# a16z/Lasso

Hardware: AMD Instinct MI355X
Metric: prover lookups/sec for SparsePolynomialEvaluationProof, 2^24 AND lookups (higher is better)
Workload: dtype u256 (Montgomery Fr / ed25519 Fq integers)

## Files before the change

### lasso_amd/build.py

```python
import os
import subprocess
import sys

HERE = os.path.dirname(os.path.abspath(__file__))
ROOT = os.path.dirname(HERE)
HIPCC = os.environ.get("HIPCC", "/opt/rocm/bin/hipcc")
ARCH = "gfx950"


def _stale(target, sources):
    if not os.path.exists(target):
        return True
    t = os.path.getmtime(target)
    return any(os.path.getmtime(s) > t for s in sources)


def _glob(d, exts):
    return [os.path.join(d, f) for f in sorted(os.listdir(d)) if f.endswith(exts)]


CURVES = {"curve25519": ("", []), "bn254": ("_bn254", ["-DLASSO_BN254", "-Wl,-Bsymbolic"])}


def build_device(force=False, verbose=False, curve="curve25519"):
    suffix, flags = CURVES[curve]
    csrc = os.path.join(HERE, "csrc")
    target = os.path.join(HERE, f"liblasso_hip{suffix}.so")
    sources = _glob(csrc, (".hip", ".cuh")) + [os.path.join(ROOT, "include", f) for f in ("lasso_hip.h", "lasso_hip_wire.h", "lasso_hip_msm.h", "lasso_custom_check.h")]
    if force or _stale(target, sources):
        extra = os.environ.get("LASSO_EXTRA_HIPCC_FLAGS", "").split()
        cmd = [HIPCC, f"--offload-arch={ARCH}", "-O3", "-std=c++17", "-fPIC", "-shared", "-Wno-unused-result", *flags, *extra,
               "-o", target, os.path.join(csrc, "lasso_hip.hip")]
        if verbose:
            print(" ".join(cmd))
        subprocess.check_call(cmd)
    return target


def host_march_flags():
    ov = os.environ.get("LASSO_HOST_MARCH")
    if ov:
        return [] if ov == "none" else [f"-march={ov}"] + (["-DLASSO_HOST_V3"] if ov == "x86-64-v3" else [])
    try:
        flags = set(next(l for l in open("/proc/cpuinfo") if l.startswith("flags")).split())
    except Exception:
        flags = set()
    if {"avx2", "bmi1", "bmi2", "fma", "movbe"} <= flags:
        return ["-march=x86-64-v3", "-DLASSO_HOST_V3"]
    return []


def build_host(force=False, verbose=False, curve="curve25519"):
    suffix, flags = CURVES[curve]
    hdir = os.path.join(HERE, "host")
    target = os.path.join(HERE, f"liblasso_prover{suffix}.so")
    sources = _glob(hdir, (".cpp", ".hpp")) + _glob(os.path.join(HERE, "csrc"), (".cuh",)) + [os.path.join(ROOT, "include", f) for f in ("lasso_hip.h", "lasso_hip_wire.h", "lasso_hip_msm.h", "lasso_prover.h", "lasso_custom_check.h")]
    if not os.path.exists(os.path.join(hdir, "prover_capi.cpp")):
        return None
    dev = build_device(force=False, verbose=verbose, curve=curve)
    if force or _stale(target, sources + [dev]):
        cmd = ["g++", "-O2", *host_march_flags(), "-std=c++17", "-fPIC", "-shared", "-Wall", "-Wno-unused-function", "-Wno-unknown-pragmas", "-fno-gnu-unique", "-Wl,-Bsymbolic", *flags, "-o", target,
               os.path.join(hdir, "prover_capi.cpp"), "-L" + HERE, f"-llasso_hip{suffix}", "-Wl,-rpath,$ORIGIN"]
        if verbose:
            print(" ".join(cmd))
        subprocess.check_call(cmd)
    return target


def build_all(force=False, verbose=False):
    out = []
    for curve in CURVES:
        out += [build_device(force, verbose, curve), build_host(force, verbose, curve)]
    return tuple(out)


if __name__ == "__main__":
    print(build_all(force="--force" in sys.argv, verbose=True))
```

### lasso_amd/csrc/device_switches.cuh

```cuda
#pragma once
#include <cstddef>
#include <cstdint>
#include <cstdlib>

namespace lasso { namespace dsw {
inline bool unless0(const char* e) { return !(e && e[0] == '0'); }
inline bool if1(const char* e) { return e && e[0] == '1'; }
#define LASSO_DSWITCH(type, name, value) inline type name() { static const type v = (value); return v; }
LASSO_DSWITCH(bool, tagged_results, unless0(getenv("LASSO_TAGGED_RESULTS")))
LASSO_DSWITCH(long long, seq_start, [] { const char* e = getenv("LASSO_SEQ_START"); return e ? (long long)(uint32_t)strtoul(e, nullptr, 0) : -1LL; }())
LASSO_DSWITCH(bool, msm_tagged, unless0(getenv("LASSO_MSM_TAGGED")))
LASSO_DSWITCH(long, cubic_nx, [] { const char* e = getenv("LASSO_CUBIC_NX"); return e ? atol(e) : 0L; }())
LASSO_DSWITCH(bool, cubic_wide, unless0(getenv("LASSO_CUBIC_WIDE")))
LASSO_DSWITCH(unsigned, direct_nx, [] { const char* e = getenv("LASSO_DIRECT_NX"); const long x = e ? atol(e) : 16; return (unsigned)(x < 0 ? 0 : x > 64 ? 64 : x); }())
LASSO_DSWITCH(bool, eq_inline_big, if1(getenv("LASSO_EQ_INLINE_BIG")))
LASSO_DSWITCH(bool, lb_pipeline, unless0(getenv("LASSO_LB_PIPELINE")))
LASSO_DSWITCH(bool, lb_nt, if1(getenv("LASSO_LB_NT")))
LASSO_DSWITCH(unsigned, ahead_inkernel_wgs, [] { const char* e = getenv("LASSO_AHEAD_INKERNEL_WGS"); const long x = e ? atol(e) : 32; return (unsigned)(x < 0 ? 0 : x > 4096 ? 4096 : x); }())
LASSO_DSWITCH(bool, rounds_ahead, unless0(getenv("LASSO_ROUNDS_AHEAD")))
LASSO_DSWITCH(bool, layer_ahead, unless0(getenv("LASSO_LAYER_AHEAD")))
LASSO_DSWITCH(bool, tail_q_256, [] { const char* e = getenv("LASSO_TAIL_Q"); return (e ? atol(e) : 0) == 256; }())
LASSO_DSWITCH(bool, exp_no_leaf_store, if1(getenv("LASSO_EXP_NO_LEAF_STORE")))
LASSO_DSWITCH(size_t, msm_direct_max_n, [] { const char* e = getenv("LASSO_MSM_DIRECT_MAX_N"); return e ? (size_t)atoll(e) : (((size_t)1 << 17) + 64); }())
LASSO_DSWITCH(size_t, msm_direct8_max_n, [] { if (!unless0(getenv("LASSO_MSM_DIRECT8"))) return (size_t)0; const char* e = getenv("LASSO_MSM_DIRECT8_MAX_N"); return e ? (size_t)atoll(e) : (((size_t)1 << 14) + 64); }())
LASSO_DSWITCH(bool, msm_direct, unless0(getenv("LASSO_MSM_DIRECT")))
LASSO_DSWITCH(long, msm_direct_wgs, [] { const char* e = getenv("LASSO_MSM_DIRECT_WGS"); return e ? atol(e) : 0L; }())
LASSO_DSWITCH(bool, msm_fused, unless0(getenv("LASSO_MSM_FUSED")))
LASSO_DSWITCH(bool, msm_rows8, unless0(getenv("LASSO_MSM_ROWS8")))
LASSO_DSWITCH(bool, msm_rows8w, unless0(getenv("LASSO_MSM_ROWS8W")))
LASSO_DSWITCH(size_t, msm_rows8w_waves, [] { const char* e = getenv("LASSO_MSM_ROWS8W_WAVES"); const long x = e ? atol(e) : 0; return (size_t)(x < 0 ? 0 : x); }())
LASSO_DSWITCH(bool, msm_full8, if1(getenv("LASSO_MSM_FULL8")))
LASSO_DSWITCH(bool, bullet_ahead, unless0(getenv("LASSO_BULLET_AHEAD")))
LASSO_DSWITCH(bool, bullet_tail_ahead, unless0(getenv("LASSO_BULLET_TAIL_AHEAD")))
inline bool msm_pip() { return unless0(getenv("LASSO_MSM_PIP")); }
inline size_t msm_pip_min_cols() { const char* e = getenv("LASSO_MSM_PIP_MIN_COLS"); const long x = e ? atol(e) : 512; return (size_t)(x < 1 ? 1 : x); }
inline size_t msm_pip_scratch_mb() { const char* e = getenv("LASSO_MSM_PIP_SCRATCH_MB"); const long x = e ? atol(e) : 1200; return (size_t)(x < 16 ? 16 : x); }
#undef LASSO_DSWITCH
} }
```

### lasso_amd/csrc/lasso_hip.hip

```cpp
#include <hip/hip_runtime.h>
#include <mutex>
#include <string>
#include <unordered_map>
#include <vector>
#include <cstring>
#include <cstdio>
#include <cstdlib>
#include <ctime>
#include "../../include/lasso_hip.h"
#include "device_switches.cuh"
#include "launch_plan.cuh"
#include "poly_kernels.cuh"
#include "msm_kernels.cuh"
#include "densify_kernels.cuh"
#include "../../include/lasso_hip_wire.h"
#include "wire_kernels.cuh"
#include "../../include/lasso_hip_msm.h"
#include "msm_points_kernels.cuh"

__global__ void __launch_bounds__(256) k_inner_lr(const fr_t* __restrict__ a, const fr_t* __restrict__ b, size_t half, fr_t* __restrict__ partials) {
  __shared__ RedScratch S;
  fr29 acc[3] = {fr29_zero(), fr29_zero(), fr29_zero()}; uint32_t cnt = 0;
  for (size_t i = blockIdx.x * (size_t)blockDim.x + threadIdx.x; i < half; i += (size_t)gridDim.x * blockDim.x) {
    acc[0] = fr29_weak(fr29_add(acc[0], fr29_mul(fr29_unpack_u(a[i]), fr29_unpack_s(b[half + i]))));
    acc[1] = fr29_weak(fr29_add(acc[1], fr29_mul(fr29_unpack_u(a[half + i]), fr29_unpack_s(b[i]))));
    if ((++cnt & 127u) == 0) { acc[0] = fr29_mul(acc[0], fr29_one_s()); acc[1] = fr29_mul(acc[1], fr29_one_s()); }
  }
  store_block_partials<3>(acc, 2, partials + 2 * (size_t)blockIdx.x, 0, S);
}

static_assert(sizeof(lasso_fr) == 32 && sizeof(fr_t) == 32, "Fr layout");
static_assert(sizeof(lasso_affine) == 64 && sizeof(lasso_point) == 128 && sizeof(ed_point) == 128 && sizeof(niels29) == (MSM_NIELS_ALIGN > 16 ? 128 : 112) && sizeof(pt29) == MSM_PT29_BYTES, "curve layouts");

namespace dsw = lasso::dsw;
struct EventPair { hipEvent_t a, b; int kid; double bytes, units, units2; bool large; bool counted; };
#define LASSO_PROF_COUNT_SLOTS 4096
struct lasso_ctx {
  int device = 0;
  hipStream_t stream = nullptr;
  std::string err;
  void* d_scratch = nullptr; size_t scratch_cap = 0;
  void* d_pip = nullptr; size_t pip_cap = 0;
  fr_t* d_small = nullptr;
  fr_t* h_small = nullptr;
  size_t small_cap = 0;
  uint32_t* h_flag = nullptr; uint32_t* d_flag = nullptr;
  uint32_t* h_tag = nullptr; uint32_t* d_tag = nullptr;
  bool tagged = true;
  HandoffState proto;
  std::vector<lasso_fr> group_tmp;
  uint32_t* mail_h = nullptr; uint32_t* mail_d = nullptr;
  uint32_t seq = 0;
  uint64_t stat_waits = 0; double stat_wait_us = 0;
  fr_t* d_big = nullptr; fr_t* h_big = nullptr; size_t big_cap = 0;
  uint32_t* d_flags = nullptr;
  uint32_t* d_counters = nullptr;
  uint32_t* d_gmail = nullptr;
  uint32_t* pmail_h = nullptr; uint32_t* pmail_d = nullptr; uint32_t* d_gpoint = nullptr;
  uint32_t prof_mask = 0;
  std::vector<EventPair> events; size_t events_used = 0;
  uint64_t prof_launches[LASSO_K_COUNT] = {0}; double prof_ms[LASSO_K_COUNT] = {0}; double prof_bytes[LASSO_K_COUNT] = {0};
  uint64_t big_launches[LASSO_K_COUNT] = {0}; double big_ms[LASSO_K_COUNT] = {0}; double big_bytes[LASSO_K_COUNT] = {0};
  double prof_units[LASSO_K_COUNT] = {0}; double big_units[LASSO_K_COUNT] = {0};
  double prof_units2[LASSO_K_COUNT] = {0}; double big_units2[LASSO_K_COUNT] = {0};
  double prof_units3[LASSO_K_COUNT] = {0}; double big_units3[LASSO_K_COUNT] = {0};
  uint32_t* d_prof_counts = nullptr;
  void* d_terms = nullptr; std::vector<uint8_t> terms_host;
  void* rccl_comm = nullptr; int rccl_world = 0; int rccl_rank = -1;
  std::unordered_map<void*, size_t> mem_sizes; uint64_t mem_live = 0, mem_peak = 0; std::mutex mem_mu;
};
struct lasso_bases {
  size_t n = 0; niels29* d_table = nullptr;
  lasso_ctx* owner = nullptr;
  niels29* d_mult = nullptr;
  niels29* d_mult8 = nullptr;
  niels29* d_tab8[2] = {nullptr, nullptr};
  bool tab8_failed = false;
  std::mutex tab8_mu;
};

static thread_local std::string g_create_err;
static std::mutex g_ctx_mu; static std::vector<lasso_ctx*> g_ctx_live;
static lasso_ctx* live_or_null(lasso_ctx* c) { std::lock_guard<std::mutex> g(g_ctx_mu); for (lasso_ctx* x : g_ctx_live) if (x == c) return c; return nullptr; }

static int32_t fail(lasso_ctx* c, int32_t code, const std::string& msg) { if (c) c->err = msg; else g_create_err = msg; return code; }
#define HIPCHK(c, call) do { hipError_t e_ = (call); if (e_ != hipSuccess) return fail((c), e_ == hipErrorOutOfMemory ? LASSO_ERR_OOM : LASSO_ERR_HIP, std::string(#call) + ": " + hipGetErrorString(e_)); } while (0)
static inline bool bind_device(lasso_ctx* c) { if (!c) return true; int d = -1; if (hipGetDevice(&d) == hipSuccess && d == c->device) return true; return hipSetDevice(c->device) == hipSuccess; }
#define REQUIRE(c, cond) do { if (!bind_device(c)) return fail((c), LASSO_ERR_HIP, "hipSetDevice failed for the context's device"); \
                              if (!(cond)) return fail((c), LASSO_ERR_INVALID, std::string("invalid argument: ") + #cond); } while (0)

static hipError_t dmalloc(lasso_ctx* c, void** p, size_t bytes) {
  hipError_t e = hipMalloc(p, bytes);
  if (e == hipSuccess && c) { std::lock_guard<std::mutex> g(c->mem_mu); c->mem_sizes[*p] = bytes; c->mem_live += bytes; if (c->mem_live > c->mem_peak) c->mem_peak = c->mem_live; }
  return e;
}
static hipError_t dfree(lasso_ctx* c, void* p) {
  if (c && p) { std::lock_guard<std::mutex> g(c->mem_mu); auto it = c->mem_sizes.find(p); if (it != c->mem_sizes.end()) { c->mem_live -= it->second; c->mem_sizes.erase(it); } }
  return hipFree(p);
}

static int32_t grow_guard(lasso_ctx* c) {
  if (c->proto.no_grow) return LASSO_ERR_UNSUPPORTED;
  if (c->proto.waiting_on_device()) return fail(c, LASSO_ERR_INVALID, "a launch is waiting on the device for its challenge: only lasso_result_wait and the post of that challenge are legal until then");
  return 0;
}
static int32_t ensure_scratch(lasso_ctx* c, size_t bytes) {
  if (bytes <= c->scratch_cap) return 0;
  if (int32_t g = grow_guard(c)) return g;
  if (c->d_scratch) { HIPCHK(c, hipStreamSynchronize(c->stream)); HIPCHK(c, dfree(c, c->d_scratch)); c->d_scratch = nullptr; c->scratch_cap = 0; }
  size_t cap = bytes < ((size_t)1 << 22) ? ((size_t)1 << 22) : bytes;
  HIPCHK(c, dmalloc(c, &c->d_scratch, cap)); c->scratch_cap = cap; return 0;
}
static int32_t ensure_pip(lasso_ctx* c, size_t bytes) {
  if (bytes <= c->pip_cap) return 0;
  if (!c->proto.may_grow()) return LASSO_ERR_UNSUPPORTED;
  if (c->d_pip) { HIPCHK(c, hipStreamSynchronize(c->stream)); HIPCHK(c, dfree(c, c->d_pip)); c->d_pip = nullptr; c->pip_cap = 0; }
  if (dmalloc(c, &c->d_pip, bytes) != hipSuccess) { (void)hipGetLastError(); c->d_pip = nullptr; return LASSO_ERR_UNSUPPORTED; }
  c->pip_cap = bytes; return 0;
}
static int32_t ensure_small(lasso_ctx* c, size_t count) {
  if (count <= c->small_cap) return 0;
  if (int32_t g = grow_guard(c)) return g;
  HIPCHK(c, hipStreamSynchronize(c->stream));
  if (c->h_small) (void)hipHostFree(c->h_small);
  c->h_small = nullptr; c->d_small = nullptr; c->small_cap = 0;
  size_t cap = count < 4096 ? 4096 : count;
  HIPCHK(c, hipHostMalloc((void**)&c->h_small, cap * sizeof(fr_t), hipHostMallocMapped | hipHostMallocCoherent));
  HIPCHK(c, hipHostGetDevicePointer((void**)&c->d_small, c->h_small, 0));
  if (c->h_tag) (void)hipHostFree(c->h_tag);
  c->h_tag = nullptr; c->d_tag = nullptr;
  HIPCHK(c, hipHostMalloc((void**)&c->h_tag, cap * 48, hipHostMallocMapped | hipHostMallocCoherent));
  memset(c->h_tag, 0, cap * 48);
  HIPCHK(c, hipHostGetDevicePointer((void**)&c->d_tag, c->h_tag, 0));
  c->small_cap = cap; return 0;
}
static int32_t ensure_big(lasso_ctx* c, size_t count) {
  if (count <= c->big_cap) return 0;
  if (int32_t g = grow_guard(c)) return g;
  HIPCHK(c, hipStreamSynchronize(c->stream));
  if (c->d_big) (void)dfree(c, c->d_big);
  if (c->h_big) (void)hipHostFree(c->h_big);
// ... 199 lines not shown
      rc = LASSO_ERR_HIP; msg = "lasso_rccl_selftest: the 1 KB all-gather did not complete within 20 s (a peer never entered it, or the fabric is down)";
      if (a->CommAbort) (void)a->CommAbort((ncclComm_t)c->rccl_comm); c->rccl_comm = nullptr; c->rccl_world = 0;
    }
  }
  if (!rc) {
    if (hipMemcpy(all.data(), d + bytes, bytes * (size_t)world, hipMemcpyDeviceToHost) != hipSuccess) { rc = LASSO_ERR_HIP; msg = "lasso_rccl_selftest: download"; }
    else for (int g = 0; g < world && !rc; g++) for (size_t i = 0; i < bytes; i++) if (all[(size_t)g * bytes + i] != (uint8_t)(((size_t)g * 131 + i * 7 + 1) % 251)) { rc = LASSO_ERR_HIP; msg = "lasso_rccl_selftest: slot " + std::to_string(g) + " does not hold rank " + std::to_string(g) + "'s bytes"; break; }
  }
  if (ev) (void)hipEventDestroy(ev);
  if (c->rccl_comm || rc == 0) (void)hipFree(d);
  (void)hipGetLastError();
  return rc ? fail(c, rc, msg) : 0;
}
int32_t lasso_rccl_allgather(lasso_ctx* c, const void* d_send, void* d_recv, size_t bytes) {
  REQUIRE(c, d_send && d_recv && c->rccl_comm);
  RcclApi* a = rccl_api(nullptr);
  ncclResult_t r = a->AllGather(d_send, d_recv, bytes, ncclUint8, (ncclComm_t)c->rccl_comm, c->stream);
  if (r != ncclSuccess) return fail(c, LASSO_ERR_HIP, std::string("ncclAllGather: ") + a->GetErrorString(r));
  return 0;
}
int32_t lasso_points_reduce_compress(lasso_ctx* c, const void* d_parts, uint32_t groups, size_t rows, uint8_t* out32) {
  REQUIRE(c, d_parts && out32 && groups >= 1 && rows >= 1);
  int32_t rc = ensure_scratch(c, rows * 32 + 256); if (rc) return rc;
  {
    ProfScope ps(c, LASSO_K_MSM, (double)groups * rows * sizeof(pt29), (double)(groups - 1) * rows);
    hipLaunchKernelGGL(k_points_reduce_compress, dim3(grid_for(rows)), dim3(256), 0, c->stream, (const pt29*)d_parts, groups, rows, (uint32_t*)c->d_scratch);
  }
  HIPCHK(c, hipGetLastError());
  HIPCHK(c, hipMemcpyAsync(out32, c->d_scratch, rows * 32, hipMemcpyDeviceToHost, c->stream));
  HIPCHK(c, hipStreamSynchronize(c->stream));
  return 0;
}

static inline void post_mail(lasso_ctx* c, uint32_t tag, const uint32_t w[8]) {
  mail_chunks(c->mail_h, tag, w);
  mail_fence();
}
int32_t lasso_ctx_create(int32_t device, lasso_ctx** out) { return lasso_ctx_create_background(device, 0, out); }
int32_t lasso_ctx_device_uuid(lasso_ctx* c, uint8_t out[16]) {
  REQUIRE(c, c && out);
  hipUUID u; memset(&u, 0, sizeof(u));
  HIPCHK(c, hipDeviceGetUuid(&u, c->device));
  static_assert(sizeof(u.bytes) == 16, "hipUUID");
  memcpy(out, u.bytes, 16); return 0;
}
int32_t lasso_ctx_create_background(int32_t device, int32_t background, lasso_ctx** out) {
  if (!out) return fail(nullptr, LASSO_ERR_INVALID, "out is NULL");
  int n = 0;
  hipError_t e = hipGetDeviceCount(&n);
  if (e != hipSuccess || n == 0) return fail(nullptr, LASSO_ERR_HIP, std::string("no HIP device: ") + hipGetErrorString(e));
  if (device < 0 || device >= n) return fail(nullptr, LASSO_ERR_INVALID, "device index out of range");
  lasso_ctx* c = new lasso_ctx(); c->device = device;
  int prio_lo = 0, prio_hi = 0;
  if ((e = hipSetDevice(device)) == hipSuccess) (void)hipDeviceGetStreamPriorityRange(&prio_lo, &prio_hi);
  if (e != hipSuccess || (e = hipStreamCreateWithPriority(&c->stream, hipStreamNonBlocking, background ? prio_lo : prio_hi)) != hipSuccess) {
    std::string m = hipGetErrorString(e); delete c; return fail(nullptr, LASSO_ERR_HIP, m);
  }
  if (hipMalloc((void**)&c->d_flags, 64) != hipSuccess) { delete c; return fail(nullptr, LASSO_ERR_OOM, "flags alloc"); }
  if (hipMalloc((void**)&c->d_counters, (LASSO_MAX_PTRS + 40) * 4) != hipSuccess || hipMemset(c->d_counters, 0, (LASSO_MAX_PTRS + 40) * 4) != hipSuccess) { delete c; return fail(nullptr, LASSO_ERR_OOM, "counters alloc"); }
  if (hipHostMalloc((void**)&c->h_flag, 256, hipHostMallocMapped | hipHostMallocCoherent) != hipSuccess || hipHostGetDevicePointer((void**)&c->d_flag, c->h_flag, 0) != hipSuccess) { delete c; return fail(nullptr, LASSO_ERR_OOM, "mapped flag alloc"); }
  *c->h_flag = 0;
  c->tagged = dsw::tagged_results();
  if (dsw::seq_start() >= 0) c->seq = (uint32_t)dsw::seq_start();
  c->mail_h = c->h_flag + 32; c->mail_d = c->d_flag + 32;
  memset(c->h_flag, 0, 256);
  int32_t rc = ensure_small(c, (size_t)1 << 16); if (rc) { g_create_err = c->err; delete c; return rc; }
  rc = ensure_scratch(c, (size_t)1 << 22); if (rc) { g_create_err = c->err; delete c; return rc; }
  if (dmalloc(c, (void**)&c->d_gmail, 128) != hipSuccess || hipMemset(c->d_gmail, 0, 128) != hipSuccess) { g_create_err = "gmail alloc"; delete c; return LASSO_ERR_OOM; }
  if (hipHostMalloc((void**)&c->pmail_h, LASSO_PMAIL_BYTES, hipHostMallocMapped | hipHostMallocCoherent) != hipSuccess || hipHostGetDevicePointer((void**)&c->pmail_d, c->pmail_h, 0) != hipSuccess) { g_create_err = "point mailbox alloc"; delete c; return LASSO_ERR_OOM; }
  memset(c->pmail_h, 0, LASSO_PMAIL_BYTES);
  if (dmalloc(c, (void**)&c->d_gpoint, LASSO_GPOINT_BYTES) != hipSuccess || hipMemset(c->d_gpoint, 0, LASSO_GPOINT_BYTES) != hipSuccess) { g_create_err = "gpoint alloc"; delete c; return LASSO_ERR_OOM; }
  { std::lock_guard<std::mutex> g(g_ctx_mu); g_ctx_live.push_back(c); }
  *out = c; return 0;
}
int32_t lasso_abort(lasso_ctx* c) {
  REQUIRE(c, c);
  const uint32_t zero8[8] = {0, 0, 0, 0, 0, 0, 0, 0};
  if (c->proto.lay_active && c->pmail_h) for (uint32_t j = 0; j < LASSO_POINT_MAX + 2; j++) mail_chunks(c->pmail_h + 12 * j, LASSO_MAIL_POISON, zero8);
  if (c->proto.tail_active || c->proto.waiting_on_device()) { mail_chunks(c->mail_h + 12, LASSO_MAIL_POISON, zero8); post_mail(c, LASSO_MAIL_POISON, zero8); }
  (void)hipStreamSynchronize(c->stream);
  (void)hipGetLastError();
  if (c->pmail_h) memset(c->pmail_h, 0, LASSO_PMAIL_BYTES);
  mail_chunks(c->mail_h + 12, 0, zero8); post_mail(c, 0, zero8);
  c->proto.reset(); c->events_used = 0;
  HIPCHK(c, hipMemsetAsync(c->d_counters, 0, (LASSO_MAX_PTRS + 40) * 4, c->stream));
  HIPCHK(c, hipStreamSynchronize(c->stream));
  return 0;
}
void lasso_ctx_destroy(lasso_ctx* c) {
  if (!c) return;
  { std::lock_guard<std::mutex> g(g_ctx_mu); for (size_t i = 0; i < g_ctx_live.size(); i++) if (g_ctx_live[i] == c) { g_ctx_live.erase(g_ctx_live.begin() + i); break; } }
  (void)hipSetDevice(c->device);
  if (!c->proto.idle()) (void)lasso_abort(c);
  (void)hipStreamSynchronize(c->stream);
  rccl_release(c);
  for (auto& p : c->events) { (void)hipEventDestroy(p.a); (void)hipEventDestroy(p.b); }
  if (c->d_scratch) (void)hipFree(c->d_scratch);
  if (c->d_pip) (void)hipFree(c->d_pip);
  if (c->d_gmail) (void)hipFree(c->d_gmail);
  if (c->d_gpoint) (void)hipFree(c->d_gpoint);
  if (c->pmail_h) (void)hipHostFree(c->pmail_h);
  if (c->h_small) (void)hipHostFree(c->h_small);
  if (c->h_tag) (void)hipHostFree(c->h_tag);
  if (c->h_flag) (void)hipHostFree(c->h_flag);
  if (c->d_big) (void)hipFree(c->d_big);
  if (c->h_big) (void)hipHostFree(c->h_big);
  if (c->d_flags) (void)hipFree(c->d_flags);
  if (c->d_counters) (void)hipFree(c->d_counters);
  if (c->d_prof_counts) (void)hipFree(c->d_prof_counts);
  if (c->d_terms) (void)hipFree(c->d_terms);
  (void)hipStreamDestroy(c->stream);
  delete c;
}
const char* lasso_last_error(lasso_ctx* c) { return c ? c->err.c_str() : g_create_err.c_str(); }
void* lasso_stream(lasso_ctx* c) { return c ? (void*)c->stream : nullptr; }
int32_t lasso_alloc(lasso_ctx* c, size_t bytes, void** d_out) { REQUIRE(c, d_out); HIPCHK(c, dmalloc(c, d_out, bytes ? bytes : 1)); return 0; }
int32_t lasso_free(lasso_ctx* c, void* p) { if (!p) return 0; REQUIRE(c, c && !c->proto.waiting_on_device()); HIPCHK(c, hipStreamSynchronize(c->stream)); HIPCHK(c, dfree(c, p)); return 0; }
int32_t lasso_mem_stats(lasso_ctx* c, uint64_t* live_bytes, uint64_t* peak_bytes, int32_t reset_peak) {
  REQUIRE(c, c); std::lock_guard<std::mutex> g(c->mem_mu);
  if (live_bytes) *live_bytes = c->mem_live; if (peak_bytes) *peak_bytes = c->mem_peak; if (reset_peak) c->mem_peak = c->mem_live; return 0;
}
int32_t lasso_trim(lasso_ctx* c) {
  REQUIRE(c, c && c->proto.idle());
  HIPCHK(c, hipStreamSynchronize(c->stream));
  if (c->d_pip) { HIPCHK(c, dfree(c, c->d_pip)); c->d_pip = nullptr; c->pip_cap = 0; }
  if (c->scratch_cap <= ((size_t)1 << 22)) return 0;
  HIPCHK(c, dfree(c, c->d_scratch)); c->d_scratch = nullptr; c->scratch_cap = 0;
  return ensure_scratch(c, (size_t)1 << 22);
}
int32_t lasso_upload(lasso_ctx* c, void* d, const void* s, size_t n) { REQUIRE(c, d && s && !c->proto.waiting_on_device()); HIPCHK(c, hipMemcpyAsync(d, s, n, hipMemcpyHostToDevice, c->stream)); HIPCHK(c, hipStreamSynchronize(c->stream)); return 0; }
int32_t lasso_download(lasso_ctx* c, void* d, const void* s, size_t n) { REQUIRE(c, d && s && !c->proto.waiting_on_device()); HIPCHK(c, hipMemcpyAsync(d, s, n, hipMemcpyDeviceToHost, c->stream)); HIPCHK(c, hipStreamSynchronize(c->stream)); return 0; }
int32_t lasso_copy(lasso_ctx* c, void* d, const void* s, size_t n) { REQUIRE(c, d && s); ProfScope ps(c, LASSO_K_MISC, 2.0 * n); HIPCHK(c, hipMemcpyAsync(d, s, n, hipMemcpyDeviceToDevice, c->stream)); return 0; }
int32_t lasso_zero(lasso_ctx* c, void* d, size_t n) { REQUIRE(c, d); HIPCHK(c, hipMemsetAsync(d, 0, n, c->stream)); return 0; }
int32_t lasso_sync(lasso_ctx* c) { REQUIRE(c, c && !c->proto.waiting_on_device()); HIPCHK(c, hipStreamSynchronize(c->stream)); return 0; }

int32_t lasso_prof_get_large(lasso_ctx* c, int32_t k, uint64_t* launches, double* ms, double* bytes) {
  REQUIRE(c, k >= 0 && k < LASSO_K_COUNT); prof_flush(c);
  if (launches) *launches = c->big_launches[k]; if (ms) *ms = c->big_ms[k]; if (bytes) *bytes = c->big_bytes[k]; return 0;
}
int32_t lasso_wait_stats(lasso_ctx* c, uint64_t* waits, double* wait_us, int32_t reset) { REQUIRE(c, waits && wait_us); *waits = c->stat_waits; *wait_us = c->stat_wait_us; if (reset) { c->stat_waits = 0; c->stat_wait_us = 0; } return 0; }
int32_t lasso_prof_enable(lasso_ctx* c, int32_t mask) { prof_flush(c); c->prof_mask = (uint32_t)mask; return 0; }
int32_t lasso_prof_reset(lasso_ctx* c) { prof_flush(c); for (int i = 0; i < LASSO_K_COUNT; i++) { c->prof_launches[i] = 0; c->prof_ms[i] = 0; c->prof_bytes[i] = 0; c->big_launches[i] = 0; c->big_ms[i] = 0; c->big_bytes[i] = 0; c->prof_units[i] = 0; c->big_units[i] = 0; c->prof_units2[i] = 0; c->big_units2[i] = 0; c->prof_units3[i] = 0; c->big_units3[i] = 0; } return 0; }
int32_t lasso_prof_get_units(lasso_ctx* c, int32_t k, int32_t large_only, double* units) {
  REQUIRE(c, k >= 0 && k < LASSO_K_COUNT && units); prof_flush(c);
  const bool large = large_only & 1, second = large_only & 2, third = large_only & 4;
  *units = third ? (large ? c->big_units3[k] : c->prof_units3[k]) : second ? (large ? c->big_units2[k] : c->prof_units2[k]) : (large ? c->big_units[k] : c->prof_units[k]); return 0;
}
int32_t lasso_prof_get(lasso_ctx* c, int32_t k, uint64_t* launches, double* ms, double* bytes) {
  REQUIRE(c, k >= 0 && k < LASSO_K_COUNT); prof_flush(c);
  if (launches) *launches = c->prof_launches[k]; if (ms) *ms = c->prof_ms[k]; if (bytes) *bytes = c->prof_bytes[k]; return 0;
}

int32_t lasso_fr_from_u32(lasso_ctx* c, const uint32_t* d_src, size_t n, lasso_fr* d_dst) {
  REQUIRE(c, d_src && d_dst); if (!n) return 0;
  ProfScope ps(c, LASSO_K_MISC, 36.0 * n);
  hipLaunchKernelGGL(k_from_u32, dim3(grid_for(n)), dim3(LASSO_BLOCK), 0, c->stream, d_src, n, (fr_t*)d_dst);
  HIPCHK(c, hipGetLastError()); return 0;
}
__global__ void __launch_bounds__(256) k_subtable_u32(int32_t kind, uint32_t sub, uint32_t log_m, uint32_t log_r, uint32_t* __restrict__ out) {
  const size_t m = (size_t)1 << log_m; const uint32_t bits = log_m / 2, mask = (1u << bits) - 1u;
  for (size_t i = blockIdx.x * (size_t)blockDim.x + threadIdx.x; i < m; i += (size_t)gridDim.x * blockDim.x) {
    const uint32_t r = (uint32_t)i & mask, l = (uint32_t)(i >> bits) & mask;
    uint32_t v;
    if (kind == LASSO_AND) v = l & r;
    else if (kind == LASSO_OR) v = l | r;
    else if (kind == LASSO_XOR) v = l ^ r;
    else if (kind == LASSO_LT) v = sub == 0 ? (l < r ? 1u : 0u) : (l == r ? 1u : 0u);
    else { const size_t cutoff = (size_t)1 << (log_r % log_m); v = sub == 0 ? (uint32_t)i : (sub == 1 ? (i < cutoff ? (uint32_t)i : 0u) : 0u); }
    out[i] = v;
  }
}
int32_t lasso_materialize_subtable_u32(lasso_ctx* c, const lasso_strategy* s, uint32_t sub, uint32_t* d_out) {
  REQUIRE(c, s && d_out && s->kind >= LASSO_AND && s->kind <= LASSO_RANGE && s->log_m >= 1 && s->log_m <= 31);
  const uint32_t nsub = s->kind == LASSO_LT ? 2u : (s->kind == LASSO_RANGE ? 3u : 1u);
  REQUIRE(c, sub < nsub);
  hipLaunchKernelGGL(k_subtable_u32, dim3(grid_for((size_t)1 << s->log_m)), dim3(256), 0, c->stream, s->kind, sub, s->log_m, s->log_r, d_out);
  HIPCHK(c, hipGetLastError()); return 0;
}
int32_t lasso_gather(lasso_ctx* c, const lasso_fr* d_table, const uint32_t* d_idx, size_t n, lasso_fr* d_out) {
  REQUIRE(c, d_table && d_idx && d_out); if (!n) return 0;
  ProfScope ps(c, LASSO_K_MISC, 68.0 * n);
  hipLaunchKernelGGL(k_gather, dim3(grid_for(n)), dim3(LASSO_BLOCK), 0, c->stream, (const fr_t*)d_table, d_idx, n, (fr_t*)d_out);
  HIPCHK(c, hipGetLastError()); return 0;
}
int32_t lasso_eq_evals(lasso_ctx* c, const lasso_fr* r, uint32_t ell, lasso_fr* d_out) { return lasso_eq_evals_scaled(c, r, ell, nullptr, d_out); }
int32_t lasso_eq_evals_scaled(lasso_ctx* c, const lasso_fr* r, uint32_t ell, const lasso_fr* scale, lasso_fr* d_out) {
  REQUIRE(c, d_out && ell <= 40 && (r || ell == 0));
  const fr_t sc = scale ? to_fr(scale) : fr_one();
  const size_t n = (size_t)1 << ell;
  ProfScope ps(c, LASSO_K_EQ, 32.0 * n);
  if (ell <= 12) {
    RTable R; for (uint32_t j = 0; j < ell; j++) R.r[j] = to_fr(r + j);
    hipLaunchKernelGGL(k_eq_small, dim3(grid_for(n)), dim3(LASSO_BLOCK), 0, c->stream, R, ell, sc, (fr_t*)d_out);
  } else {
    const uint32_t lo_bits = ell / 2, hi_bits = ell - lo_bits;
    int32_t rc = ensure_scratch(c, (((size_t)1 << hi_bits) + ((size_t)1 << lo_bits)) * sizeof(fr_t)); if (rc) return rc;
    fr_t* hi = (fr_t*)c->d_scratch; fr_t* lo = hi + ((size_t)1 << hi_bits);
    if (hi_bits <= 16) {
      RTable16 Rh, Rl; for (uint32_t j = 0; j < 16; j++) { Rh.r[j] = j < hi_bits ? to_fr(r + j) : fr_zero(); Rl.r[j] = j < lo_bits ? to_fr(r + hi_bits + j) : fr_zero(); }
      const unsigned hb = grid_for((size_t)1 << hi_bits), lb = grid_for((size_t)1 << lo_bits);
      hipLaunchKernelGGL(k_eq_small2, dim3(hb + lb), dim3(LASSO_BLOCK), 0, c->stream, Rh, hi_bits, sc, hi, hb, Rl, lo_bits, lo);
    } else {
      RTable Rh, Rl; for (uint32_t j = 0; j < hi_bits; j++) Rh.r[j] = to_fr(r + j); for (uint32_t j = 0; j < lo_bits; j++) Rl.r[j] = to_fr(r + hi_bits + j);
      hipLaunchKernelGGL(k_eq_small, dim3(grid_for((size_t)1 << hi_bits)), dim3(LASSO_BLOCK), 0, c->stream, Rh, hi_bits, sc, hi);
      hipLaunchKernelGGL(k_eq_small, dim3(grid_for((size_t)1 << lo_bits)), dim3(LASSO_BLOCK), 0, c->stream, Rl, lo_bits, fr_one(), lo);
    }
    hipLaunchKernelGGL(k_eq_outer, dim3(grid_for(n, 4096)), dim3(LASSO_BLOCK), 0, c->stream, (const fr_t*)hi, (const fr_t*)lo, lo_bits, n, (fr_t*)d_out);
  }
  HIPCHK(c, hipGetLastError()); return 0;
}
int32_t lasso_bind_top(lasso_ctx* c, lasso_fr* const* d_polys, uint32_t npolys, size_t n, const lasso_fr* r) {
  REQUIRE(c, d_polys && r && npolys >= 1 && npolys <= LASSO_MAX_PTRS && n >= 2 && (n & (n - 1)) == 0);
  MutPtrTable T; for (uint32_t i = 0; i < npolys; i++) { REQUIRE(c, d_polys[i]); T.p[i] = (fr_t*)d_polys[i]; }
  const size_t half = n / 2;
  ProfScope ps(c, LASSO_K_BIND, 48.0 * n * npolys);
  hipLaunchKernelGGL(k_bind_top, dim3(grid_for(half, 4096), npolys), dim3(LASSO_BLOCK), 0, c->stream, T, half, to_fr(r));
  HIPCHK(c, hipGetLastError()); return 0;
}
static unsigned round_nx(size_t items, unsigned ny) { return round_nx(items, ny, dsw::cubic_nx()); }
int32_t lasso_sumcheck_cubic_round(lasso_ctx* c, const lasso_fr* const* d_A, const lasso_fr* const* d_B, uint32_t ncirc, const lasso_fr* d_C, size_t n, lasso_fr* out) {
  REQUIRE(c, d_A && d_B && d_C && out && ncirc >= 1 && ncirc <= LASSO_MAX_PTRS && n >= 2 && (n & (n - 1)) == 0);
  const size_t half = n / 2;
  int32_t rc = ensure_small(c, (size_t)ncirc * 3); if (rc) return rc;
  const uint32_t seq = next_seq(c);
  PtrTable A, B; for (uint32_t i = 0; i < ncirc; i++) { REQUIRE(c, d_A[i] && d_B[i]); A.p[i] = (const fr_t*)d_A[i]; B.p[i] = (const fr_t*)d_B[i]; }
  const unsigned ny = ncirc, nx = round_nx(half, ny);
  rc = ensure_scratch(c, (size_t)nx * ny * 3 * sizeof(fr_t)); if (rc) return rc;
  {
    ProfScope ps(c, LASSO_K_CUBIC, 32.0 * n * (2.0 * ncirc + 1.0));
    hipLaunchKernelGGL(k_cubic_round_lb, dim3(nx * ny), dim3(LASSO_BLOCK), 0, c->stream, A, B, nx, ny, (const fr_t*)d_C, half, (fr_t*)c->d_scratch, c->d_counters, RES(c), seq);
  }
  HIPCHK(c, hipGetLastError());
  return wait_flag(c, seq, (size_t)ncirc * 3, out, c->tagged);
}
extern "C++" {
struct EqPointArg { const lasso_fr* point; uint32_t ell; fr_t scale; };
static CubicPlan cubic_plan_for(lasso_ctx* c, uint32_t ncirc, size_t n, bool has_r, int NT, bool has_eqi, bool want_groups, bool ahead, const EqPointArg* eqg, int gate_ell) {
  const CubicShape s = {n, ncirc, NT, ahead, has_r, has_eqi, eqg != nullptr, eqg ? eqg->ell : 0u, gate_ell, c->prof_mask, want_groups && c->tagged};
  const CubicSwitches sw = {dsw::cubic_nx(), dsw::cubic_wide(), dsw::direct_nx(), dsw::eq_inline_big(), dsw::lb_pipeline(), dsw::lb_nt(), dsw::ahead_inkernel_wgs()};
  return cubic_plan(s, sw);
}
template <class TM, class TP>
static int32_t cubic_eqw_launch_t(lasso_ctx* c, lasso_fr* const* d_A, lasso_fr* const* d_B, uint32_t ncirc, const lasso_fr* d_E, size_t n, const lasso_fr* r, int NT, uint32_t* seq_out, const EqInline* eqi, uint32_t* groups_out, bool ahead = false, const EqPointArg* eqg = nullptr, int gate_ell = -1) {
  if (groups_out) *groups_out = 1;
  const CubicPlan P = cubic_plan_for(c, ncirc, n, r != nullptr, NT, eqi != nullptr, groups_out != nullptr, ahead, eqg, gate_ell);
  if (P.form == CUBIC_REFUSED) return fail(c, LASSO_ERR_UNSUPPORTED, P.refusal);
  TM A, B; for (uint32_t i = 0; i < ncirc; i++) { REQUIRE(c, d_A[i] && d_B[i]); A.p[i] = (fr_t*)d_A[i]; B.p[i] = (fr_t*)d_B[i]; }
  int32_t rc = ensure_small(c, (size_t)ncirc * 3); if (rc) return rc;
  const uint32_t seq = next_seq(c); *seq_out = seq;
  const unsigned nx = P.nx, ny = P.ny;
  const fr_t rr = r ? to_fr(r) : fr_zero();
  const double bytes = (P.bind ? 48.0 : 32.0) * n * (2.0 * ncirc + 1.0);
  fr_t* r_out = nullptr; uint32_t* r_flag = nullptr;
  auto reserve = [&]() -> int32_t {
    int32_t e = ensure_scratch(c, P.scratch_elems * sizeof(fr_t)); if (e) return e;
    if (P.direct) { *groups_out = nx; e = ensure_small(c, (size_t)ncirc * 3 * nx); if (e) return e; }
    r_out = c->tagged ? (fr_t*)c->d_tag : c->d_small; r_flag = P.direct ? LASSO_TAGGED_DIRECT : c->tagged ? LASSO_TAGGED : c->d_flag;
    return 0;
  };
  if (P.form == CUBIC_SMALL) {
    ProfScope ps(c, LASSO_K_CUBIC, bytes);
#define LAUNCH_CSMALL(BIND_, NT_) hipLaunchKernelGGL((k_cubic_eqw_small<BIND_, NT_, TM>), dim3(ncirc), dim3(LASSO_BLOCK), 0, c->stream, A, B, (const fr_t*)d_E, (uint32_t)P.items, rr, c->d_counters, RES(c), seq)
    if (P.bind) { if (NT == 3) LAUNCH_CSMALL(true, 3); else LAUNCH_CSMALL(true, 2); }
    else { if (NT == 3) LAUNCH_CSMALL(false, 3); else LAUNCH_CSMALL(false, 2); }
  } else if (P.form == CUBIC_FUSED) {
    if (ahead) { if ((rc = reserve())) return rc; if (P.gate) hipLaunchKernelGGL(k_gate, dim3(1), dim3(64), 0, c->stream, (const uint32_t*)c->mail_d, c->d_gmail, seq, 0u); }
    ProfScope ps(c, LASSO_K_CUBIC, bytes);
    if (!ahead && (rc = reserve())) return rc;
    const uint32_t* const gmail = ahead ? (const uint32_t*)c->d_gmail : (const uint32_t*)nullptr; const uint32_t* const wait_mail = P.inkernel ? (const uint32_t*)c->mail_d : (const uint32_t*)nullptr;
#define LAUNCH_CFUSED(NT_, WIDE_, AHEAD_) hipLaunchKernelGGL((k_cubic_eqw_fused<NT_, WIDE_, TM, AHEAD_>), dim3(nx * ny), dim3(LASSO_BLOCK), 0, c->stream, A, B, nx, ny, (const fr_t*)d_E, P.items, rr, (fr_t*)c->d_scratch, c->d_counters, r_out, r_flag, seq, gmail, wait_mail)
    if (ahead) { if (P.wide) LAUNCH_CFUSED(2, true, true); else LAUNCH_CFUSED(2, false, true); }
    else if (NT == 3) LAUNCH_CFUSED(3, false, false);
    else if (P.wide) LAUNCH_CFUSED(2, true, false);
    else LAUNCH_CFUSED(2, false, false);
  } else {
    const CubicLbPlan& L = P.lb;
    TP Ac, Bc; for (uint32_t i = 0; i < ncirc; i++) { Ac.p[i] = A.p[i]; Bc.p[i] = B.p[i]; }
    if ((rc = reserve())) return rc;
    fr_t* const f_hi = (fr_t*)c->d_scratch + P.part_elems; fr_t* const f_lo = f_hi + ((size_t)1 << L.g_hi);
    if (L.gate) { hipLaunchKernelGGL(k_gate_point, dim3(1), dim3(64), 0, c->stream, (const uint32_t*)c->pmail_d, c->d_gpoint, seq, (uint32_t)gate_ell + 2u, c->pmail_d + LASSO_PMAIL_ACK_WORD); c->proto.gate_sent = seq; }
    const uint32_t* const gate_gp = L.gate ? (const uint32_t*)c->d_gpoint : (const uint32_t*)nullptr;
    if (L.factors) {
      ProfScope pe(c, LASSO_K_EQ, L.eq_outer ? 32.0 * P.items : 32.0 * (((size_t)1 << L.g_hi) + ((size_t)1 << L.g_lo)));
      const unsigned hb = grid_for((size_t)1 << L.g_hi), lb2 = grid_for((size_t)1 << L.g_lo);
      if (L.factors_gated) hipLaunchKernelGGL(k_eq_small2_mem, dim3(hb + lb2), dim3(LASSO_BLOCK), 0, c->stream, (const uint32_t*)c->d_gpoint, seq, L.g_hi, f_hi, hb, L.g_lo, f_lo);
      else {
        RTable16 Rh, Rl; for (uint32_t j = 0; j < 16; j++) { Rh.r[j] = j < L.g_hi ? to_fr(eqg->point + j) : fr_zero(); Rl.r[j] = j < L.g_lo ? to_fr(eqg->point + L.g_hi + j) : fr_zero(); }
        hipLaunchKernelGGL(k_eq_small2, dim3(hb + lb2), dim3(LASSO_BLOCK), 0, c->stream, Rh, L.g_hi, eqg->scale, f_hi, hb, Rl, L.g_lo, f_lo);
      }
      if (L.eq_outer) hipLaunchKernelGGL(k_eq_outer, dim3(grid_for(P.items, 4096)), dim3(LASSO_BLOCK), 0, c->stream, (const fr_t*)f_hi, (const fr_t*)f_lo, L.g_lo, P.items, (fr_t*)d_E, gate_gp, seq);
    }
    ProfScope ps(c, LASSO_K_CUBIC, bytes);
#define LAUNCH_CLB(NT_, EQI_, TE_, NTL_, E_, EQ_, OUT_) hipLaunchKernelGGL((k_cubic_eqw_lb<NT_, EQI_, TP, TE_, NTL_>), dim3(nx * ny), dim3(LASSO_BLOCK), 0, c->stream, Ac, Bc, nx, ny, (const fr_t*)(E_), P.items, (fr_t*)c->d_scratch, c->d_counters, r_out, r_flag, seq, L.pipe, EQ_, (fr_t*)(OUT_))
    switch (L.eq) {
      case CUBIC_EQ_TABLE: {
        EqNone EN; if (L.eq_outer) { EN.gp = gate_gp; EN.seq = seq; }
        if (NT == 3) LAUNCH_CLB(3, false, EqNone, false, d_E, EN, nullptr);
        else if (L.nt) LAUNCH_CLB(2, false, EqNone, true, d_E, EN, nullptr);
        else LAUNCH_CLB(2, false, EqNone, false, d_E, EN, nullptr);
      } break;
      case CUBIC_EQ_LDS: LAUNCH_CLB(2, true, EqInline, false, nullptr, *eqi, d_E); break;
      case CUBIC_EQ_GATED: { EqInlineMem M; M.gp = c->d_gpoint; M.seq = seq; M.ell = (uint32_t)gate_ell; LAUNCH_CLB(2, true, EqInlineMem, false, nullptr, M, d_E); } break;
      case CUBIC_EQ_FACTORS: {
        EqGlobal G; G.hi = f_hi; G.lo = f_lo; G.lo_bits = L.g_lo; G.ell = L.g_ell; G.gp = L.gate ? c->d_gpoint : nullptr; G.seq = L.gate ? seq : 0;
        LAUNCH_CLB(2, true, EqGlobal, false, nullptr, G, d_E);
      } break;
    }
  }
  HIPCHK(c, hipGetLastError());
  return 0;
}
}
static int32_t cubic_eqw_launch(lasso_ctx* c, lasso_fr* const* d_A, lasso_fr* const* d_B, uint32_t ncirc, const lasso_fr* d_E, size_t n, const lasso_fr* r, int NT, uint32_t* seq_out, const EqInline* eqi = nullptr, uint32_t* groups_out = nullptr, bool ahead = false, const EqPointArg* eqg = nullptr, int gate_ell = -1) {
  return ncirc <= 8 ? cubic_eqw_launch_t<MutPtrTable8, PtrTable8>(c, d_A, d_B, ncirc, d_E, n, r, NT, seq_out, eqi, groups_out, ahead, eqg, gate_ell) : cubic_eqw_launch_t<MutPtrTable, PtrTable>(c, d_A, d_B, ncirc, d_E, n, r, NT, seq_out, eqi, groups_out, ahead, eqg, gate_ell);
}
int32_t lasso_sumcheck_cubic_eqw_round(lasso_ctx* c, const lasso_fr* const* d_A, const lasso_fr* const* d_B, uint32_t ncirc, const lasso_fr* d_E, size_t n, lasso_fr* out) {
  REQUIRE(c, d_A && d_B && d_E && out && ncirc >= 1 && ncirc <= LASSO_MAX_PTRS && n >= 2 && (n & (n - 1)) == 0);
  uint32_t seq, groups; int32_t rc = cubic_eqw_launch(c, (lasso_fr* const*)d_A, (lasso_fr* const*)d_B, ncirc, d_E, n, nullptr, 3, &seq, nullptr, &groups); if (rc) return rc;
  return wait_flag(c, seq, (size_t)ncirc * 3, out, c->tagged, groups, 3);
}
int32_t lasso_sumcheck_cubic_eqw_round_fused(lasso_ctx* c, lasso_fr* const* d_A, lasso_fr* const* d_B, uint32_t ncirc, const lasso_fr* d_E, size_t n, const lasso_fr* r, lasso_fr* out) {
  REQUIRE(c, d_A && d_B && d_E && r && out && ncirc >= 1 && ncirc <= LASSO_MAX_PTRS && n >= 4 && (n & (n - 1)) == 0);
  uint32_t seq, groups; int32_t rc = cubic_eqw_launch(c, d_A, d_B, ncirc, d_E, n, r, 3, &seq, nullptr, &groups); if (rc) return rc;
  return wait_flag(c, seq, (size_t)ncirc * 3, out, c->tagged, groups, 3);
}
int32_t lasso_sumcheck_cubic_eqw2_begin(lasso_ctx* c, lasso_fr* const* d_A, lasso_fr* const* d_B, uint32_t ncirc, const lasso_fr* d_E, size_t n, const lasso_fr* r) {
  REQUIRE(c, d_A && d_B && d_E && ncirc >= 1 && ncirc <= LASSO_MAX_PTRS && n >= (r ? 4u : 2u) && (n & (n - 1)) == 0 && !c->proto.pending);
  uint32_t seq, groups; int32_t rc = cubic_eqw_launch(c, d_A, d_B, ncirc, d_E, n, r, 2, &seq, nullptr, &groups); if (rc) return rc;
  c->proto.park(Handoff{seq, (size_t)ncirc * 2, c->tagged, groups, 2});
  return 0;
}
int32_t lasso_sumcheck_cubic_eqw2_begin_ahead(lasso_ctx* c, lasso_fr* const* d_A, lasso_fr* const* d_B, uint32_t ncirc, const lasso_fr* d_E, size_t n) {
  REQUIRE(c, d_A && d_B && d_E && ncirc >= 1 && ncirc <= LASSO_MAX_PTRS && n >= 4 && (n & (n - 1)) == 0 && !c->proto.ahead_active && !c->proto.tail_active && !c->proto.defer_next);
  const CubicPlan P = cubic_plan_for(c, ncirc, n, false, 2, false, true, true, nullptr, -1);
  if (P.form == CUBIC_REFUSED) return fail(c, LASSO_ERR_UNSUPPORTED, "lasso_sumcheck_cubic_eqw2_begin_ahead: streaming rounds only");
  { int32_t rc0 = ensure_small(c, (size_t)ncirc * 3 * (P.direct ? P.nx : 1)); if (rc0) return rc0; rc0 = ensure_scratch(c, P.scratch_elems * sizeof(fr_t)); if (rc0) return rc0; }
  uint32_t seq, groups; int32_t rc = cubic_eqw_launch(c, d_A, d_B, ncirc, d_E, n, nullptr, 2, &seq, nullptr, &groups, true); if (rc) return rc;
  c->proto.arm_ahead(Handoff{seq, (size_t)ncirc * 2, c->tagged, groups, 2}, false);
  return 0;
}
int32_t lasso_challenge_post(lasso_ctx* c, const lasso_fr* r) {
  REQUIRE(c, r && c->proto.ahead_active && !c->proto.ahead_bullet && !c->proto.pending);
  post_mail(c, c->proto.post_ahead(), (const uint32_t*)r);
  return 0;
}
int32_t lasso_rounds_ahead_ok(lasso_ctx* c) { return c && dsw::rounds_ahead() && c->mail_d && c->d_gmail ? 1 : 0; }
static int32_t cubic_tail_begin_impl(lasso_ctx* c, uint32_t m_stop, lasso_fr* const* d_A, lasso_fr* const* d_B, uint32_t ncirc, const lasso_fr* d_E, size_t n, const lasso_fr* r, const EqInline* eqi, bool ahead, int gate_ell = -1);
static uint32_t take_handover(lasso_ctx* c) { return c ? c->proto.take_handover() : 0; }
int32_t lasso_sumcheck_cubic_tail_begin(lasso_ctx* c, lasso_fr* const* d_A, lasso_fr* const* d_B, uint32_t ncirc, const lasso_fr* d_E, size_t n, const lasso_fr* r) {
  const uint32_t ho = take_handover(c);
  REQUIRE(c, d_E);
  return cubic_tail_begin_impl(c, ho, d_A, d_B, ncirc, d_E, n, r, nullptr, false);
}
static bool make_eq_inline(const lasso_fr* point, uint32_t ell, const lasso_fr* scale, EqInline& Q) {
  if (ell > 14 || (ell && !point)) return false;
  for (uint32_t j = 0; j < 14; j++) Q.r[j] = j < ell ? to_fr(point + j) : fr_zero();
  Q.scale = scale ? to_fr(scale) : fr_one(); Q.ell = ell; return true;
}
int32_t lasso_sumcheck_cubic_eqw2_begin_eq(lasso_ctx* c, lasso_fr* const* d_A, lasso_fr* const* d_B, uint32_t ncirc, lasso_fr* d_E_out, size_t n, const lasso_fr* point, uint32_t ell, const lasso_fr* scale) {
  REQUIRE(c, d_A && d_B && d_E_out && ncirc >= 1 && ncirc <= LASSO_MAX_PTRS && n >= 2 && (n & (n - 1)) == 0 && !c->proto.pending && ((size_t)1 << ell) == n / 2);
  EqInline Q;
  if (n / 2 <= CUBIC_SMALL_Q || (ell && !point) || ell > 32) return fail(c, LASSO_ERR_UNSUPPORTED, "lasso_sumcheck_cubic_eqw2_begin_eq: tables of 2^7 .. 2^32 entries only");
  uint32_t seq, groups; int32_t rc;
  if (make_eq_inline(point, ell, scale, Q)) rc = cubic_eqw_launch(c, d_A, d_B, ncirc, d_E_out, n, nullptr, 2, &seq, &Q, &groups);
  else { EqPointArg G; G.point = point; G.ell = ell; G.scale = scale ? to_fr(scale) : fr_one(); rc = cubic_eqw_launch(c, d_A, d_B, ncirc, d_E_out, n, nullptr, 2, &seq, nullptr, &groups, false, &G); }
  if (rc) return rc;
  c->proto.park(Handoff{seq, (size_t)ncirc * 2, c->tagged, groups, 2});
  return 0;
}
int32_t lasso_sumcheck_cubic_tail_begin_eq(lasso_ctx* c, lasso_fr* const* d_A, lasso_fr* const* d_B, uint32_t ncirc, size_t n, const lasso_fr* point, uint32_t ell, const lasso_fr* scale) {
  const uint32_t ho = take_handover(c);
  REQUIRE(c, n >= 2 && ((size_t)1 << ell) == n / 2 && ell <= 9);
  EqInline Q; if (!make_eq_inline(point, ell, scale, Q)) return fail(c, LASSO_ERR_INVALID, "lasso_sumcheck_cubic_tail_begin_eq: bad point");
  return cubic_tail_begin_impl(c, ho, d_A, d_B, ncirc, nullptr, n, nullptr, &Q, false);
}
extern "C++" {
template <class TM>
static int32_t cubic_tail_begin_t(lasso_ctx* c, uint32_t m_stop_arg, lasso_fr* const* d_A, lasso_fr* const* d_B, uint32_t ncirc, const lasso_fr* d_E, size_t n, const lasso_fr* r, const EqInline* eqi, bool ahead, int gate_ell) {
  const uint32_t m_stop = m_stop_arg ? m_stop_arg : 1u;
  const bool gated = gate_ell >= 0;
  REQUIRE(c, d_A && d_B && (d_E || eqi || gated) && ncirc >= 1 && ncirc <= LASSO_MAX_PTRS && n >= ((r || ahead) ? 4u : 2u) && (n & (n - 1)) == 0 && (ahead || gated || !c->proto.pending) && (gated || !c->proto.tail_active) && !c->proto.defer_next && !c->proto.ahead_active && !c->proto.lay_active);
  const size_t q = (r || ahead) ? n / 4 : n / 2;
  REQUIRE(c, q >= 1 && q <= CUBIC_TAIL_Q && (m_stop & (m_stop - 1)) == 0 && m_stop <= 128 && 2 * q > m_stop);
  TM A, B; for (uint32_t i = 0; i < ncirc; i++) { REQUIRE(c, d_A[i] && d_B[i]); A.p[i] = (fr_t*)d_A[i]; B.p[i] = (fr_t*)d_B[i]; }
  int32_t rc = ensure_small(c, (size_t)ncirc * 2 * (m_stop > 2 ? m_stop : 2)); if (rc) return rc;
  uint32_t turns = 0; while (((size_t)m_stop << turns) < 2 * q) turns++;
  const uint32_t seq0 = next_seq(c, turns + 1);
#define LAUNCH_CTAIL(B_, Q_, I_, TE_, R_, EQ_) hipLaunchKernelGGL((k_cubic_tail<B_, Q_, I_, TM, TE_>), dim3(ncirc), dim3(Q_), 0, c->stream, A, B, (const fr_t*)d_E, (uint32_t)q, R_, (const uint32_t*)c->mail_d, c->d_counters, RES(c), seq0, EQ_, m_stop, ahead ? 1u : 0u)
  if (gated) {
    hipLaunchKernelGGL(k_gate_point, dim3(1), dim3(64), 0, c->stream, (const uint32_t*)c->pmail_d, c->d_gpoint, seq0, (uint32_t)gate_ell + 2u, c->pmail_d + LASSO_PMAIL_ACK_WORD); c->proto.gate_sent = seq0;
    EqInlineMem M; M.gp = c->d_gpoint; M.seq = seq0; M.ell = (uint32_t)gate_ell;
    if (tail_threads(q) == 256) LAUNCH_CTAIL(false, 256, true, EqInlineMem, fr_zero(), M); else LAUNCH_CTAIL(false, 512, true, EqInlineMem, fr_zero(), M);
    HIPCHK(c, hipGetLastError());
    c->proto.arm_layer_tail(Handoff{seq0, (size_t)ncirc * 2, c->tagged}, (uint32_t)gate_ell, turns, (size_t)ncirc * 2 * m_stop);
    return 0;
  }
  if (eqi) { if (tail_threads(q) == 256) LAUNCH_CTAIL(false, 256, true, EqInline, fr_zero(), *eqi); else LAUNCH_CTAIL(false, 512, true, EqInline, fr_zero(), *eqi); }
  else if (tail_threads(q) == 256) { if (r || ahead) LAUNCH_CTAIL(true, 256, false, EqNone, r ? to_fr(r) : fr_zero(), EqNone()); else LAUNCH_CTAIL(false, 256, false, EqNone, fr_zero(), EqNone()); }
  else { if (r || ahead) LAUNCH_CTAIL(true, 512, false, EqNone, r ? to_fr(r) : fr_zero(), EqNone()); else LAUNCH_CTAIL(false, 512, false, EqNone, fr_zero(), EqNone()); }
  HIPCHK(c, hipGetLastError());
  c->proto.begin_tail(Handoff{seq0, (size_t)ncirc * 2, c->tagged}, turns, (size_t)ncirc * 2 * m_stop, ahead);
  return 0;
}
}
static int32_t cubic_tail_begin_impl(lasso_ctx* c, uint32_t m_stop, lasso_fr* const* d_A, lasso_fr* const* d_B, uint32_t ncirc, const lasso_fr* d_E, size_t n, const lasso_fr* r, const EqInline* eqi, bool ahead, int gate_ell) {
  return ncirc <= 8 ? cubic_tail_begin_t<MutPtrTable8>(c, m_stop, d_A, d_B, ncirc, d_E, n, r, eqi, ahead, gate_ell) : cubic_tail_begin_t<MutPtrTable>(c, m_stop, d_A, d_B, ncirc, d_E, n, r, eqi, ahead, gate_ell);
}
static bool gate_free(lasso_ctx* c) { return !c->proto.gate_sent || __atomic_load_n(c->pmail_h + LASSO_PMAIL_ACK_WORD, __ATOMIC_ACQUIRE) == c->proto.gate_sent; }
int32_t lasso_layer_ahead_ok(lasso_ctx* c) { return c && dsw::layer_ahead() && c->pmail_d && c->d_gpoint ? 1 : 0; }
int32_t lasso_sumcheck_cubic_eqw2_begin_eq_ahead(lasso_ctx* c, lasso_fr* const* d_A, lasso_fr* const* d_B, uint32_t ncirc, lasso_fr* d_E_out, size_t n, uint32_t ell) {
  REQUIRE(c, d_A && d_B && d_E_out && ncirc >= 1 && ncirc <= LASSO_MAX_PTRS && n >= 2 && (n & (n - 1)) == 0 && ell < 48 && ((size_t)1 << ell) == n / 2 && !c->proto.waiting_on_device() && !c->proto.defer_next);
  if (!lasso_layer_ahead_ok(c) || n / 2 <= CUBIC_SMALL_Q || ell > 32 || ell > LASSO_POINT_MAX) return fail(c, LASSO_ERR_UNSUPPORTED, "lasso_sumcheck_cubic_eqw2_begin_eq_ahead: tables of 2^7 .. 2^32 entries only");
  if (!gate_free(c)) return fail(c, LASSO_ERR_UNSUPPORTED, "lasso_sumcheck_cubic_eqw2_begin_eq_ahead: the previous point gate has not consumed its message yet");
  uint32_t seq, groups;
  c->proto.no_grow = true;
  const int32_t rc = cubic_eqw_launch(c, d_A, d_B, ncirc, d_E_out, n, nullptr, 2, &seq, nullptr, &groups, false, nullptr, (int)ell);
  c->proto.no_grow = false;
  if (rc == LASSO_ERR_UNSUPPORTED) return fail(c, rc, "lasso_sumcheck_cubic_eqw2_begin_eq_ahead: a buffer would have to grow while kernels are in flight");
  if (rc) return rc;
  HIPCHK(c, hipGetLastError());
  c->proto.arm_layer(Handoff{seq, (size_t)ncirc * 2, c->tagged, groups, 2}, ell);
  return 0;
}
int32_t lasso_sumcheck_cubic_tail_begin_eq_ahead(lasso_ctx* c, lasso_fr* const* d_A, lasso_fr* const* d_B, uint32_t ncirc, size_t n, uint32_t ell) {
  const uint32_t ho = take_handover(c);
  REQUIRE(c, n >= 2 && ell <= 9 && ((size_t)1 << ell) == n / 2);
  if (!lasso_layer_ahead_ok(c)) return fail(c, LASSO_ERR_UNSUPPORTED, "lasso_sumcheck_cubic_tail_begin_eq_ahead: switched off");
  if (!gate_free(c)) return fail(c, LASSO_ERR_UNSUPPORTED, "lasso_sumcheck_cubic_tail_begin_eq_ahead: the previous point gate has not consumed its message yet");
  c->proto.no_grow = true;
  const int32_t rc = cubic_tail_begin_impl(c, ho, d_A, d_B, ncirc, nullptr, n, nullptr, nullptr, false, (int)ell);
  c->proto.no_grow = false;
  if (rc == LASSO_ERR_UNSUPPORTED) return fail(c, rc, "lasso_sumcheck_cubic_tail_begin_eq_ahead: a buffer would have to grow while kernels are in flight");
  return rc;
}
static void point_mail(lasso_ctx* c, uint32_t ell, const lasso_fr* point, const lasso_fr* scale, uint32_t ctrl) {
  const uint32_t zero8[8] = {0, 0, 0, 0, 0, 0, 0, 0}; const fr_t one = fr_one();
  for (uint32_t j = 0; j < ell; j++) mail_chunks(c->pmail_h + 12 * j, c->proto.lay.seq, point ? (const uint32_t*)(point + j) : zero8);
  mail_chunks(c->pmail_h + 12 * ell, c->proto.lay.seq, scale ? (const uint32_t*)scale : one.v);
  const uint32_t ctl[8] = {ctrl, 0, 0, 0, 0, 0, 0, 0};
  mail_chunks(c->pmail_h + 12 * (ell + 1), c->proto.lay.seq, ctl);
  mail_fence();
}
int32_t lasso_point_post(lasso_ctx* c, const lasso_fr* point, uint32_t ell, const lasso_fr* scale) {
  REQUIRE(c, c && c->proto.lay_active && ell == c->proto.lay_ell && (point || !ell) && !c->proto.pending && !c->proto.tail_active && !c->proto.ahead_active);
  point_mail(c, ell, point, scale, 0u);
  c->proto.post_layer();
  return 0;
}
int32_t lasso_point_cancel(lasso_ctx* c) {
  REQUIRE(c, c && c->proto.lay_active);
  point_mail(c, c->proto.lay_ell, nullptr, nullptr, 1u);
  c->proto.cancel_layer();
  return 0;
}
int32_t lasso_sumcheck_cubic_tail_begin_ahead(lasso_ctx* c, lasso_fr* const* d_A, lasso_fr* const* d_B, uint32_t ncirc, const lasso_fr* d_E, size_t n) {
  const uint32_t ho = take_handover(c);
  REQUIRE(c, d_E);
  return cubic_tail_begin_impl(c, ho, d_A, d_B, ncirc, d_E, n, nullptr, nullptr, true);
}
int32_t lasso_tail_handover_next(lasso_ctx* c, uint32_t m_stop) {
  REQUIRE(c, c && (m_stop & (m_stop - 1)) == 0 && m_stop <= 128);
  c->proto.handover_next = m_stop <= 1 ? 0 : m_stop; return 0;
}
int32_t lasso_sumcheck_linear_tail_begin(lasso_ctx* c, const lasso_fr* const* d_src, uint32_t alpha, const lasso_fr* d_E, size_t n, const lasso_fr* r) {
  const uint32_t ho = take_handover(c);
  REQUIRE(c, d_src && d_E && alpha >= 1 && alpha <= LASSO_MAX_PTRS && n >= (r ? 4u : 2u) && (n & (n - 1)) == 0 && !c->proto.pending && !c->proto.tail_active && !c->proto.defer_next && !ho && !c->proto.ahead_active);
  const size_t q = r ? n / 4 : n / 2;
  REQUIRE(c, q >= 1 && q <= CUBIC_TAIL_Q);
  PtrTable Src; for (uint32_t i = 0; i < alpha; i++) { REQUIRE(c, d_src[i]); Src.p[i] = (const fr_t*)d_src[i]; }
  int32_t rc = ensure_small(c, (size_t)alpha * 3); if (rc) return rc;
  uint32_t turns = 0; while (((size_t)1 << turns) < 2 * q) turns++;
  const uint32_t seq0 = next_seq(c, turns + 1);
#define LAUNCH_LTAIL(B_, Q_, R_) hipLaunchKernelGGL((k_linear_tail<B_, Q_>), dim3(alpha), dim3(Q_), 0, c->stream, Src, (const fr_t*)d_E, (uint32_t)q, R_, (const uint32_t*)c->mail_d, c->d_counters, RES(c), seq0)
  if (tail_threads(q) == 256) { if (r) LAUNCH_LTAIL(true, 256, to_fr(r)); else LAUNCH_LTAIL(false, 256, fr_zero()); }
  else { if (r) LAUNCH_LTAIL(true, 512, to_fr(r)); else LAUNCH_LTAIL(false, 512, fr_zero()); }
  HIPCHK(c, hipGetLastError());
  c->proto.begin_tail(Handoff{seq0, (size_t)alpha * 2, c->tagged}, turns, alpha, false);
  return 0;
}
int32_t lasso_sumcheck_cubic_tail_next(lasso_ctx* c, const lasso_fr* r) {
  REQUIRE(c, r && c->proto.tail_active && !c->proto.pending);
  const fr_t rr = to_fr(r);
  post_mail(c, c->proto.tail_next(), rr.v);
  return 0;
}
uint32_t lasso_sumcheck_tail_capacity(void) { return dsw::tail_q_256() ? 256 : CUBIC_TAIL_Q; }
int32_t lasso_defer_next(lasso_ctx* c) { REQUIRE(c, !c->proto.pending && !c->proto.defer_next); c->proto.defer_next = true; return 0; }
int32_t lasso_result_wait(lasso_ctx* c, lasso_fr* out, size_t count) {
  REQUIRE(c, out && c->proto.pending && count == c->proto.result.count);
  const Handoff h = c->proto.collect();
  return wait_flag(c, h.seq, count, out, h.tagged, h.groups, h.K);
}
// ... 899 lines not shown
```

### lasso_amd/csrc/launch_plan.cuh

```cuda
#pragma once
#include <cstddef>
#include <cstdint>
#include "../../include/lasso_hip.h"

#define LASSO_BLOCK 256
#define CUBIC_SMALL_Q 64
#define CUBIC_TAIL_Q 512
#define MSM_THREADS 256
#define MSM_WINDOWS 64
#define MSM_PIP_WINDOWS 21
#define MSM_PIP_BUCKETS 2048
#define MSM_SMALL_ROWS 16
#define MSM_PT29_BYTES 144
#ifdef LASSO_BN254
#define FR_MODULUS_BITS 254u
#else
#define FR_MODULUS_BITS 253u
#endif
constexpr uint32_t msm_direct_windows(int wb) { return 256u / (uint32_t)wb; }

static inline unsigned grid_for(size_t n, unsigned cap = 2048) { size_t g = (n + LASSO_BLOCK - 1) / LASSO_BLOCK; if (g < 1) g = 1; if (g > cap) g = cap; return (unsigned)g; }
static inline bool prof_bracketed(uint32_t prof_mask, int family) { return ((prof_mask >> family) & 1u) && !(prof_mask & (uint32_t)LASSO_PROF_LARGE_ONLY); }

static inline unsigned round_nx(size_t items, unsigned ny, long cubic_nx) {
  unsigned cap = 512 / (ny ? ny : 1); if (cap < 64) cap = 64;
  return grid_for(items, cubic_nx > 0 ? (unsigned)cubic_nx : cap);
}
static inline unsigned tail_threads(size_t q) { return q <= 256 ? 256u : 512u; }

struct CubicSwitches { long cubic_nx; bool wide; unsigned direct_nx; bool eq_inline_big, lb_pipeline, lb_nt; unsigned ahead_inkernel_wgs; };
struct CubicShape { size_t n; uint32_t ncirc; int NT; bool ahead, has_r, has_eqi, has_eqg; uint32_t eqg_ell; int gate_ell; uint32_t prof_mask; bool direct_ok; };
enum CubicForm { CUBIC_REFUSED, CUBIC_SMALL, CUBIC_LB, CUBIC_FUSED };
enum CubicEq {
  CUBIC_EQ_TABLE,
  CUBIC_EQ_LDS,
  CUBIC_EQ_GATED,
  CUBIC_EQ_FACTORS
};
struct CubicLbPlan {
  CubicEq eq;
  bool gate;
  bool factors;
  bool factors_gated;
  bool eq_outer;
  uint32_t g_ell, g_hi, g_lo;
  uint32_t pipe;
  bool nt;
};
struct CubicPlan {
  CubicForm form; const char* refusal;
  bool bind;
  size_t items;
  unsigned nx, ny;
  size_t part_elems;
  size_t scratch_elems;
  bool direct;
  bool wide;
  bool gate, inkernel;
  CubicLbPlan lb;
};
static inline CubicPlan cubic_plan(const CubicShape& s, const CubicSwitches& sw) {
  CubicPlan p = {}; p.ny = s.ncirc; p.nx = 1;
  if (s.ahead && (s.NT != 2 || s.n / 4 <= CUBIC_SMALL_Q)) { p.form = CUBIC_REFUSED; p.refusal = "a round launched ahead of its challenge: two-sum streaming rounds only (more than 64 index quadruples per circuit)"; return p; }
  p.bind = s.has_r || s.ahead; p.items = p.bind ? s.n / 4 : s.n / 2;
  if (p.items <= CUBIC_SMALL_Q) { p.form = CUBIC_SMALL; return p; }
  p.form = p.bind ? CUBIC_FUSED : CUBIC_LB;
  p.nx = round_nx(p.items, p.ny, sw.cubic_nx);
  p.part_elems = p.scratch_elems = (size_t)p.nx * p.ny * 3;
  p.direct = s.direct_ok && p.nx > 1 && p.nx <= sw.direct_nx;
  if (p.bind) {
    p.wide = s.NT == 2 && sw.wide;
    if (s.ahead) { p.inkernel = p.nx * p.ny <= sw.ahead_inkernel_wgs && !prof_bracketed(s.prof_mask, LASSO_K_CUBIC); p.gate = !p.inkernel; }
    return p;
  }
  CubicLbPlan& l = p.lb;
  const bool gated = s.gate_ell >= 0, gbig = gated && s.gate_ell > 14;
  l.g_ell = gbig ? (uint32_t)s.gate_ell : s.has_eqg ? s.eqg_ell : 0; l.g_lo = l.g_ell / 2; l.g_hi = l.g_ell - l.g_lo;
  if (s.has_eqg || gbig) p.scratch_elems += ((size_t)1 << l.g_hi) + ((size_t)1 << l.g_lo);
  if (s.NT != 2) { l.eq = CUBIC_EQ_TABLE; l.pipe = 0; return p; }
  l.gate = gated; l.factors = gbig || s.has_eqg; l.factors_gated = gbig; l.eq_outer = l.factors && !sw.eq_inline_big;
  l.eq = l.eq_outer ? CUBIC_EQ_TABLE : gated ? (gbig ? CUBIC_EQ_FACTORS : CUBIC_EQ_GATED) : s.has_eqg ? CUBIC_EQ_FACTORS : s.has_eqi ? CUBIC_EQ_LDS : CUBIC_EQ_TABLE;
  const bool plain = l.eq == CUBIC_EQ_TABLE;
  l.pipe = plain ? (sw.lb_pipeline ? 1u : 0u) : 1u;
  l.nt = plain && !l.eq_outer && sw.lb_nt && l.pipe;
  return p;
}

static inline double msm_ref_adds(size_t rows, size_t n, uint32_t num_bits) {
  size_t lg = n <= 1 ? 0 : 64 - (size_t)__builtin_clzll((unsigned long long)(n - 1));
  const size_t cw = n < 32 ? 3 : lg * 69 / 100 + 2, W = (num_bits + cw - 1) / cw;
  return (double)rows * ((double)n * W + (double)W * 2.0 * (double)((size_t)1 << cw) + (double)(W > 0 ? W - 1 : 0) * (cw + 1.0));
}
static inline size_t msm_chunks(size_t rows, size_t n_cols, uint32_t W) {
  size_t pairs = n_cols * W, K = 1;
  if (rows < 256) { K = 256 / rows; size_t kmax = (pairs + 1023) / 1024; if (kmax < 1) kmax = 1; if (K > kmax) K = kmax; }
  size_t cols_per_chunk = (n_cols + K - 1) / K;
  return (n_cols + cols_per_chunk - 1) / cols_per_chunk;
}
static inline size_t msm_direct_wgs(long parsed) { return (size_t)(parsed >= 1 && parsed <= 4096 ? parsed : 256); }
static inline size_t bullet_wgs(long parsed) { return (size_t)(parsed >= 4 && parsed <= 4096 ? parsed : 256); }
static inline size_t msm_direct_chunks(size_t rows, size_t n_cols, uint32_t* items_per_chunk, size_t wgs, size_t windows = MSM_WINDOWS) {
  const size_t total = n_cols * windows;
  size_t K = wgs / rows; if (K < 1) K = 1;
  size_t ipc = ((total + K - 1) / K + 255) / 256 * 256;
  const size_t ipc_max = windows * 128;
  if (ipc > ipc_max) ipc = ipc_max;
  *items_per_chunk = (uint32_t)ipc;
  return (total + ipc - 1) / ipc;
}
static inline size_t msm_pts_bytes(size_t rows, size_t n_cols, size_t wgs) {
  uint32_t ipc; const size_t kd = rows <= MSM_SMALL_ROWS ? msm_direct_chunks(rows, n_cols, &ipc, wgs) : 0, kb = msm_chunks(rows, n_cols, MSM_WINDOWS);
  return (rows * (kd > kb ? kd : kb) + 2 * rows + 4) * MSM_PT29_BYTES + 512;
}
struct MsmDirectPlan { bool w8; size_t windows, K; uint32_t ipc; double ref_adds, adds; };
static inline MsmDirectPlan msm_direct_plan(size_t rows, size_t n_cols, bool mult8, long wgs_parsed) {
  MsmDirectPlan p = {}; p.w8 = mult8; p.windows = msm_direct_windows(mult8 ? 8 : 4);
  p.K = msm_direct_chunks(rows, n_cols, &p.ipc, msm_direct_wgs(wgs_parsed), p.windows);
  p.ref_adds = msm_ref_adds(rows, n_cols, FR_MODULUS_BITS); p.adds = (double)rows * n_cols * p.windows;
  return p;
}
struct BulletPlan { bool w8; size_t windows, n_loc, K; uint32_t ipc; };
static inline BulletPlan bullet_plan(size_t n, size_t nk, uint32_t world, bool mult8, long wgs_parsed) {
  BulletPlan p = {}; p.w8 = mult8; p.windows = msm_direct_windows(mult8 ? 8 : 4);
  p.n_loc = n / world; const size_t cols = (nk / 2 >= world) ? p.n_loc / 2 : p.n_loc;
  const size_t total = cols * p.windows, kmax = (bullet_wgs(wgs_parsed) - 2) / 2;
  size_t ipc = (total + kmax - 1) / kmax; ipc = (ipc + p.windows - 1) / p.windows * p.windows; if (ipc < 256) ipc = 256; if (ipc > p.windows * 128) ipc = p.windows * 128;
  p.ipc = (uint32_t)ipc; p.K = (total + ipc - 1) / ipc;
  return p;
}

struct MsmSwitches { bool direct, rows8, rows8w, full8, pip; size_t rows8w_waves, pip_min_cols, pip_scratch_mb; long direct_wgs; };
struct MsmShape { uint32_t bps, W; size_t rows, n_cols; bool compressed, dev_rows; };
struct MsmHave { size_t n; bool mult, mult8, tab8, pip_scratch; };
enum MsmKernel { MSM_K_DIRECT, MSM_K_ROWS8W, MSM_K_ROWS8, MSM_K_PIP, MSM_K_FULL8, MSM_K_BUCKETS };
enum MsmResult {
  MSM_R_FLAG,
  MSM_R_COMPRESSED_MAPPED,
  MSM_R_COMPRESSED_MEMCPY,
  MSM_R_DEVICE_ROWS,
  MSM_R_MEMCPY
};
struct MsmPlan {
  MsmKernel kernel; MsmResult result;
  size_t K, cols_per_chunk; uint32_t W8;
  size_t rpw, waves;
  size_t pip_items, pip_row_bytes, pip_group;
  double ref_adds, adds;
};
static inline MsmPlan msm_plan(const MsmShape& s, const MsmHave& have, const MsmSwitches& sw) {
  MsmPlan p = {};
  const bool comp = s.compressed || s.dev_rows, small = s.rows <= MSM_SMALL_ROWS && !comp;
  p.result = s.dev_rows ? MSM_R_DEVICE_ROWS : s.compressed ? (s.rows <= ((size_t)1 << 16) ? MSM_R_COMPRESSED_MAPPED : MSM_R_COMPRESSED_MEMCPY) : small ? MSM_R_FLAG : MSM_R_MEMCPY;
  if (s.bps == 32 && small && have.mult && sw.direct) { p.kernel = MSM_K_DIRECT; return p; }
  p.K = msm_chunks(s.rows, s.n_cols, s.W); p.cols_per_chunk = (s.n_cols + p.K - 1) / p.K; p.W8 = (s.W + 1) / 2;
  p.rpw = sw.rows8w_waves ? (s.rows + sw.rows8w_waves - 1) / sw.rows8w_waves : 1; p.waves = (s.rows + p.rpw - 1) / p.rpw;
  const bool tab8 = s.bps == 4 && s.W <= 4 && s.rows >= 32 && sw.rows8 && have.tab8;
  const bool full8 = s.bps == 32 && have.mult8 && sw.full8 && !tab8;
  if (s.bps == 32 && sw.pip && !full8 && p.K == 1 && s.rows >= 256 && s.n_cols >= sw.pip_min_cols && s.n_cols < ((size_t)1 << 26) && have.n * MSM_WINDOWS < ((size_t)1 << 31) && have.pip_scratch) {
    p.pip_items = s.n_cols * MSM_PIP_WINDOWS;
    p.pip_row_bytes = ((p.pip_items * 4 + (MSM_PIP_BUCKETS + 1) * 4 + MSM_PIP_BUCKETS * 2 + (size_t)MSM_PIP_BUCKETS * MSM_PT29_BYTES + s.n_cols) + 255) & ~(size_t)255;
    p.pip_group = (sw.pip_scratch_mb << 20) / p.pip_row_bytes; if (p.pip_group < 64) p.pip_group = 64; if (p.pip_group > s.rows) p.pip_group = s.rows;
  }
  p.kernel = tab8 ? (sw.rows8w && p.K == 1 && s.rows >= 1024 && s.n_cols * p.W8 <= 8192 ? MSM_K_ROWS8W : MSM_K_ROWS8) : p.pip_group ? MSM_K_PIP : full8 ? MSM_K_FULL8 : MSM_K_BUCKETS;
// ... 5 lines not shown
```

### lasso_amd/csrc/poly_kernels.cuh

```cuda
#pragma once
#include <hip/hip_runtime.h>
#include "fr.cuh"
#include "fr29.cuh"
#include "handoff_device.cuh"
#include "launch_plan.cuh"

#ifndef LASSO_MAX_PTRS
#define LASSO_MAX_PTRS 136
#endif
#define LASSO_MAX_ALPHA 32

struct PtrTable { const fr_t* p[LASSO_MAX_PTRS]; };
struct MutPtrTable { fr_t* p[LASSO_MAX_PTRS]; };
struct PtrTable8 { const fr_t* p[8]; };
struct MutPtrTable8 { fr_t* p[8]; };
struct StrategyDev { int kind; uint32_t c, log_m, log_r, alpha; };
struct WeightTable { fr_t w[LASSO_MAX_ALPHA]; };

struct RedScratch { int32_t rows[LASSO_BLOCK * 27]; int64_t strips[8 * 27]; int64_t cols[27]; };
template <int NV>
__device__ __forceinline__ void block_columns(const fr29* vals, RedScratch& S) {
  const uint32_t t = threadIdx.x;
  __syncthreads();
#pragma unroll
// ... 230 lines not shown
  last_block_reduce(partials, g.nx, K, g.by, g.ny, counters, out, S, flag, seq);
}
#define CUBIC_ACCUMULATE(e, t0, t2, t3, cnt)                                                                                          \
  do {                                                                                                                                \
    e[0] = fr29_weak(fr29_add(e[0], t0)); e[1] = fr29_weak(fr29_add(e[1], t2)); e[2] = fr29_weak(fr29_add(e[2], t3));                    \
    if ((++cnt & 127u) == 0) { e[0] = fr29_mul(e[0], fr29_one_s()); e[1] = fr29_mul(e[1], fr29_one_s()); e[2] = fr29_mul(e[2], fr29_one_s()); } \
  } while (0)
__global__ void __launch_bounds__(LASSO_BLOCK) k_cubic_round_lb(PtrTable A, PtrTable B, uint32_t nx, uint32_t ny, const fr_t* __restrict__ C, size_t half, fr_t* __restrict__ partials, uint32_t* counters,
                                                                 fr_t* __restrict__ out, uint32_t* flag, uint32_t seq) {
  __shared__ RedScratch S;
  const CubicGrid g = cubic_grid(nx, ny);
  const fr_t* __restrict__ a = A.p[g.by];
  const fr_t* __restrict__ b = B.p[g.by];
  fr29 e[3] = {fr29_zero(), fr29_zero(), fr29_zero()}; uint32_t cnt = 0;
  for (size_t i = g.bx * (size_t)blockDim.x + threadIdx.x; i < half; i += (size_t)nx * blockDim.x) {
    fr29 t0, t2, t3;
    cubic_terms(fr29_unpack_u(a[i]), fr29_unpack_u(a[i + half]), fr29_unpack_u(b[i]), fr29_unpack_u(b[i + half]), fr29_unpack_u(C[i]), fr29_unpack_u(C[i + half]), t0, t2, t3);
    CUBIC_ACCUMULATE(e, t0, t2, t3, cnt);
  }
  cubic_epilogue(e, g, partials, counters, out, flag, seq, S, 10);
}
__device__ __forceinline__ fr29 bind29_semi(const fr_t& lo, const fr_t& hi, const fr29& rs) {
  const fr29 l = fr29_unpack_u(lo);
  return fr29_semi(fr29_add(l, fr29_mul(fr29_sub(fr29_unpack_u(hi), l), rs)));
}
__device__ __forceinline__ fr29 bind29(const fr_t& lo, const fr_t& hi, const fr29& rs) {
  const fr29 l = fr29_unpack_u(lo);
  return fr29_canonical(fr29_add(l, fr29_mul(fr29_sub(fr29_unpack_u(hi), l), rs)));
}

__device__ __forceinline__ void cubic_eqw_terms(const fr29& a0, const fr29& a1, const fr29& b0, const fr29& b1, const fr29& es, fr29& t0, fr29& t2, fr29& t3) {
  const fr29 g0 = fr29_mul(a0, es), g1 = fr29_mul(a1, es);
  t0 = fr29_mul(b0, g0);
  const fr29 dg = fr29_sub(g1, g0), db = fr29_sub(b1, b0);
  const fr29 g2 = fr29_weak(fr29_add(g1, dg)), b2 = fr29_weak(fr29_add(b1, db));
  t2 = fr29_mul(b2, g2);
  t3 = fr29_mul(fr29_add(b2, db), fr29_weak(fr29_add(g2, dg)));
}
__device__ __forceinline__ void cubic_eqw_terms2(const fr29& a0, const fr29& a1, const fr29& b0, const fr29& b1, const fr29& es, fr29& t0, fr29& tinf) {
  const fr29 g0 = fr29_mul(a0, es), g1 = fr29_mul(a1, es);
  t0 = fr29_mul(b0, g0);
  tinf = fr29_mul(fr29_sub(g1, g0), fr29_sub(b1, b0));
}
#define CUBIC_ACCUMULATE2(e, t0, t1, cnt)                                                                         \
  do {                                                                                                            \
    e[0] = fr29_weak(fr29_add(e[0], t0)); e[1] = fr29_weak(fr29_add(e[1], t1));                                     \
    if ((++cnt & 127u) == 0) { e[0] = fr29_mul(e[0], fr29_one_s()); e[1] = fr29_mul(e[1], fr29_one_s()); }          \
  } while (0)
struct EqInline { fr_t r[14]; fr_t scale; uint32_t ell; };
struct EqNone { uint32_t ell = 0; const uint32_t* gp = nullptr; uint32_t seq = 0; };
struct EqInlineTables { fr29 hi_s[128], lo_s[128], lo_u[128]; };
struct EqInlineMem { const uint32_t* gp; uint32_t seq; uint32_t ell; };
__device__ __forceinline__ fr_t eq_point_r(const EqInline& Q, uint32_t j) { return Q.r[j]; }
__device__ __forceinline__ fr_t eq_point_scale(const EqInline& Q) { return Q.scale; }
__device__ __forceinline__ bool eq_point_ok(const EqInline&) { return true; }
__device__ __forceinline__ fr_t eq_point_r(const EqInlineMem& Q, uint32_t j) { return gate_point_fr(Q.gp, j); }
__device__ __forceinline__ fr_t eq_point_scale(const EqInlineMem& Q) { return gate_point_fr(Q.gp, Q.ell); }
__device__ __forceinline__ bool eq_point_ok(const EqInlineMem& Q) { return gate_point_ok(Q.gp, Q.seq); }
template <class QT>
__device__ __forceinline__ bool eq_inline_build_t(const QT& Q, EqInlineTables& T) {
  if (!eq_point_ok(Q)) return false;
  const uint32_t t = threadIdx.x, lb = Q.ell / 2, hb = Q.ell - lb;
  const fr29 one_s = fr29_one_s();
  if (t < (1u << hb)) {
    fr29 p = fr29_unpack_s(eq_point_scale(Q));
    for (uint32_t j = 0; j < hb; j++) { const bool bit = (t >> (hb - 1 - j)) & 1u; const fr29 rs = fr29_unpack_s(eq_point_r(Q, j)); p = fr29_mul(bit ? rs : fr29_sub(one_s, rs), p); }
    T.hi_s[t] = p;
  } else if (t >= 128 && t - 128 < (1u << lb)) {
    const uint32_t x = t - 128;
    fr29 p = one_s;
    for (uint32_t j = 0; j < lb; j++) { const bool bit = (x >> (lb - 1 - j)) & 1u; const fr29 rs = fr29_unpack_s(eq_point_r(Q, hb + j)); p = fr29_mul(bit ? rs : fr29_sub(one_s, rs), p); }
    T.lo_s[x] = p;
    T.lo_u[x] = fr29_mul(p, fr29_unpack_u(fr_one()));
  }
  __syncthreads();
  return true;
}
__device__ __forceinline__ bool eq_inline_build(const EqInline& Q, EqInlineTables& T) { return eq_inline_build_t(Q, T); }
__device__ __forceinline__ bool eq_inline_build(const EqInlineMem& Q, EqInlineTables& T) { return eq_inline_build_t(Q, T); }
__device__ __forceinline__ fr29 eq_inline_s(const EqInlineTables& T, uint32_t lb, size_t x) { return fr29_mul(T.hi_s[x >> lb], T.lo_s[x & ((1u << lb) - 1u)]); }
struct EqGlobal { const fr_t* hi; const fr_t* lo; uint32_t lo_bits; uint32_t ell; const uint32_t* gp; uint32_t seq; };
__device__ __forceinline__ bool eq_inline_build(const EqGlobal& Q, EqInlineTables&) { return Q.gp == nullptr || gate_point_ok(Q.gp, Q.seq); }
__device__ __forceinline__ bool eq_inline_build(const EqNone&, EqInlineTables&) { return true; }
template <class TE> __device__ __forceinline__ bool eq_gate_ok(const TE&) { return true; }
template <> __device__ __forceinline__ bool eq_gate_ok<EqNone>(const EqNone& Q) { return Q.gp == nullptr || gate_point_ok(Q.gp, Q.seq); }
__device__ __forceinline__ fr29 eq_inline_value(const EqInline&, const EqInlineTables& T, uint32_t lb, size_t i, bool write, fr_t* __restrict__ E_out) {
  if (write) E_out[i] = fr29_store(fr29_mul(T.hi_s[i >> lb], T.lo_u[i & ((1u << lb) - 1u)]));
  return eq_inline_s(T, lb, i);
}
__device__ __forceinline__ fr29 eq_inline_value(const EqInlineMem&, const EqInlineTables& T, uint32_t lb, size_t i, bool write, fr_t* __restrict__ E_out) {
  if (write) E_out[i] = fr29_store(fr29_mul(T.hi_s[i >> lb], T.lo_u[i & ((1u << lb) - 1u)]));
  return eq_inline_s(T, lb, i);
}
__device__ __forceinline__ fr29 eq_inline_value(const EqGlobal& Q, const EqInlineTables&, uint32_t, size_t i, bool write, fr_t* __restrict__ E_out) {
  const fr_t mem = fr29_store(fr29_mul(fr29_unpack_u(Q.hi[i >> Q.lo_bits]), fr29_unpack_s(Q.lo[i & (((size_t)1 << Q.lo_bits) - 1)])));
  if (write) E_out[i] = mem;
  return fr29_unpack_s(mem);
}
__device__ __forceinline__ fr29 eq_inline_value(const EqNone&, const EqInlineTables&, uint32_t, size_t, bool, fr_t* __restrict__) { return fr29_zero(); }
__device__ __forceinline__ fr_t fr_load_nt(const fr_t* p) {
  const lasso_u32x4* q = reinterpret_cast<const lasso_u32x4*>(p);
  const lasso_u32x4 x = __builtin_nontemporal_load(q), y = __builtin_nontemporal_load(q + 1);
  fr_t r; r.v[0] = x.x; r.v[1] = x.y; r.v[2] = x.z; r.v[3] = x.w; r.v[4] = y.x; r.v[5] = y.y; r.v[6] = y.z; r.v[7] = y.w; return r;
}
template <int NT, bool EQI = false, class TP = PtrTable, class TE = EqInline, bool NTL = false>
__global__ void __launch_bounds__(LASSO_BLOCK) k_cubic_eqw_lb(TP A, TP B, uint32_t nx, uint32_t ny, const fr_t* __restrict__ E, size_t half, fr_t* __restrict__ partials, uint32_t* counters,
                                                               fr_t* __restrict__ out, uint32_t* flag, uint32_t seq, uint32_t pipeline, TE EQ = TE(), fr_t* __restrict__ E_out = nullptr) {
  __shared__ RedScratch S;
  __shared__ EqInlineTables ET;
  const CubicGrid g = cubic_grid(nx, ny);
  const uint32_t elb = EQ.ell / 2;
  if constexpr (EQI) { if (!eq_inline_build(EQ, ET)) return; } else { if (!eq_gate_ok(EQ)) return; }
  const fr_t* __restrict__ a = A.p[g.by];
  const fr_t* __restrict__ b = B.p[g.by];
  fr29 e[3] = {fr29_zero(), fr29_zero(), fr29_zero()}; uint32_t cnt = 0;
  fr29_acc w0 = fr29_acc_zero(), w1 = fr29_acc_zero();
  const size_t stride = (size_t)nx * blockDim.x;
  size_t i = g.bx * (size_t)blockDim.x + threadIdx.x;
  if (NT == 3) {
    for (; i < half; i += stride) {
      fr29 t0, t2, t3;
      cubic_eqw_terms(fr29_unpack_u(a[i]), fr29_unpack_u(a[i + half]), fr29_unpack_u(b[i]), fr29_unpack_u(b[i + half]), fr29_unpack_s(E[i]), t0, t2, t3); CUBIC_ACCUMULATE(e, t0, t2, t3, cnt);
    }
  } else if (!pipeline) {
    for (; i < half; i += stride) {
      const fr29 es = fr29_unpack_s(E[i]), b0 = fr29_unpack_u(b[i]), b1 = fr29_unpack_u(b[i + half]);
      const fr29 g0 = fr29_mul(fr29_unpack_u(a[i]), es), g1 = fr29_mul(fr29_unpack_u(a[i + half]), es);
      fr29_mul_acc(w0, b0, g0); fr29_mul_acc(w1, fr29_sub(g1, g0), fr29_sub(b1, b0));
      if (++cnt == 3) { fr29_acc_carry(w0); fr29_acc_carry(w1); cnt = 0; }
    }
  } else if (i < half) {
#define LB_LD(ptr) (NTL ? fr_load_nt(ptr) : *(ptr))
    fr_t a0 = LB_LD(a + i), a1 = LB_LD(a + i + half), b0m = LB_LD(b + i), b1m = LB_LD(b + i + half), em = EQI ? fr_zero() : E[i];
    for (;;) {
      const size_t in = i + stride; const bool more = in < half;
      const size_t ip = more ? in : i;
      const fr_t na0 = LB_LD(a + ip), na1 = LB_LD(a + ip + half), nb0 = LB_LD(b + ip), nb1 = LB_LD(b + ip + half), ne = EQI ? fr_zero() : E[ip];
#undef LB_LD
      fr29 es;
      if (EQI) es = eq_inline_value(EQ, ET, elb, i, g.by == 0, E_out);
      else es = fr29_unpack_s(em);
      const fr29 b0 = fr29_unpack_u(b0m), b1 = fr29_unpack_u(b1m);
      const fr29 g0 = fr29_mul(fr29_unpack_u(a0), es), g1 = fr29_mul(fr29_unpack_u(a1), es);
      fr29_mul_acc(w0, b0, g0); fr29_mul_acc(w1, fr29_sub(g1, g0), fr29_sub(b1, b0));
      if (++cnt == 3) { fr29_acc_carry(w0); fr29_acc_carry(w1); cnt = 0; }
      if (!more) break;
      a0 = na0; a1 = na1; b0m = nb0; b1m = nb1; em = ne; i = in;
    }
  }
  if (NT == 2) { fr29_acc_carry(w0); fr29_acc_carry(w1); e[0] = fr29_acc_reduce(w0); e[1] = fr29_acc_reduce(w1); }
  cubic_epilogue(e, g, partials, counters, out, flag, seq, S, 5, NT);
}
template <int NT, bool WIDE = false, class TM = MutPtrTable, bool AHEAD = false>
#ifdef LASSO_FUSED_WAVES
__attribute__((amdgpu_waves_per_eu(LASSO_FUSED_WAVES, LASSO_FUSED_WAVES)))
#endif
__global__ void __launch_bounds__(LASSO_BLOCK) k_cubic_eqw_fused(TM A, TM B, uint32_t nx, uint32_t ny, const fr_t* __restrict__ E, size_t q, fr_t r,
                                                                  fr_t* __restrict__ partials, uint32_t* counters, fr_t* __restrict__ out, uint32_t* flag, uint32_t seq,
                                                                  const uint32_t* gmail = nullptr, const uint32_t* mail = nullptr) {
  __shared__ RedScratch S;
  const CubicGrid g = cubic_grid(nx, ny);
  fr_t* __restrict__ a = A.p[g.by];
  fr_t* __restrict__ b = B.p[g.by];
  if constexpr (AHEAD) {
    __shared__ uint32_t s_mail[17];
    if (mail) {
      if (!ahead_challenge(mail, const_cast<uint32_t*>(gmail), seq, r, s_mail)) return;
    } else {
      if (!gated_challenge(gmail, seq, 8, s_mail)) return;
#pragma unroll
      for (int k = 0; k < 8; k++) r.v[k] = s_mail[k];
    }
  }
  const fr29 rs = fr29_unpack_s(r);
  fr29 e[3] = {fr29_zero(), fr29_zero(), fr29_zero()}; uint32_t cnt = 0;
  fr29_acc w0 = fr29_acc_zero(), w1 = fr29_acc_zero();
  for (size_t i = g.bx * (size_t)blockDim.x + threadIdx.x; i < q; i += (size_t)nx * blockDim.x) {
    const fr29 a0 = NT == 2 ? bind29_semi(a[i], a[i + 2 * q], rs) : bind29(a[i], a[i + 2 * q], rs), a1 = NT == 2 ? bind29_semi(a[i + q], a[i + 3 * q], rs) : bind29(a[i + q], a[i + 3 * q], rs);
    a[i] = fr29_pack(a0); a[i + q] = fr29_pack(a1);
    const fr29 b0 = NT == 2 ? bind29_semi(b[i], b[i + 2 * q], rs) : bind29(b[i], b[i + 2 * q], rs), b1 = NT == 2 ? bind29_semi(b[i + q], b[i + 3 * q], rs) : bind29(b[i + q], b[i + 3 * q], rs);
    b[i] = fr29_pack(b0); b[i + q] = fr29_pack(b1);
    fr29 t0, t2, t3;
    if (NT == 3) { cubic_eqw_terms(a0, a1, b0, b1, fr29_unpack_s(E[i]), t0, t2, t3); CUBIC_ACCUMULATE(e, t0, t2, t3, cnt); }
    else if (!WIDE) { cubic_eqw_terms2(a0, a1, b0, b1, fr29_unpack_s(E[i]), t0, t2); CUBIC_ACCUMULATE2(e, t0, t2, cnt); }
    else {
      const fr29 es = fr29_unpack_s(E[i]);
      const fr29 g0 = fr29_mul(a0, es), g1 = fr29_mul(a1, es);
      fr29_mul_acc(w0, b0, g0); fr29_mul_acc(w1, fr29_sub(g1, g0), fr29_sub(b1, b0));
      if (++cnt == 3) { fr29_acc_carry(w0); fr29_acc_carry(w1); cnt = 0; }
    }
  }
  if (WIDE && NT == 2) { fr29_acc_carry(w0); fr29_acc_carry(w1); e[0] = fr29_acc_reduce(w0); e[1] = fr29_acc_reduce(w1); }
  cubic_epilogue(e, g, partials, counters, out, flag, seq, S, 5, NT);
}
template <bool BIND, int NT, class TM = MutPtrTable>
__global__ void __launch_bounds__(LASSO_BLOCK) k_cubic_eqw_small(TM A, TM B, const fr_t* __restrict__ E, uint32_t q, fr_t r, uint32_t* counters, fr_t* __restrict__ out,
                                                                  uint32_t* flag, uint32_t seq) {
  __shared__ fr29 bound[2][128];
  __shared__ fr29 ge[128];
  __shared__ int32_t rows[192 * 9];
  __shared__ int64_t cols[27];
  const uint32_t t = threadIdx.x, y = blockIdx.x, m = 2 * q;
  const fr29 rs = fr29_unpack_s(r);
  for (uint32_t item = t; item < 2 * m; item += LASSO_BLOCK) {
    const uint32_t p = item / m, i = item - p * m;
    fr_t* dst = p == 0 ? A.p[y] : B.p[y];
    fr29 v;
    if (BIND) { v = bind29(dst[i], dst[i + m], rs); dst[i] = fr29_pack(v); } else v = fr29_unpack_u(dst[i]);
    bound[p][i] = v;
  }
  __syncthreads();
  if (t < m) ge[t] = fr29_mul(bound[0][t], fr29_unpack_s(E[t < q ? t : t - q]));
  __syncthreads();
  const uint32_t x = t >> 6, i = t & 63;
  if (x < NT) {
    fr29 term = fr29_zero();
    if (i < q) {
      const fr29 g0 = ge[i], g1 = ge[i + q], b0 = bound[1][i], b1 = bound[1][i + q];
      if (x == 0) term = fr29_mul(b0, g0);
      else if (NT == 2) term = fr29_mul(fr29_sub(g1, g0), fr29_sub(b1, b0));
      else {
        const fr29 dg = fr29_sub(g1, g0), db = fr29_sub(b1, b0);
        const fr29 g2 = fr29_weak(fr29_add(g1, dg)), b2 = fr29_weak(fr29_add(b1, db));
        term = x == 1 ? fr29_mul(b2, g2) : fr29_mul(fr29_add(b2, db), fr29_weak(fr29_add(g2, dg)));
      }
    }
#pragma unroll
    for (int k = 0; k < 9; k++) rows[t * 9 + k] = term.v[k];
  }
  __syncthreads();
  if (t < 9 * NT) {
    const uint32_t v = t / 9, k = t - v * 9;
    int64_t sum = 0;
    for (uint32_t j = 0; j < 64; j++) sum += rows[(v * 64 + j) * 9 + k];
    cols[t] = sum;
  }
  __syncthreads();
  if (t < NT) {
    int64_t c[9];
#pragma unroll
    for (int k = 0; k < 9; k++) c[k] = cols[t * 9 + k];
    result_store(out, (size_t)y * NT + t, fr29_pack(fr29_reduce_columns(c, 5)), flag, seq);
  }
  row_done(gridDim.x, counters, flag, seq);
}

#ifdef TAIL_PHASE_CLOCK
__device__ uint64_t tail_phase_clock[16 * 8];
#define TAIL_STAMP(k) do { if (threadIdx.x == 0 && blockIdx.x == 0 && turn < 16) tail_phase_clock[turn * 8 + (k)] = wall_clock64(); } while (0)
#else
#define TAIL_STAMP(k) do { } while (0)
#endif
__device__ __forceinline__ void tail_sums_publish(const int32_t* rows, int64_t* strips, int64_t* cols, uint32_t h, int shift, fr_t* out, uint32_t y, uint32_t* flag, uint32_t seq0, uint32_t turn) {
  const uint32_t t = threadIdx.x;
  if (h > 16) {
    if (t < 8 * 18) {
      const uint32_t col = t % 18, strip = t / 18, v = col / 9, k = col - v * 9;
      const uint32_t per = (h + 7) / 8, i0 = strip * per, i1 = i0 + per < h ? i0 + per : h;
      int64_t sum = 0;
      for (uint32_t i = i0; i < i1; i++) sum += rows[(v * h + i) * 9 + k];
      strips[strip * 18 + col] = sum;
    }
    __syncthreads();
    if (t < 18) { int64_t sum = 0; for (int g = 0; g < 8; g++) sum += strips[g * 18 + t]; cols[t] = sum; }
  } else if (t < 18) {
    const uint32_t v = t / 9, k = t - v * 9;
    int64_t sum = 0;
    for (uint32_t i = 0; i < h; i++) sum += rows[(v * h + i) * 9 + k];
    cols[t] = sum;
  }
  __syncthreads();
  TAIL_STAMP(2);
  if (t < 2) {
    int64_t c[9];
#pragma unroll
// ... 496 lines not shown
    fr29 g = fr29_zero();
    for (uint32_t t = 0; t < nt; t++) {
      const uint32_t b = __builtin_amdgcn_readfirstlane(L.term_start[t]), e = __builtin_amdgcn_readfirstlane(L.term_start[t + 1]);
      fr29 term;
      if (b == e) term = L.coeff[t];
      else {
        term = fr29_unpack_u(polys.p[__builtin_amdgcn_readfirstlane(L.term_mem[b])][i]);
        if (!(__builtin_amdgcn_readfirstlane(L.flags[t]) & 2u)) term = fr29_mul(term, L.coeff[t]);
        for (uint32_t j = b + 1; j < e; j++) term = fr29_mul(fr29_unpack_s(polys.p[__builtin_amdgcn_readfirstlane(L.term_mem[j])][i]), term);
      }
      g = fr29_weak(fr29_add(g, term));
      if ((t & 3u) == 3u) g = fr29_mul(g, fr29_one_s());
    }
    acc_add(acc[0], fr29_mul(g, fr29_unpack_u(eq[i])), cnt);
  }
  store_block_partials<1>(acc, 1, partials + blockIdx.x, 5, R);
}
template <int A>
__global__ void __launch_bounds__(LASSO_BLOCK) k_combine_claim(StrategyDev S, PtrTable polys, const fr_t* __restrict__ eq, WeightTable W, size_t n, fr_t* __restrict__ partials) {
  __shared__ RedScratch R;
  __shared__ fr29 ws[LASSO_MAX_ALPHA];
  load_weights(S, W, ws);
  const bool lt = S.kind == 3, prod = S.kind == 5;
  fr29 acc[1] = {fr29_zero()}; uint32_t cnt = 0;
  for (size_t i = blockIdx.x * (size_t)blockDim.x + threadIdx.x; i < n; i += (size_t)gridDim.x * blockDim.x) {
    fr29 g;
    if (prod) {
      g = fr29_unpack_s(polys.p[S.c - 1][i]);
      for (uint32_t m = S.c - 1; m-- > 0;) g = fr29_mul(fr29_unpack_s(polys.p[m][i]), g);
    } else if (lt) {
      g = fr29_unpack_s(polys.p[2 * (S.c - 1)][i]);
      for (uint32_t m = S.c - 1; m-- > 0;) g = fr29_weak(fr29_add(fr29_unpack_s(polys.p[2 * m][i]), fr29_mul(fr29_unpack_s(polys.p[2 * m + 1][i]), g)));
    } else g = weighted_sum(polys, i, S.alpha, ws);
    acc_add(acc[0], fr29_mul(g, fr29_unpack_u(eq[i])), cnt);
  }
  store_block_partials<1>(acc, 1, partials + blockIdx.x, (lt || prod) ? 0 : 5, R);
}

__global__ void __launch_bounds__(LASSO_BLOCK) k_multi_dot(PtrTable polys, uint32_t nx, uint32_t ny, const fr_t* __restrict__ w, size_t n, fr_t* __restrict__ partials) {
  __shared__ RedScratch R;
  const CubicGrid g = cubic_grid(nx, ny);
  const fr_t* __restrict__ z = polys.p[g.by];
  fr29_acc wa = fr29_acc_zero(); uint32_t cnt = 0;
  for (size_t i = g.bx * (size_t)blockDim.x + threadIdx.x; i < n; i += (size_t)nx * blockDim.x) {
    fr29_mul_acc(wa, fr29_unpack_u(z[i]), fr29_unpack_s(w[i]));
    if (++cnt == 3) { fr29_acc_carry(wa); cnt = 0; }
  }
  fr29_acc_carry(wa);
  fr29 acc[1] = {fr29_acc_reduce(wa)};
  store_block_partials<1>(acc, 1, partials + (size_t)g.by * nx + g.bx, 0, R);
}

struct RTable { fr_t r[32]; };
__global__ void k_eq_small(RTable R, uint32_t ell, fr_t scale, fr_t* __restrict__ out) {
  size_t x = blockIdx.x * (size_t)blockDim.x + threadIdx.x;
  if (x >= ((size_t)1 << ell)) return;
  fr29 p = fr29_unpack_u(scale);
  const fr29 one_s = fr29_one_s();
  for (uint32_t j = 0; j < ell; j++) { const bool bit = (x >> (ell - 1 - j)) & 1; const fr29 rs = fr29_unpack_s(R.r[j]); p = fr29_mul(bit ? rs : fr29_sub(one_s, rs), p); }
  out[x] = fr29_store(p);
}
struct RTable16 { fr_t r[16]; };
__global__ void k_eq_small2(RTable16 Rh, uint32_t hi_bits, fr_t scale, fr_t* __restrict__ hi, uint32_t hi_blocks, RTable16 Rl, uint32_t lo_bits, fr_t* __restrict__ lo) {
  const bool is_lo = blockIdx.x >= hi_blocks;
  const uint32_t ell = is_lo ? lo_bits : hi_bits;
  const size_t x = (blockIdx.x - (is_lo ? hi_blocks : 0u)) * (size_t)blockDim.x + threadIdx.x;
  if (x >= ((size_t)1 << ell)) return;
  fr29 p = is_lo ? fr29_unpack_u(fr_one()) : fr29_unpack_u(scale);
  const fr29 one_s = fr29_one_s();
  if (is_lo) { for (uint32_t j = 0; j < ell; j++) { const bool bit = (x >> (ell - 1 - j)) & 1; const fr29 rs = fr29_unpack_s(Rl.r[j]); p = fr29_mul(bit ? rs : fr29_sub(one_s, rs), p); } lo[x] = fr29_store(p); }
  else { for (uint32_t j = 0; j < ell; j++) { const bool bit = (x >> (ell - 1 - j)) & 1; const fr29 rs = fr29_unpack_s(Rh.r[j]); p = fr29_mul(bit ? rs : fr29_sub(one_s, rs), p); } hi[x] = fr29_store(p); }
}
__global__ void k_eq_small2_mem(const uint32_t* __restrict__ gp, uint32_t seq, uint32_t hi_bits, fr_t* __restrict__ hi, uint32_t hi_blocks, uint32_t lo_bits, fr_t* __restrict__ lo) {
  if (!gate_point_ok(gp, seq)) return;
  const bool is_lo = blockIdx.x >= hi_blocks;
  const uint32_t ell = is_lo ? lo_bits : hi_bits, j0 = is_lo ? hi_bits : 0u;
  const size_t x = (blockIdx.x - (is_lo ? hi_blocks : 0u)) * (size_t)blockDim.x + threadIdx.x;
  if (x >= ((size_t)1 << ell)) return;
  fr29 p = is_lo ? fr29_unpack_u(fr_one()) : fr29_unpack_u(gate_point_fr(gp, hi_bits + lo_bits));
  const fr29 one_s = fr29_one_s();
  for (uint32_t j = 0; j < ell; j++) { const bool bit = (x >> (ell - 1 - j)) & 1; const fr29 rs = fr29_unpack_s(gate_point_fr(gp, j0 + j)); p = fr29_mul(bit ? rs : fr29_sub(one_s, rs), p); }
  (is_lo ? lo : hi)[x] = fr29_store(p);
}
__global__ void __launch_bounds__(LASSO_BLOCK) k_eq_outer(const fr_t* __restrict__ hi, const fr_t* __restrict__ lo, uint32_t lo_bits, size_t n, fr_t* __restrict__ out, const uint32_t* __restrict__ gp = nullptr, uint32_t seq = 0) {
  if (gp != nullptr && !gate_point_ok(gp, seq)) return;
  const size_t mask = ((size_t)1 << lo_bits) - 1;
  for (size_t x = blockIdx.x * (size_t)blockDim.x + threadIdx.x; x < n; x += (size_t)gridDim.x * blockDim.x) out[x] = fr29_store(fr29_mul(fr29_unpack_u(hi[x >> lo_bits]), fr29_unpack_s(lo[x & mask])));
}

__global__ void __launch_bounds__(LASSO_BLOCK) k_gp_layer(const fr_t* __restrict__ in, size_t half, fr_t* __restrict__ out) {
  for (size_t i = blockIdx.x * (size_t)blockDim.x + threadIdx.x; i < half; i += (size_t)gridDim.x * blockDim.x) out[i] = fr29_store(fr29_mul(fr29_unpack_u(in[i]), fr29_unpack_s(in[i + half])));
}
__global__ void __launch_bounds__(LASSO_BLOCK) k_gp_layer2(const fr_t* __restrict__ in, size_t q, fr_t* __restrict__ o1, fr_t* __restrict__ o2) {
  for (size_t i = blockIdx.x * (size_t)blockDim.x + threadIdx.x; i < q; i += (size_t)gridDim.x * blockDim.x) {
    const fr_t a = fr29_store(fr29_mul(fr29_unpack_u(in[i]), fr29_unpack_s(in[i + 2 * q])));
    const fr_t b = fr29_store(fr29_mul(fr29_unpack_u(in[i + q]), fr29_unpack_s(in[i + 3 * q])));
    o1[i] = a; o1[i + q] = b;
    o2[i] = fr29_store(fr29_mul(fr29_unpack_u(a), fr29_unpack_s(b)));
  }
}
__global__ void k_gp_tail(fr_t* __restrict__ tree, size_t len) {
  fr_t* in = tree;
  while (len > 2) {
    size_t half = len / 2; fr_t* out = in + len;
    for (size_t i = threadIdx.x; i < half; i += blockDim.x) out[i] = fr29_store(fr29_mul(fr29_unpack_u(in[i]), fr29_unpack_s(in[i + half])));
    __threadfence_block();
    __syncthreads();
    in = out; len = half;
  }
}

__global__ void __launch_bounds__(LASSO_BLOCK) k_fingerprint_ops(const fr_t* __restrict__ table, const uint32_t* __restrict__ dim, const fr_t* __restrict__ read, size_t s,
                                                                  fr_t gamma, fr_t gamma2, fr_t tau, fr_t* __restrict__ out_r, fr_t* __restrict__ out_w) {
  const fr29 gs = fr29_unpack_s(gamma), g2s = fr29_unpack_s(gamma2), g2u = fr29_unpack_u(gamma2), tu = fr29_unpack_u(tau), r2s = fr29_r2s();
  for (size_t i = blockIdx.x * (size_t)blockDim.x + threadIdx.x; i < s; i += (size_t)gridDim.x * blockDim.x) {
    const uint32_t a = dim[i];
    fr29 h = fr29_add(fr29_mul(fr29_unpack_u(read[i]), g2s), fr29_mul(fr29_unpack_u(table[a]), gs));
    h = fr29_canonical(fr29_sub(fr29_add(h, fr29_mul(fr29_from_u64_int(a), r2s)), tu));
    out_r[i] = fr29_pack(h);
    out_w[i] = fr29_store(fr29_add(h, g2u));
  }
}
template <bool RU32>
__global__ void __launch_bounds__(LASSO_BLOCK) k_fingerprint_ops_l1(const fr_t* __restrict__ table, const uint32_t* __restrict__ dim, const void* __restrict__ read_any, size_t s,
                                                                     fr_t gamma, fr_t gamma2, fr_t tau, fr_t* __restrict__ out_r, fr_t* __restrict__ out_w, fr_t* __restrict__ l1_r, fr_t* __restrict__ l1_w,
                                                                     uint32_t store_leaves) {
  const fr29 gs = fr29_unpack_s(gamma), g2s = fr29_unpack_s(gamma2), g2u = fr29_unpack_u(gamma2), tu = fr29_unpack_u(tau), r2s = fr29_r2s();
  const fr29 g2r = fr29_mul(g2s, r2s);
  const fr_t* __restrict__ read = reinterpret_cast<const fr_t*>(read_any); const uint32_t* __restrict__ read32 = reinterpret_cast<const uint32_t*>(read_any);
  const size_t half = s / 2;
  for (size_t i = blockIdx.x * (size_t)blockDim.x + threadIdx.x; i < half; i += (size_t)gridDim.x * blockDim.x) {
    fr_t lr[2], lw[2];
#pragma unroll
    for (int e = 0; e < 2; e++) {
      const size_t k = i + e * half;
      const uint32_t a = dim[k];
      fr29 h = fr29_add(RU32 ? fr29_mul(fr29_from_u64_int(read32[k]), g2r) : fr29_mul(fr29_unpack_u(read[k]), g2s), fr29_mul(fr29_unpack_u(table[a]), gs));
      h = fr29_canonical(fr29_sub(fr29_add(h, fr29_mul(fr29_from_u64_int(a), r2s)), tu));
      lr[e] = fr29_pack(h); lw[e] = fr29_store(fr29_add(h, g2u));
      if (store_leaves) { out_r[k] = lr[e]; out_w[k] = lw[e]; }
    }
    l1_r[i] = fr29_store(fr29_mul(fr29_unpack_u(lr[0]), fr29_unpack_s(lr[1])));
    l1_w[i] = fr29_store(fr29_mul(fr29_unpack_u(lw[0]), fr29_unpack_s(lw[1])));
  }
}
template <bool RU32>
__global__ void __launch_bounds__(LASSO_BLOCK) k_fingerprint_ops_strips(const fr_t* __restrict__ table, const uint32_t* __restrict__ dim, const void* __restrict__ read_any, size_t s,
                                                                         fr_t gamma, fr_t gamma2, fr_t tau, uint32_t nstrips, size_t stride, size_t i0, size_t cs,
                                                                         fr_t* __restrict__ out_r, fr_t* __restrict__ out_w) {
  const fr29 gs = fr29_unpack_s(gamma), g2s = fr29_unpack_s(gamma2), g2u = fr29_unpack_u(gamma2), tu = fr29_unpack_u(tau), r2s = fr29_r2s();
  const fr29 g2r = fr29_mul(g2s, r2s);
  const fr_t* __restrict__ read = reinterpret_cast<const fr_t*>(read_any); const uint32_t* __restrict__ read32 = reinterpret_cast<const uint32_t*>(read_any);
  const size_t total = 2 * (size_t)nstrips * cs;
  for (size_t j = blockIdx.x * (size_t)blockDim.x + threadIdx.x; j < total; j += (size_t)gridDim.x * blockDim.x) {
    const size_t strip = j / cs, i = j - strip * cs, arr = strip / nstrips, t = strip - arr * nstrips;
    const size_t k = arr * (s / 2) + t * stride + i0 + i;
    const uint32_t a = dim[k];
    fr29 h = fr29_add(RU32 ? fr29_mul(fr29_from_u64_int(read32[k]), g2r) : fr29_mul(fr29_unpack_u(read[k]), g2s), fr29_mul(fr29_unpack_u(table[a]), gs));
    h = fr29_canonical(fr29_sub(fr29_add(h, fr29_mul(fr29_from_u64_int(a), r2s)), tu));
    out_r[j] = fr29_pack(h);
    out_w[j] = fr29_store(fr29_add(h, g2u));
  }
}
__global__ void __launch_bounds__(LASSO_BLOCK) k_fingerprint_mem(const fr_t* __restrict__ table, const fr_t* __restrict__ fin, size_t m, uint32_t world, uint32_t rank, fr_t gamma, fr_t gamma2, fr_t tau,
                                                                  fr_t* __restrict__ out_i, fr_t* __restrict__ out_f) {
  const fr29 gs = fr29_unpack_s(gamma), g2s = fr29_unpack_s(gamma2), tu = fr29_unpack_u(tau), r2s = fr29_r2s();
// ... 46 lines not shown
```

### lasso_amd/host/prover.hpp

```cpp
#pragma once
#include <array>
#include <functional>
#include <map>
#include <memory>
#include <string>
#include <vector>
#include "field_host.hpp"
#include "field52.hpp"
#include "switches.hpp"
#include "sumcheck_phase.hpp"
#include "hashes.hpp"
#include "../../include/lasso_prover.h"
#include "../../include/lasso_custom_check.h"

#include <chrono>
#include <cstdio>
#include <cstdlib>

namespace lasso {

struct Trace {
  static bool on() { return sw::trace() == 1; }
  static bool mem() { return sw::trace() == 3; }
  const char* name; lasso_ctx* ctx; std::chrono::steady_clock::time_point t0; static int& depth() { static thread_local int d = 0; return d; }
  uint64_t w0 = 0; double wus0 = 0; uint64_t live0 = 0;
  Trace(const char* n, lasso_ctx* c) : name(n), ctx(c) {
    if (on()) { t0 = std::chrono::steady_clock::now(); depth()++; if (ctx) lasso_wait_stats(ctx, &w0, &wus0, 0); }
    if (mem() && ctx) { uint64_t pk = 0; lasso_mem_stats(ctx, &live0, &pk, 1); depth()++; }
  }
  ~Trace() {
    if (mem() && ctx) {
      uint64_t live = 0, pk = 0; lasso_mem_stats(ctx, &live, &pk, 1); depth()--;
      fprintf(stderr, "[mem] %*s%s: live at entry %.2f GB, peak inside %.2f GB, live at exit %.2f GB\n", 2 * depth(), "", name, live0 / 1e9, pk / 1e9, live / 1e9);
    }
    if (!on()) return;
    if (ctx) lasso_sync(ctx);
    depth()--;
    double ms = std::chrono::duration<double, std::milli>(std::chrono::steady_clock::now() - t0).count();
    uint64_t w1 = 0; double wus1 = 0; if (ctx) lasso_wait_stats(ctx, &w1, &wus1, 0);
    fprintf(stderr, "[trace] %*s%s: time.busy=%.3fms (device hand-offs %llu, host spinning %.3fms)\n", 2 * depth(), "", name, ms, (unsigned long long)(w1 - w0), (wus1 - wus0) * 1e-3);
  }
};

struct HostClock {
  static bool on() { return sw::trace() == 2; }
  static std::map<std::string, double>& buckets() { static thread_local std::map<std::string, double> b; return b; }
  const char* name; std::chrono::steady_clock::time_point t0;
  explicit HostClock(const char* n) : name(n) { if (on()) t0 = std::chrono::steady_clock::now(); }
  ~HostClock() { if (on()) buckets()[name] += std::chrono::duration<double, std::milli>(std::chrono::steady_clock::now() - t0).count(); }
  static void dump() { if (!on()) return; for (auto& kv : buckets()) fprintf(stderr, "[host] %-28s %.3f ms\n", kv.first.c_str(), kv.second); buckets().clear(); }
};
struct Error : std::runtime_error { using std::runtime_error::runtime_error; };
#define LASSO_REQUIRE(c) do { if (!(c)) throw Error(std::string("lasso prover: requirement failed: ") + #c); } while (0)

#define LASSO_HOST_TOPS_MAX_PTRS 128
inline size_t next_pow2(size_t n) { size_t p = 1; while (p < n) p <<= 1; return p; }
inline bool is_pow2(size_t n) { return n && !(n & (n - 1)); }
inline size_t ceil_log2(size_t n) { size_t k = 0; while (((size_t)1 << k) < n) k++; return k; }

typedef int32_t (*lasso_allgather_fn)(void* user, const void* send, void* recv, size_t bytes);
struct Comm {
  size_t rank = 0, world = 1; lasso_allgather_fn fn = nullptr; void* user = nullptr;
  bool shared_device = false;
  bool sharded() const { return world > 1; }
  size_t log_world() const { size_t k = 0; while (((size_t)1 << k) < world) k++; return k; }
  void allgather(const void* send, void* recv, size_t bytes) const {
    if (world == 1) { memcpy(recv, send, bytes); return; }
    if (!fn || fn(user, send, recv, bytes) != 0) throw std::runtime_error("lasso prover: all-gather failed");
  }
  void sum(std::vector<lasso_fr>& v) const {
    if (world == 1 || v.empty()) return;
    std::vector<lasso_fr> all(v.size() * world);
    allgather(v.data(), all.data(), v.size() * sizeof(lasso_fr));
    for (size_t i = 0; i < v.size(); i++) { Sc acc = Sc::zero(); for (size_t g = 0; g < world; g++) acc += Sc::from_abi(all[g * v.size() + i]); v[i] = acc.abi(); }
  }
  Sc eq_low(const ScVec& point) const {
    const size_t p = log_world(); Sc f = Sc::one();
    for (size_t b = 0; b < p; b++) { const Sc& rv = point[point.size() - 1 - b]; f *= ((rank >> b) & 1) ? rv : (Sc::one() - rv); }
    return f;
  }
};

class Dev {
  mutable std::multimap<size_t, void*> pool_;
  mutable std::map<void*, size_t> live_;
  mutable size_t in_use_ = 0, in_use_peak_ = 0;
  int device_ = 0;
  mutable lasso_ctx* side_ = nullptr;

 public:
  lasso_ctx* ctx = nullptr;
  Comm comm;
// ... 478 lines not shown
  size_t s_loc, m_loc;
  std::vector<DBufU32> dim_u32;
  DBuf combined_l_variate_polys, combined_log_m_variate_polys;
  size_t nv_l, nv_m;
  bool compact = false;
  std::vector<DBufU32> read_u32; std::vector<uint32_t> read_max;
  const lasso_fr* dim(size_t i) const { LASSO_REQUIRE(!compact); return combined_l_variate_polys.p + i * s_loc; }
  const lasso_fr* read(size_t i) const { LASSO_REQUIRE(!compact); return combined_l_variate_polys.p + (C + i) * s_loc; }
  const uint32_t* block_u32(size_t b) const { return b < C ? dim_u32[b].p : read_u32[b - C].p; }
  uint32_t block_max(size_t b) const { return b < C ? (uint32_t)(m - 1) : read_max[b - C]; }
  void lift_block(size_t b, lasso_fr* d_tmp) const { dev->chk(lasso_fr_from_u32(dev->ctx, block_u32(b), s_loc, d_tmp), "lasso_fr_from_u32"); }
  const lasso_fr* final_(size_t i) const { return combined_log_m_variate_polys.p + i * m_loc; }

  static std::unique_ptr<DensifiedRepresentation> from_lookup_indices(const Dev& d, const uint64_t* indices, size_t n_lookups, size_t C, size_t log_m) {
    Trace tr_all("DensifiedRepresentation.from_lookup_indices", d.ctx);
    auto D = std::make_unique<DensifiedRepresentation>();
    D->dev = &d; D->C = C; D->s = next_pow2(n_lookups); D->log_m = log_m; D->m = (size_t)1 << log_m;
    const size_t s = D->s, m = D->m, P = d.comm.world;
    if (d.comm.sharded() && (s < 2 * P || m < 2 * P)) throw Error("slab sharding needs at least 2 lookups and 2 table entries per rank");
    D->s_loc = s / P; D->m_loc = m / P;
    size_t n_l = next_pow2(2 * C * s), n_m = next_pow2(C) * m;
    D->nv_l = ceil_log2(n_l); D->nv_m = ceil_log2(n_m);
    if (d.comm.sharded() && (((size_t)1 << (D->nv_m - D->nv_m / 2)) < P || ((size_t)1 << (D->nv_l - D->nv_l / 2)) < P)) throw Error("slab sharding needs every Hyrax matrix to have at least one column per rank");
    D->compact = d.capacity && sw::capacity_compact() && D->s_loc >= sw::leafless_min() && s >= ((size_t)1 << (D->nv_l - D->nv_l / 2));
    D->combined_log_m_variate_polys = DBuf(d, n_m / P);
    if (!D->compact) D->combined_l_variate_polys = DBuf(d, n_l / P);
    if (!D->compact && n_l > 2 * C * s) d.chk(lasso_zero(d.ctx, D->combined_l_variate_polys.p + 2 * C * D->s_loc, (n_l - 2 * C * s) / P * sizeof(lasso_fr)), "lasso_zero");
    if (n_m > C * m) d.chk(lasso_zero(d.ctx, D->combined_log_m_variate_polys.p + C * D->m_loc, (n_m - C * m) / P * sizeof(lasso_fr)), "lasso_zero");
    DBufU64 d_idx(d, indices, n_lookups * C);
    DBuf tmp_dim, tmp_read; if (D->compact) { tmp_dim = DBuf(d, D->s_loc); tmp_read = DBuf(d, D->s_loc); }
    for (size_t i = 0; i < C; i++) {
      DBufU32 d_access(d, D->s_loc);
      lasso_fr* dim_out = D->compact ? tmp_dim.p : D->combined_l_variate_polys.p + i * D->s_loc;
      lasso_fr* read_out = D->compact ? tmp_read.p : D->combined_l_variate_polys.p + (C + i) * D->s_loc;
      d.chk(lasso_densify_dim_slab(d.ctx, d_idx.p, n_lookups, C, i, s, (uint32_t)log_m, (uint32_t)P, (uint32_t)d.comm.rank, d_access.p, dim_out, read_out, D->combined_log_m_variate_polys.p + i * D->m_loc), "lasso_densify_dim");
      D->dim_u32.push_back(std::move(d_access));
      if (D->compact) {
        DBufU32 r32(d, D->s_loc); uint32_t mx = 0;
        d.chk(lasso_fr_to_u32(d.ctx, tmp_read.p, D->s_loc, r32.p, &mx), "lasso_fr_to_u32");
        D->read_u32.push_back(std::move(r32)); D->read_max.push_back(mx);
      }
    }
    if (D->compact) { tmp_dim.release(); tmp_read.release(); }
    if (d.capacity) (void)lasso_trim(d.ctx);
    return D;
  }
  SparsePolynomialCommitment commit(const SparsePolyCommitmentGens& gens) const {
    Trace tr_all("DensifiedRepresentation.commit", dev->ctx);
    SparsePolynomialCommitment c;
    if (!compact) c.l_variate_polys_commitment = hyrax_commit(*dev, combined_l_variate_polys.p, nv_l, gens.gens_combined_l_variate);
    else {
      const size_t L = (size_t)1 << (nv_l / 2), R = (size_t)1 << (nv_l - nv_l / 2), rows_per = s / R;
      PolyCommitment& pc = c.l_variate_polys_commitment; pc.rows = L; pc.compressed.reserve(32 * L);
      DBuf tmp(*dev, s_loc);
      for (size_t b = 0; b < 2 * C; b++) {
        PolyCommitment part;
        if (!dev->comm.sharded()) part = hyrax_commit_rows(*dev, nullptr, rows_per, R, gens.gens_combined_l_variate, block_u32(b), block_max(b));
        else { lift_block(b, tmp.p); part = hyrax_commit_rows(*dev, tmp.p, rows_per, R, gens.gens_combined_l_variate); }
        pc.compressed.insert(pc.compressed.end(), part.compressed.begin(), part.compressed.end());
      }
      if (2 * C * rows_per < L) {
        dev->chk(lasso_zero(dev->ctx, tmp.p, (R / dev->comm.world) * sizeof(lasso_fr)), "lasso_zero");
        PolyCommitment zero_row = hyrax_commit_rows(*dev, tmp.p, 1, R, gens.gens_combined_l_variate);
        for (size_t r = 2 * C * rows_per; r < L; r++) pc.compressed.insert(pc.compressed.end(), zero_row.compressed.begin(), zero_row.compressed.end());
      }
      tmp.release();
    }
    c.log_m_variate_polys_commitment = hyrax_commit(*dev, combined_log_m_variate_polys.p, nv_m, gens.gens_combined_log_m_variate);
    c.s = s; c.log_m = log_m; c.m = m; return c;
  }
};

class Prover {
  const Dev& d; const Strategy S; DensifiedRepresentation& dense; const SparsePolyCommitmentGens& gens; ProofTranscript& t; RandomTape& tape;
  size_t alpha, s, m, nv_derefs;
  size_t P, lgP, s_loc, m_loc;
  std::vector<DBuf> tables;
  DBuf combined_E;
  const lasso_fr* E(size_t i) const { return combined_E.p + i * s_loc; }
  std::vector<DBuf> tail_bufs;
  std::vector<DBuf> side_keep;
  static size_t tail_q() { static const size_t q = lasso_sumcheck_tail_capacity(); return q; }
  struct LazyEq { bool on = false; std::vector<lasso_fr> rr; lasso_fr scale; lasso_fr* d_table = nullptr; } lazy_eq;
  struct LayerAhead { bool on = false, tail = false; std::vector<lasso_fr*> A, B; lasso_fr* d_table = nullptr; size_t len = 0, m_stop = 1; uint32_t ell = 0; } layer_ahead;
  std::function<void()> next_layer_hook;
  void enqueue_next_layer(const std::vector<lasso_fr*>& trees, size_t n, size_t layer_id, lasso_fr* d_table) {
    layer_ahead.on = false;
    const size_t len = (n >> layer_id) / 2, off = 2 * n - 4 * len, k = trees.size(); const uint32_t ell = (uint32_t)ceil_log2(len / 2);
    if (!(P == 1 && !d.no_ahead() && sw::eq_inline() && sw::cubic_tail() && lasso_layer_ahead_ok(d.ctx) == 1) || len < 4) return;
    LayerAhead la; la.d_table = d_table; la.len = len; la.ell = ell; for (auto* tr : trees) { la.A.push_back(tr + off); la.B.push_back(tr + off + len); }
    int32_t rc;
    if (len / 2 <= tail_q()) {
      if (ell > 9) return;
      const size_t m0 = host_m_stop(k); la.m_stop = (m0 >= 2 && m0 < len) ? m0 : 1; la.tail = true;
      if (la.m_stop > 1) d.chk(lasso_tail_handover_next(d.ctx, (uint32_t)la.m_stop), "lasso_tail_handover_next");
      rc = lasso_sumcheck_cubic_tail_begin_eq_ahead(d.ctx, la.A.data(), la.B.data(), (uint32_t)k, len, ell);
    } else {
      if (ell > 32 || len / 2 <= 64) return;
      rc = lasso_sumcheck_cubic_eqw2_begin_eq_ahead(d.ctx, la.A.data(), la.B.data(), (uint32_t)k, d_table, len, ell);
    }
    if (rc == LASSO_ERR_UNSUPPORTED) return;
    d.chk(rc, "lasso_sumcheck_cubic_*_begin_eq_ahead");
    la.on = true; layer_ahead = std::move(la);
  }

 public:
  std::vector<uint8_t> proof_bytes;
  Prover(const Dev& d_, const Strategy& S_, DensifiedRepresentation& dense_, const SparsePolyCommitmentGens& gens_, ProofTranscript& t_, RandomTape& tape_)
      : d(d_), S(S_), dense(dense_), gens(gens_), t(t_), tape(tape_) {
    alpha = S.num_memories(); s = dense.s; m = dense.m; LASSO_REQUIRE(S.C() == dense.C && S.M() == dense.m);
    P = d.comm.world; lgP = d.comm.log_world(); s_loc = dense.s_loc; m_loc = dense.m_loc;
  }

  void eq_evals_local(const ScVec& point, lasso_fr* d_out) {
    LASSO_REQUIRE(point.size() >= lgP);
    std::vector<lasso_fr> rr; for (size_t i = 0; i + lgP < point.size(); i++) rr.push_back(point[i].abi());
    if (P == 1) { d.chk(lasso_eq_evals(d.ctx, rr.data(), (uint32_t)rr.size(), d_out), "lasso_eq_evals"); return; }
    lasso_fr sc = d.comm.eq_low(point).abi();
    d.chk(lasso_eq_evals_scaled(d.ctx, rr.data(), (uint32_t)rr.size(), &sc, d_out), "lasso_eq_evals_scaled");
  }
  LazyEq eq_half_spec(const ScVec& point, lasso_fr* d_out) {
    LASSO_REQUIRE(point.size() >= lgP);
    LazyEq z; if (point.size() == lgP) return z;
    for (size_t i = 1; i + lgP < point.size(); i++) z.rr.push_back(point[i].abi());
    Sc scale = Sc::one() - point[0]; if (P > 1) scale *= d.comm.eq_low(point);
    z.scale = scale.abi(); z.d_table = d_out; z.on = true; return z;
  }
  void eq_build(LazyEq& z) { if (z.on) { d.chk(lasso_eq_evals_scaled(d.ctx, z.rr.data(), (uint32_t)z.rr.size(), &z.scale, z.d_table), "lasso_eq_evals_scaled"); z.on = false; } }
  void eq_half_local(const ScVec& point, lasso_fr* d_out) { LazyEq z = eq_half_spec(point, d_out); eq_build(z); }
  void eq_half_lazy(const ScVec& point, lasso_fr* d_out) { lazy_eq = eq_half_spec(point, d_out); }
  std::vector<lasso_fr*> slab_tail(const std::vector<lasso_fr*>& polys, const ScVec& point = ScVec(), size_t local_rounds = 0, size_t num_rounds = 0, lasso_fr** d_eq = nullptr) {
    const size_t k = polys.size();
    std::vector<lasso_fr> mine(k), all(k * P), col(P);
    d.chk(lasso_read_heads(d.ctx, (const lasso_fr* const*)polys.data(), (uint32_t)k, mine.data()), "lasso_read_heads");
    d.comm.allgather(mine.data(), all.data(), k * sizeof(lasso_fr));
    std::vector<lasso_fr*> out;
    for (size_t i = 0; i < k; i++) {
      for (size_t g = 0; g < P; g++) col[g] = all[g * k + i];
      tail_bufs.emplace_back(d, P);
      d.chk(lasso_upload(d.ctx, tail_bufs.back().p, col.data(), P * sizeof(lasso_fr)), "lasso_upload");
      out.push_back(tail_bufs.back().p);
    }
    if (!d_eq) return out;
    tail_bufs.emplace_back(d, P); *d_eq = tail_bufs.back().p;
    std::vector<lasso_fr> rr; for (size_t i = local_rounds; i < num_rounds; i++) rr.push_back(point[i].abi());
    d.chk(lasso_eq_evals(d.ctx, rr.data(), (uint32_t)rr.size(), *d_eq), "lasso_eq_evals");
    return out;
  }

  struct PhaseState {
    bool in_tail = false;
    bool queued = false, queued_tail = false;
    void round_enqueued() { queued = true; }      void round_posted() { queued = false; }
    void tail_enqueued() { queued_tail = true; }  void tail_begun() { queued_tail = false; in_tail = true; }
    bool idle() const { return !queued && !queued_tail; }
  };
  Sc round_step(const UniPoly& up, SumcheckProof& proof, ScVec& r_out) {
    up.append_to_transcript(t, "poly");
    Sc r_j = t.challenge_scalar("challenge_nextround"); r_out.push_back(r_j);
    proof.compressed_polys.push_back(up.compress());
    return r_j;
  }
  const lasso_fr* degenerate_table(const EqPhase& ph, size_t j, bool reduce, const DBuf& tj) {
    std::vector<lasso_fr> rr; for (size_t t2 = ph.v0 + j + 1; t2 < ph.v0 + ph.rounds; t2++) rr.push_back(ph.point[t2].abi());
    lasso_fr sc = (reduce ? d.comm.eq_low(ph.point) : Sc::one()).abi();
    d.chk(lasso_eq_evals_scaled(d.ctx, rr.data(), (uint32_t)rr.size(), &sc, tj.p), "lasso_eq_evals_scaled");
    return tj.p;
  }
  bool rounds_ahead_ok(const EqPhase& ph, bool reduce, bool one_gpu) { return sw::rounds_ahead() && !ph.degenerate && (reduce ? (sw::slab_ahead() && !d.ranks_share_a_device()) : one_gpu) && !d.no_ahead() && lasso_rounds_ahead_ok(d.ctx) == 1; }

  void arbitrary_rounds(size_t rounds, size_t len, std::vector<lasso_fr*>& polys, size_t combined_degree, bool reduce, SumcheckProof& proof, ScVec& r_out, const std::vector<const uint32_t*>* first_u32 = nullptr) {
    std::vector<const lasso_fr*> cp(polys.begin(), polys.begin() + alpha);
    for (size_t round = 0; round < rounds; round++) {
      std::vector<lasso_fr> ev(combined_degree + 1);
      if (S.spark() || S.general()) d.chk(lasso_sumcheck_combine_round(d.ctx, S.abi_ptr(), cp.data(), polys[alpha], len, (uint32_t)combined_degree, ev.data()), "lasso_sumcheck_combine_round");
      else if (round == 0 && first_u32) d.chk(lasso_sumcheck_combine_round_lt_u32(d.ctx, &S.abi, first_u32->data(), polys[alpha], len, (uint32_t)combined_degree, ev.data()), "lasso_sumcheck_combine_round_lt_u32");
      else d.chk(lasso_sumcheck_combine_round_lt_scaled(d.ctx, &S.abi, cp.data(), polys[alpha], len, (uint32_t)combined_degree, ev.data()), "lasso_sumcheck_combine_round_lt_scaled");
      if (reduce) d.comm.sum(ev);
      ScVec evals; for (auto& e : ev) evals.push_back(Sc::from_abi(e));
      lasso_fr rj = round_step(UniPoly::from_evals(evals), proof, r_out).abi();
      d.chk(lasso_bind_top(d.ctx, polys.data(), (uint32_t)polys.size(), len, &rj), "lasso_bind_top");
      len /= 2;
    }
  }
// ... 138 lines not shown
      if (m.read32) { lifted = DBuf(d, L.n_loc); d.chk(lasso_fr_from_u32(d.ctx, m.read32, L.n_loc, lifted.p), "lasso_fr_from_u32"); }
      d.chk(lasso_fingerprint_ops(d.ctx, m.table, m.dim, m.read32 ? lifted.p : m.read, L.n_loc, &L.gamma, &L.tau, lr.p, lw.p), "lasso_fingerprint_ops");
      A.push_back(lr.p); B.push_back(lr.p + L.n_loc / 2); A.push_back(lw.p); B.push_back(lw.p + L.n_loc / 2);
      out.push_back(std::move(lr)); out.push_back(std::move(lw));
    }
    return out;
  }
  static size_t host_tail_budget() { return sw::host_tail(field52_ok()); }
  size_t host_m_stop(size_t k) const { return P != 1 ? 1 : lasso::host_m_stop(k, host_tail_budget()); }
  void host_cubic_rounds(std::vector<ScVec>& a, std::vector<ScVec>& b, size_t rounds_left, const ScVec& rand, size_t first, const ScVec& coeffs, const Sc& s_run, Sc& e, SumcheckProof& proof,
                         ScVec& r_out, std::vector<lasso_fr>& heads) {
    HostClock hc("host rounds (handed-over tails, tree tops)");
    const size_t k = a.size(); size_t m = (size_t)1 << rounds_left;
    LASSO_REQUIRE(k == b.size() && first + rounds_left <= rand.size());
    for (size_t c = 0; c < k; c++) LASSO_REQUIRE(a[c].size() == m && b[c].size() == m);
    auto to_sc = [](const H4& x) { Sc r; r.v = h4_to(x); return r; };
    std::vector<H4> C = eq_evals_host_scaled(rand.data() + first, rounds_left, s_run);
#ifdef LASSO_HOST_IFMA
    std::unique_ptr<HostRounds52> v52;
    bool w_nonzero = true; for (size_t c = 0; c < k; c++) if (coeffs[c].is_zero()) w_nonzero = false;
    if (field52_ok() && HostRounds52::fits(k, m) && w_nonzero) {
      std::vector<std::vector<H4>> ha(k, std::vector<H4>(m)), hb(k, std::vector<H4>(m)); std::vector<H4> w(k);
      for (size_t c = 0; c < k; c++) { w[c] = h4_from(coeffs[c].v); for (size_t i = 0; i < m; i++) { ha[c][i] = h4_from(a[c][i].v); hb[c][i] = h4_from(b[c][i].v); } }
      v52.reset(new HostRounds52(ha, hb, w, C));
    }
    const bool vec = v52 != nullptr;
#else
    const bool vec = false;
#endif
    std::vector<H4> A, B, Aw;
    if (!vec) {
      A.resize(k * m); B.resize(k * m); Aw.resize(k * m);
      for (size_t c = 0; c < k; c++) { const H4 w = h4_from(coeffs[c].v); for (size_t i = 0; i < m; i++) { A[c * m + i] = h4_from(a[c][i].v); B[c * m + i] = h4_from(b[c][i].v); Aw[c * m + i] = h4_mul(A[c * m + i], w); } }
    }
    size_t stride = m;
    for (size_t j = 0; j < rounds_left; j++) {
      const size_t h = m / 2;
      H4 e0 = h4_zero(), e2 = h4_zero(), e3 = h4_zero();
#ifdef LASSO_HOST_IFMA
      if (vec) v52->sums(h, e0, e2, e3); else
#endif
      for (size_t i = 0; i < h; i++) {
        H4 t0 = h4_zero(), t2 = h4_zero(), t3 = h4_zero();
        for (size_t c = 0; c < k; c++) {
          const H4 *pa = &Aw[c * stride], *pb = &B[c * stride];
          const H4 da = h4_sub(pa[i + h], pa[i]), db = h4_sub(pb[i + h], pb[i]), a2 = h4_add(pa[i + h], da), b2 = h4_add(pb[i + h], db), a3 = h4_add(a2, da), b3 = h4_add(b2, db);
          t0 = h4_add(t0, h4_mul(pa[i], pb[i])); t2 = h4_add(t2, h4_mul(a2, b2)); t3 = h4_add(t3, h4_mul(a3, b3));
        }
        const H4 dc = h4_sub(C[i + h], C[i]), c2 = h4_add(C[i + h], dc), c3 = h4_add(c2, dc);
        e0 = h4_add(e0, h4_mul(t0, C[i])); e2 = h4_add(e2, h4_mul(t2, c2)); e3 = h4_add(e3, h4_mul(t3, c3));
      }
      static const H4 inv2 = h4_from(Sc::from_u64(2).inverse().v), inv6 = h4_from(Sc::from_u64(6).inverse().v);
      const H4 e1 = h4_sub(h4_from(e.v), e0);
      const H4 t32 = h4_sub(e3, h4_add(h4_add(e2, e2), e2)), t11 = h4_add(h4_add(e1, e1), e1);
      const H4 k3 = h4_mul(h4_sub(h4_add(t32, t11), e0), inv6);
      const H4 k2 = h4_sub(h4_mul(h4_add(h4_sub(e2, h4_add(e1, e1)), e0), inv2), h4_add(h4_add(k3, k3), k3));
      const H4 k1 = h4_sub(h4_sub(h4_sub(e1, e0), k2), k3);
      UniPoly poly; poly.coeffs = {to_sc(e0), to_sc(k1), to_sc(k2), to_sc(k3)};
      const Sc r_j = round_step(poly, proof, r_out);
      e = poly.evaluate(r_j);
      const H4 rj = h4_from(r_j.v);
#ifdef LASSO_HOST_IFMA
      if (vec) v52->bind(h, rj); else
#endif
      {
        for (size_t c = 0; c < k; c++) for (H4* arr : {&A[c * stride], &B[c * stride], &Aw[c * stride]}) for (size_t i = 0; i < h; i++) arr[i] = h4_add(arr[i], h4_mul(rj, h4_sub(arr[i + h], arr[i])));
        for (size_t i = 0; i < h; i++) C[i] = h4_add(C[i], h4_mul(rj, h4_sub(C[i + h], C[i])));
      }
      m = h;
    }
    heads.resize(2 * k);
#ifdef LASSO_HOST_IFMA
    if (vec) { std::vector<H4> hh; v52->heads(hh); for (size_t c = 0; c < 2 * k; c++) heads[c] = to_sc(hh[c]).abi(); return; }
#endif
    for (size_t c = 0; c < k; c++) { heads[c] = to_sc(A[c * stride]).abi(); heads[k + c] = to_sc(B[c * stride]).abi(); }
  }
  void cubic_rounds(size_t rounds, size_t len, std::vector<lasso_fr*>& A, std::vector<lasso_fr*>& B, const lasso_fr* d_E, const ScVec& rand, size_t v0, const ScVec& coeffs, bool reduce, Sc& s_run,
                    Sc& e, SumcheckProof& proof, ScVec& r_out, std::vector<lasso_fr>* heads_out = nullptr, const LeafLayer* leaf = nullptr) {
    const size_t k = leaf ? 2 * leaf->mems.size() : A.size();
    if (heads_out) heads_out->clear();
    std::unique_ptr<HostClock> hpro(new HostClock("layer transition: sumcheck prologue"));
    LayerAhead pre = std::move(layer_ahead); layer_ahead.on = false;
    std::function<void()> hook = std::move(next_layer_hook); next_layer_hook = nullptr;
    if (!rounds) { if (pre.on) d.chk(lasso_point_cancel(d.ctx), "lasso_point_cancel"); return; }
    const EqPhase ph(rand, v0, rounds);
    DBuf tj; if (ph.degenerate) tj = DBuf(d, len / 2);
    Sc r_prev = Sc::zero();
    LazyEq lz; if (lazy_eq.on && lazy_eq.d_table == d_E && v0 == 0 && !ph.degenerate) { lz = lazy_eq; } lazy_eq.on = false;
    const size_t tail_from = lasso::tail_from(rounds, len, tail_q(), heads_out && !reduce && !ph.degenerate && sw::cubic_tail(), [&](size_t j0) { return ph.no_zero_from(j0); });
    const HostHandover ho = host_handover(rounds, len, tail_from, host_m_stop(k));
    bool use_pre = false;
    if (pre.on) {
      use_pre = lz.on && !ph.degenerate && !leaf && v0 == 0 && heads_out && !reduce && pre.len == len && pre.A == A && pre.B == B && pre.d_table == lz.d_table && pre.ell == lz.rr.size() &&
                (pre.tail ? (tail_from == 0 && ho.m_stop == pre.m_stop) : (tail_from > 0 && !sw::cubic_three_sums() && !rand[0].is_zero() && !s_run.is_zero()));
      if (!use_pre) d.chk(lasso_point_cancel(d.ctx), "lasso_point_cancel");
    }
    const bool ahead_ok = rounds_ahead_ok(ph, reduce, P == 1 && heads_out != nullptr);
    PhaseState st;
    std::vector<DBuf> leaf_full;
    if (leaf) {
      const bool plain = v0 == 0 && !ph.degenerate && !sw::cubic_three_sums() && rounds >= 3 && tail_from >= 2 && !rand[0].is_zero() && !rand[1].is_zero() && !s_run.is_zero();
      if (!plain) { leaf_full = leaf_materialise(*leaf, A, B); leaf = nullptr; }
    }
    enum class Tail { posted, with_eq, plain, ahead };
    auto begin_tail = [&](Tail form, const lasso_fr* table, const lasso_fr* rp) {
      if (form != Tail::posted && ho.m_stop > 1) d.chk(lasso_tail_handover_next(d.ctx, (uint32_t)ho.m_stop), "lasso_tail_handover_next");
      if (form == Tail::with_eq) { d.chk(lasso_sumcheck_cubic_tail_begin_eq(d.ctx, A.data(), B.data(), (uint32_t)k, len, lz.rr.data(), (uint32_t)lz.rr.size(), &lz.scale), "lasso_sumcheck_cubic_tail_begin_eq"); lz.on = false; }
      if (form == Tail::plain) d.chk(lasso_sumcheck_cubic_tail_begin(d.ctx, A.data(), B.data(), (uint32_t)k, table, len, rp), "lasso_sumcheck_cubic_tail_begin");
      if (form == Tail::ahead) d.chk(lasso_sumcheck_cubic_tail_begin_ahead(d.ctx, A.data(), B.data(), (uint32_t)k, table, len), "lasso_sumcheck_cubic_tail_begin_ahead");
      if (form == Tail::ahead) st.tail_enqueued(); else st.tail_begun();
      if (hook) { hook(); hook = nullptr; }
    };
    auto launch = [&](size_t j, const lasso_fr* table, const lasso_fr* rp, std::vector<lasso_fr>& ev) {
      const uint32_t ell = (uint32_t)lz.rr.size();
      const lasso_fr* rp0 = j == 0 ? nullptr : rp;
      if (st.queued) { d.chk(lasso_challenge_post(d.ctx, rp), "lasso_challenge_post"); st.round_posted(); }
      else if (st.queued_tail) { d.chk(lasso_sumcheck_cubic_tail_next(d.ctx, rp), "lasso_sumcheck_cubic_tail_next"); st.tail_begun(); }
      else if (j == 0 && use_pre) {
        { HostClock hp("layer transition: point post"); d.chk(lasso_point_post(d.ctx, lz.rr.data(), ell, &lz.scale), "lasso_point_post"); } lz.on = false;
        if (pre.tail) begin_tail(Tail::posted, nullptr, nullptr);
      } else if (leaf && j < 2) {
        eq_build(lz);
        leaf_round(*leaf, j, len, table, rp0, ev);
        if (j == 1) { A = leaf->work_a; B = leaf->work_b; }
        return true;
      } else if (j == 0 && lz.on && j < tail_from && ell <= 32 && len / 2 > 64) {
        d.chk(lasso_sumcheck_cubic_eqw2_begin_eq(d.ctx, A.data(), B.data(), (uint32_t)k, lz.d_table, len, lz.rr.data(), ell, &lz.scale), "lasso_sumcheck_cubic_eqw2_begin_eq"); lz.on = false;
      } else if (j == 0 && lz.on && j >= tail_from && ell <= 9) begin_tail(Tail::with_eq, nullptr, nullptr);
      else {
        eq_build(lz);
        if (j < tail_from) d.chk(lasso_sumcheck_cubic_eqw2_begin(d.ctx, A.data(), B.data(), (uint32_t)k, table, len, rp0), "lasso_sumcheck_cubic_eqw2_begin");
        else if (!st.in_tail) begin_tail(Tail::plain, table, rp0);
        else d.chk(lasso_sumcheck_cubic_tail_next(d.ctx, rp), "lasso_sumcheck_cubic_tail_next");
      }
      return false;
    };
    hpro.reset();
    for (size_t j = 0; j < ho.j_host; j++) {
      const lasso_fr* table = ph.degenerate ? degenerate_table(ph, j, reduce, tj) : d_E;
      const Sc base = ph.base(j, s_run), f0 = ph.f0(j, base), f1 = ph.f1(j, base);
      const lasso_fr rp = r_prev.abi();
      UniPoly poly;
      if (j >= tail_from || st.queued || (!f1.is_zero() && !sw::cubic_three_sums())) {
        std::vector<lasso_fr> ev(2 * k);
        const bool have_ev = launch(j, table, &rp, ev);
        if (j) len /= 2;
        if (ahead_ok && !st.in_tail && !lz.on && j + 1 < ho.j_host && !(leaf && j + 1 < 3) && !rand[v0 + j + 1].is_zero()) {
          if (j + 1 < tail_from) {
            const int32_t rc = lasso_sumcheck_cubic_eqw2_begin_ahead(d.ctx, A.data(), B.data(), (uint32_t)k, table, len);
            if (rc == 0) st.round_enqueued(); else if (rc != LASSO_ERR_UNSUPPORTED) d.chk(rc, "lasso_sumcheck_cubic_eqw2_begin_ahead");
          } else if (j + 1 == tail_from) begin_tail(Tail::ahead, table, nullptr);
        }
        const Sc f1_inv = f1.is_zero() ? Sc::zero() : f1.inverse();
        if (!have_ev) d.chk(lasso_result_wait(d.ctx, ev.data(), 2 * k), "lasso_result_wait");
        if (reduce) d.comm.sum(ev);
        HostClock hc("cubic round host work");
        Sc q0 = Sc::zero(), qi = Sc::zero();
        for (size_t i = 0; i < k; i++) { q0 += Sc::from_abi(ev[2 * i]) * coeffs[i]; qi += Sc::from_abi(ev[2 * i + 1]) * coeffs[i]; }
        const Sc c0 = f0 * q0, q1 = (e - c0) * f1_inv, ql = q1 - q0 - qi, df = f1 - f0;
        poly.coeffs = {c0, f0 * ql + df * q0, f0 * qi + df * ql, df * qi};
      } else {
        std::vector<lasso_fr> ev(3 * k);
        eq_build(lz);
        if (j == 0) d.chk(lasso_sumcheck_cubic_eqw_round(d.ctx, (const lasso_fr* const*)A.data(), (const lasso_fr* const*)B.data(), (uint32_t)k, table, len, ev.data()), "lasso_sumcheck_cubic_eqw_round");
        else { d.chk(lasso_sumcheck_cubic_eqw_round_fused(d.ctx, A.data(), B.data(), (uint32_t)k, table, len, &rp, ev.data()), "lasso_sumcheck_cubic_eqw_round_fused"); len /= 2; }
        if (reduce) d.comm.sum(ev);
        Sc c0 = Sc::zero(), c2 = Sc::zero(), c3 = Sc::zero();
        for (size_t i = 0; i < k; i++) { c0 += Sc::from_abi(ev[3 * i]) * coeffs[i]; c2 += Sc::from_abi(ev[3 * i + 1]) * coeffs[i]; c3 += Sc::from_abi(ev[3 * i + 2]) * coeffs[i]; }
        c0 *= f0; c2 *= ph.f2(j, base); c3 *= ph.f3(j, base);
        poly = UniPoly::from_evals({c0, e - c0, c2, c3});
      }
      HostClock hc2("cubic round host work");
      r_prev = round_step(poly, proof, r_out);
      e = poly.evaluate(r_prev);
      ph.advance(s_run, j, r_prev);
    }
    lasso_fr rp = r_prev.abi();
    if (st.in_tail) {
      d.chk(lasso_sumcheck_cubic_tail_next(d.ctx, &rp), "lasso_sumcheck_cubic_tail_next");
      heads_out->resize(2 * k * ho.m_stop);
      d.chk(lasso_result_wait(d.ctx, heads_out->data(), 2 * k * ho.m_stop), "lasso_result_wait");
      if (ho.m_stop > 1) {
        std::vector<ScVec> ha(k, ScVec(ho.m_stop)), hb(k, ScVec(ho.m_stop));
        for (size_t c = 0; c < k; c++) for (size_t i = 0; i < ho.m_stop; i++) { ha[c][i] = Sc::from_abi((*heads_out)[c * ho.m_stop + i]); hb[c][i] = Sc::from_abi((*heads_out)[(k + c) * ho.m_stop + i]); }
        host_cubic_rounds(ha, hb, rounds - ho.j_host, rand, v0 + ho.j_host, coeffs, s_run, e, proof, r_out, *heads_out);
      }
      return;
    }
    LASSO_REQUIRE(ho.j_host == rounds && st.idle());
    std::vector<lasso_fr*> ab(A); ab.insert(ab.end(), B.begin(), B.end());
    d.chk(lasso_bind_top(d.ctx, ab.data(), (uint32_t)ab.size(), len, &rp), "lasso_bind_top");
  }
  SumcheckProof prove_cubic_batched(const Sc& claim, size_t num_rounds, bool slab, std::vector<lasso_fr*>& A, std::vector<lasso_fr*>& B, const lasso_fr* d_E, const ScVec& rand, const ScVec& coeffs,
                                    ScVec& r_out, ScVec& claims_a, ScVec& claims_b, const LeafLayer* leaf = nullptr) {
    SumcheckProof proof; Sc e = claim, s_run = Sc::one(); const size_t k = leaf ? 2 * leaf->mems.size() : A.size();
    LASSO_REQUIRE(rand.size() == num_rounds);
    std::vector<lasso_fr*> fa(A), fb(B);
    std::vector<lasso_fr> heads;
    if (!slab) {
      cubic_rounds(num_rounds, (size_t)1 << num_rounds, fa, fb, d_E, rand, 0, coeffs, false, s_run, e, proof, r_out, &heads, leaf);
    } else {
      LASSO_REQUIRE(num_rounds >= lgP);
      const size_t local_rounds = num_rounds - lgP;
      cubic_rounds(local_rounds, (size_t)1 << local_rounds, fa, fb, d_E, rand, 0, coeffs, true, s_run, e, proof, r_out, nullptr, leaf);
      std::vector<lasso_fr*> local_heads(fa); local_heads.insert(local_heads.end(), fb.begin(), fb.end());
      if (sw::slab_host_tail()) {
        std::vector<lasso_fr> mine(2 * k), all(2 * k * P);
        d.chk(lasso_read_heads(d.ctx, (const lasso_fr* const*)local_heads.data(), (uint32_t)(2 * k), mine.data()), "lasso_read_heads");
        d.comm.allgather(mine.data(), all.data(), 2 * k * sizeof(lasso_fr));
// ... 600 lines not shown
```

### lasso_amd/host/switches.hpp

```cpp
#pragma once
#include <cstdlib>

namespace lasso { namespace sw {
inline bool unless0(const char* e) { return !(e && e[0] == '0'); }
inline bool if1(const char* e) { return e && e[0] == '1'; }
#define LASSO_SWITCH(type, name, value) inline type name() { static const type v = (value); return v; }
LASSO_SWITCH(int, trace, [] { const char* e = getenv("LASSO_TRACE"); return e && e[0] >= '1' && e[0] <= '3' ? e[0] - '0' : 0; }())
LASSO_SWITCH(bool, capacity, if1(getenv("LASSO_CAPACITY")))
LASSO_SWITCH(bool, capacity_compact, unless0(getenv("LASSO_CAPACITY_COMPACT")))
LASSO_SWITCH(size_t, leafless_min, [] { const char* e = getenv("LASSO_LEAFLESS_MIN"); const size_t x = e ? (size_t)atoll(e) : ((size_t)1 << 16); return x < 64 ? (size_t)64 : x; }())
LASSO_SWITCH(bool, throughput_ahead, if1(getenv("LASSO_THROUGHPUT_AHEAD")))
LASSO_SWITCH(bool, side_stream, unless0(getenv("LASSO_SIDE_STREAM")))
LASSO_SWITCH(bool, slab_open, unless0(getenv("LASSO_SLAB_OPEN")))
LASSO_SWITCH(bool, eq_inline, unless0(getenv("LASSO_EQ_INLINE")))
LASSO_SWITCH(bool, cubic_tail, unless0(getenv("LASSO_CUBIC_TAIL")))
LASSO_SWITCH(bool, linear_tail, unless0(getenv("LASSO_LINEAR_TAIL")))
LASSO_SWITCH(bool, rounds_ahead, unless0(getenv("LASSO_ROUNDS_AHEAD")))
LASSO_SWITCH(bool, slab_ahead, unless0(getenv("LASSO_SLAB_AHEAD")))
LASSO_SWITCH(bool, cubic_three_sums, if1(getenv("LASSO_CUBIC_THREE_SUMS")))
LASSO_SWITCH(bool, slab_host_tail, unless0(getenv("LASSO_SLAB_HOST_TAIL")))
LASSO_SWITCH(bool, slab_host_tops, unless0(getenv("LASSO_SLAB_HOST_TOPS")))
LASSO_SWITCH(bool, sumcheck_u32, unless0(getenv("LASSO_SUMCHECK_U32")))
LASSO_SWITCH(bool, host_ifma, unless0(getenv("LASSO_HOST_IFMA")))
inline size_t host_tail(bool ifma) { static const size_t v = [&] { const char* e = getenv("LASSO_HOST_TAIL"); const long x = e ? atol(e) : (ifma ? 128 : 32); return (size_t)(x < 0 ? 0 : x > 1024 ? 1024 : x); }(); return v; }
LASSO_SWITCH(bool, verify_device_points, unless0(getenv("LASSO_VERIFY_DEVICE_POINTS")))
LASSO_SWITCH(size_t, wire_device_min, [] { const char* e = getenv("LASSO_WIRE_DEVICE_MIN"); const long long x = e ? atoll(e) : 376; return (size_t)(x < 1 ? 1 : x); }())
LASSO_SWITCH(bool, verify_msm_points, unless0(getenv("LASSO_VERIFY_MSM_POINTS")))
inline bool slab_rccl() { return unless0(getenv("LASSO_SLAB_RCCL")); }
inline bool debug_cubic_host() { return if1(getenv("LASSO_DEBUG_CUBIC_HOST")); }
#undef LASSO_SWITCH
} }
```

Measured before the change: 1.118 billion.

## Store large-layer eq tables as hi/lo factors plus small dense prefix

For layers with eq tables above 2^14 entries, the eq table is no longer built as a full 2^ell dense array. It is kept as two half-size factor tables (hi and lo) plus a dense prefix for the late rounds. The cubic sumcheck kernels read eq values as the product hi[x>>lb]*lo[x&mask] through a new EqHi accessor. This is meant to cut the memory written to build the table and read during the early rounds, at the cost of one extra field multiply per element and more complex planning and refusal rules. The feature is on by default through a switch and is enabled for the layer-ahead and lazy-eq paths on single-device runs.

```diff
diff --git a/include/lasso_hip_eq.h b/include/lasso_hip_eq.h
--- /dev/null
+++ b/include/lasso_hip_eq.h
@@ -0,0 +1,14 @@
+#ifndef LASSO_HIP_EQ_H
+#define LASSO_HIP_EQ_H
+#include "lasso_hip.h"
+#ifdef __cplusplus
+extern "C" {
+#endif
+
+int32_t lasso_eq_factors_use(lasso_ctx* ctx, lasso_fr* d_E, uint32_t ell, uint32_t ncirc);
+int32_t lasso_eq_factors_drop(lasso_ctx* ctx);
+
+#ifdef __cplusplus
+}
+#endif
+#endif
diff --git a/lasso_amd/build.py b/lasso_amd/build.py
--- a/lasso_amd/build.py
+++ b/lasso_amd/build.py
@@ -26,7 +26,7 @@
     suffix, flags = CURVES[curve]
     csrc = os.path.join(HERE, "csrc")
     target = os.path.join(HERE, f"liblasso_hip{suffix}.so")
-    sources = _glob(csrc, (".hip", ".cuh")) + [os.path.join(ROOT, "include", f) for f in ("lasso_hip.h", "lasso_hip_wire.h", "lasso_hip_msm.h", "lasso_custom_check.h")]
+    sources = _glob(csrc, (".hip", ".cuh")) + [os.path.join(ROOT, "include", f) for f in ("lasso_hip.h", "lasso_hip_wire.h", "lasso_hip_msm.h", "lasso_hip_eq.h", "lasso_custom_check.h")]
     if force or _stale(target, sources):
         extra = os.environ.get("LASSO_EXTRA_HIPCC_FLAGS", "").split()
         cmd = [HIPCC, f"--offload-arch={ARCH}", "-O3", "-std=c++17", "-fPIC", "-shared", "-Wno-unused-result", *flags, *extra,
@@ -54,7 +54,7 @@
     suffix, flags = CURVES[curve]
     hdir = os.path.join(HERE, "host")
     target = os.path.join(HERE, f"liblasso_prover{suffix}.so")
-    sources = _glob(hdir, (".cpp", ".hpp")) + _glob(os.path.join(HERE, "csrc"), (".cuh",)) + [os.path.join(ROOT, "include", f) for f in ("lasso_hip.h", "lasso_hip_wire.h", "lasso_hip_msm.h", "lasso_prover.h", "lasso_custom_check.h")]
+    sources = _glob(hdir, (".cpp", ".hpp")) + _glob(os.path.join(HERE, "csrc"), (".cuh",)) + [os.path.join(ROOT, "include", f) for f in ("lasso_hip.h", "lasso_hip_wire.h", "lasso_hip_msm.h", "lasso_hip_eq.h", "lasso_prover.h", "lasso_custom_check.h")]
     if not os.path.exists(os.path.join(hdir, "prover_capi.cpp")):
         return None
     dev = build_device(force=False, verbose=verbose, curve=curve)
diff --git a/lasso_amd/csrc/device_switches.cuh b/lasso_amd/csrc/device_switches.cuh
--- a/lasso_amd/csrc/device_switches.cuh
+++ b/lasso_amd/csrc/device_switches.cuh
@@ -14,6 +14,7 @@
 LASSO_DSWITCH(bool, cubic_wide, unless0(getenv("LASSO_CUBIC_WIDE")))
 LASSO_DSWITCH(unsigned, direct_nx, [] { const char* e = getenv("LASSO_DIRECT_NX"); const long x = e ? atol(e) : 16; return (unsigned)(x < 0 ? 0 : x > 64 ? 64 : x); }())
 LASSO_DSWITCH(bool, eq_inline_big, if1(getenv("LASSO_EQ_INLINE_BIG")))
+LASSO_DSWITCH(bool, eq_factors, unless0(getenv("LASSO_EQ_FACTORS")))
 LASSO_DSWITCH(bool, lb_pipeline, unless0(getenv("LASSO_LB_PIPELINE")))
 LASSO_DSWITCH(bool, lb_nt, if1(getenv("LASSO_LB_NT")))
 LASSO_DSWITCH(unsigned, ahead_inkernel_wgs, [] { const char* e = getenv("LASSO_AHEAD_INKERNEL_WGS"); const long x = e ? atol(e) : 32; return (unsigned)(x < 0 ? 0 : x > 4096 ? 4096 : x); }())
diff --git a/lasso_amd/csrc/lasso_hip.hip b/lasso_amd/csrc/lasso_hip.hip
--- a/lasso_amd/csrc/lasso_hip.hip
+++ b/lasso_amd/csrc/lasso_hip.hip
@@ -17,6 +17,7 @@
 #include "wire_kernels.cuh"
 #include "../../include/lasso_hip_msm.h"
 #include "msm_points_kernels.cuh"
+#include "../../include/lasso_hip_eq.h"
 
 __global__ void __launch_bounds__(256) k_inner_lr(const fr_t* __restrict__ a, const fr_t* __restrict__ b, size_t half, fr_t* __restrict__ partials) {
   __shared__ RedScratch S;
@@ -57,6 +58,7 @@
   uint32_t* d_counters = nullptr;
   uint32_t* d_gmail = nullptr;
   uint32_t* pmail_h = nullptr; uint32_t* pmail_d = nullptr; uint32_t* d_gpoint = nullptr;
+  const lasso_fr* eqc_buf = nullptr; uint32_t eqc_ell = 0;
   uint32_t prof_mask = 0;
   std::vector<EventPair> events; size_t events_used = 0;
   uint64_t prof_launches[LASSO_K_COUNT] = {0}; double prof_ms[LASSO_K_COUNT] = {0}; double prof_bytes[LASSO_K_COUNT] = {0};
@@ -422,7 +424,7 @@
   (void)hipGetLastError();
   if (c->pmail_h) memset(c->pmail_h, 0, LASSO_PMAIL_BYTES);
   mail_chunks(c->mail_h + 12, 0, zero8); post_mail(c, 0, zero8);
-  c->proto.reset(); c->events_used = 0;
+  c->proto.reset(); c->events_used = 0; c->eqc_buf = nullptr; c->eqc_ell = 0;
   HIPCHK(c, hipMemsetAsync(c->d_counters, 0, (LASSO_MAX_PTRS + 40) * 4, c->stream));
   HIPCHK(c, hipStreamSynchronize(c->stream));
   return 0;
@@ -575,16 +577,19 @@
 }
 extern "C++" {
 struct EqPointArg { const lasso_fr* point; uint32_t ell; fr_t scale; };
-static CubicPlan cubic_plan_for(lasso_ctx* c, uint32_t ncirc, size_t n, bool has_r, int NT, bool has_eqi, bool want_groups, bool ahead, const EqPointArg* eqg, int gate_ell) {
-  const CubicShape s = {n, ncirc, NT, ahead, has_r, has_eqi, eqg != nullptr, eqg ? eqg->ell : 0u, gate_ell, c->prof_mask, want_groups && c->tagged};
-  const CubicSwitches sw = {dsw::cubic_nx(), dsw::cubic_wide(), dsw::direct_nx(), dsw::eq_inline_big(), dsw::lb_pipeline(), dsw::lb_nt(), dsw::ahead_inkernel_wgs()};
+static uint32_t compact_ell_of(const lasso_ctx* c, const lasso_fr* d_E) { return c->eqc_buf && d_E == c->eqc_buf ? c->eqc_ell : 0u; }
+static CubicPlan cubic_plan_for(lasso_ctx* c, uint32_t ncirc, size_t n, bool has_r, int NT, bool has_eqi, bool want_groups, bool ahead, const EqPointArg* eqg, int gate_ell, uint32_t compact_ell) {
+  const CubicShape s = {n, ncirc, NT, ahead, has_r, has_eqi, eqg != nullptr, eqg ? eqg->ell : 0u, gate_ell, c->prof_mask, want_groups && c->tagged, compact_ell};
+  const CubicSwitches sw = {dsw::cubic_nx(), dsw::cubic_wide(), dsw::direct_nx(), dsw::eq_inline_big(), dsw::lb_pipeline(), dsw::lb_nt(), dsw::ahead_inkernel_wgs(), dsw::eq_factors()};
   return cubic_plan(s, sw);
 }
 template <class TM, class TP>
 static int32_t cubic_eqw_launch_t(lasso_ctx* c, lasso_fr* const* d_A, lasso_fr* const* d_B, uint32_t ncirc, const lasso_fr* d_E, size_t n, const lasso_fr* r, int NT, uint32_t* seq_out, const EqInline* eqi, uint32_t* groups_out, bool ahead = false, const EqPointArg* eqg = nullptr, int gate_ell = -1) {
   if (groups_out) *groups_out = 1;
-  const CubicPlan P = cubic_plan_for(c, ncirc, n, r != nullptr, NT, eqi != nullptr, groups_out != nullptr, ahead, eqg, gate_ell);
+  const CubicPlan P = cubic_plan_for(c, ncirc, n, r != nullptr, NT, eqi != nullptr, groups_out != nullptr, ahead, eqg, gate_ell, compact_ell_of(c, d_E));
   if (P.form == CUBIC_REFUSED) return fail(c, LASSO_ERR_UNSUPPORTED, P.refusal);
+  const EqCompactLayout CL = eq_compact_layout(c->eqc_ell);
+  EqHi H; if (P.eq_hi) { H.hi = (const fr_t*)d_E + CL.hi_off; H.lo = (const fr_t*)d_E + CL.lo_off; H.lo_bits = CL.lb; H.ell = c->eqc_ell; }
   TM A, B; for (uint32_t i = 0; i < ncirc; i++) { REQUIRE(c, d_A[i] && d_B[i]); A.p[i] = (fr_t*)d_A[i]; B.p[i] = (fr_t*)d_B[i]; }
   int32_t rc = ensure_small(c, (size_t)ncirc * 3); if (rc) return rc;
   const uint32_t seq = next_seq(c); *seq_out = seq;
@@ -609,7 +614,12 @@
     if (!ahead && (rc = reserve())) return rc;
     const uint32_t* const gmail = ahead ? (const uint32_t*)c->d_gmail : (const uint32_t*)nullptr; const uint32_t* const wait_mail = P.inkernel ? (const uint32_t*)c->mail_d : (const uint32_t*)nullptr;
 #define LAUNCH_CFUSED(NT_, WIDE_, AHEAD_) hipLaunchKernelGGL((k_cubic_eqw_fused<NT_, WIDE_, TM, AHEAD_>), dim3(nx * ny), dim3(LASSO_BLOCK), 0, c->stream, A, B, nx, ny, (const fr_t*)d_E, P.items, rr, (fr_t*)c->d_scratch, c->d_counters, r_out, r_flag, seq, gmail, wait_mail)
-    if (ahead) { if (P.wide) LAUNCH_CFUSED(2, true, true); else LAUNCH_CFUSED(2, false, true); }
+#define LAUNCH_CFUSED_HI(WIDE_, AHEAD_) hipLaunchKernelGGL((k_cubic_eqw_fused<2, WIDE_, TM, AHEAD_, EqHi>), dim3(nx * ny), dim3(LASSO_BLOCK), 0, c->stream, A, B, nx, ny, (const fr_t*)d_E, P.items, rr, (fr_t*)c->d_scratch, c->d_counters, r_out, r_flag, seq, gmail, wait_mail, H)
+    if (P.eq_hi) {
+      if (ahead) { if (P.wide) LAUNCH_CFUSED_HI(true, true); else LAUNCH_CFUSED_HI(false, true); }
+      else if (P.wide) LAUNCH_CFUSED_HI(true, false); else LAUNCH_CFUSED_HI(false, false);
+    }
+    else if (ahead) { if (P.wide) LAUNCH_CFUSED(2, true, true); else LAUNCH_CFUSED(2, false, true); }
     else if (NT == 3) LAUNCH_CFUSED(3, false, false);
     else if (P.wide) LAUNCH_CFUSED(2, true, false);
     else LAUNCH_CFUSED(2, false, false);
@@ -620,7 +630,17 @@
     fr_t* const f_hi = (fr_t*)c->d_scratch + P.part_elems; fr_t* const f_lo = f_hi + ((size_t)1 << L.g_hi);
     if (L.gate) { hipLaunchKernelGGL(k_gate_point, dim3(1), dim3(64), 0, c->stream, (const uint32_t*)c->pmail_d, c->d_gpoint, seq, (uint32_t)gate_ell + 2u, c->pmail_d + LASSO_PMAIL_ACK_WORD); c->proto.gate_sent = seq; }
     const uint32_t* const gate_gp = L.gate ? (const uint32_t*)c->d_gpoint : (const uint32_t*)nullptr;
-    if (L.factors) {
+    if (L.factors && L.eq == CUBIC_EQ_HI) {
+      ProfScope pe(c, LASSO_K_EQ, 32.0 * CL.elems);
+      const unsigned hb = grid_for((size_t)1 << CL.hb), lb2 = grid_for((size_t)1 << CL.lb), pb = grid_for(CL.pre);
+      fr_t* const base = (fr_t*)d_E;
+      if (L.factors_gated) { EqPointMem M; M.gp = c->d_gpoint; M.seq = seq; hipLaunchKernelGGL(k_eq_compact_mem, dim3(hb + lb2 + pb), dim3(LASSO_BLOCK), 0, c->stream, M, CL.hb, hb, CL.lb, lb2, CL.pre, base + CL.hi_off, base + CL.lo_off, base); }
+      else {
+        EqPointArgs Q; for (uint32_t j = 0; j < 16; j++) { Q.Rh.r[j] = j < CL.hb ? to_fr(eqg->point + j) : fr_zero(); Q.Rl.r[j] = j < CL.lb ? to_fr(eqg->point + CL.hb + j) : fr_zero(); }
+        Q.scale = eqg->scale; Q.hi_bits = CL.hb;
+        hipLaunchKernelGGL(k_eq_compact, dim3(hb + lb2 + pb), dim3(LASSO_BLOCK), 0, c->stream, Q, hb, CL.lb, lb2, CL.pre, base + CL.hi_off, base + CL.lo_off, base);
+      }
+    } else if (L.factors) {
       ProfScope pe(c, LASSO_K_EQ, L.eq_outer ? 32.0 * P.items : 32.0 * (((size_t)1 << L.g_hi) + ((size_t)1 << L.g_lo)));
       const unsigned hb = grid_for((size_t)1 << L.g_hi), lb2 = grid_for((size_t)1 << L.g_lo);
       if (L.factors_gated) hipLaunchKernelGGL(k_eq_small2_mem, dim3(hb + lb2), dim3(LASSO_BLOCK), 0, c->stream, (const uint32_t*)c->d_gpoint, seq, L.g_hi, f_hi, hb, L.g_lo, f_lo);
@@ -645,6 +665,7 @@
         EqGlobal G; G.hi = f_hi; G.lo = f_lo; G.lo_bits = L.g_lo; G.ell = L.g_ell; G.gp = L.gate ? c->d_gpoint : nullptr; G.seq = L.gate ? seq : 0;
         LAUNCH_CLB(2, true, EqGlobal, false, nullptr, G, d_E);
       } break;
+      case CUBIC_EQ_HI: { H.gp = gate_gp; H.seq = L.gate ? seq : 0; LAUNCH_CLB(2, false, EqHi, false, d_E, H, nullptr); } break;
     }
   }
   HIPCHK(c, hipGetLastError());
@@ -672,7 +693,7 @@
 }
 int32_t lasso_sumcheck_cubic_eqw2_begin_ahead(lasso_ctx* c, lasso_fr* const* d_A, lasso_fr* const* d_B, uint32_t ncirc, const lasso_fr* d_E, size_t n) {
   REQUIRE(c, d_A && d_B && d_E && ncirc >= 1 && ncirc <= LASSO_MAX_PTRS && n >= 4 && (n & (n - 1)) == 0 && !c->proto.ahead_active && !c->proto.tail_active && !c->proto.defer_next);
-  const CubicPlan P = cubic_plan_for(c, ncirc, n, false, 2, false, true, true, nullptr, -1);
+  const CubicPlan P = cubic_plan_for(c, ncirc, n, false, 2, false, true, true, nullptr, -1, compact_ell_of(c, d_E));
   if (P.form == CUBIC_REFUSED) return fail(c, LASSO_ERR_UNSUPPORTED, "lasso_sumcheck_cubic_eqw2_begin_ahead: streaming rounds only");
   { int32_t rc0 = ensure_small(c, (size_t)ncirc * 3 * (P.direct ? P.nx : 1)); if (rc0) return rc0; rc0 = ensure_scratch(c, P.scratch_elems * sizeof(fr_t)); if (rc0) return rc0; }
   uint32_t seq, groups; int32_t rc = cubic_eqw_launch(c, d_A, d_B, ncirc, d_E, n, nullptr, 2, &seq, nullptr, &groups, true); if (rc) return rc;
@@ -748,6 +769,14 @@
 }
 static bool gate_free(lasso_ctx* c) { return !c->proto.gate_sent || __atomic_load_n(c->pmail_h + LASSO_PMAIL_ACK_WORD, __ATOMIC_ACQUIRE) == c->proto.gate_sent; }
 int32_t lasso_layer_ahead_ok(lasso_ctx* c) { return c && dsw::layer_ahead() && c->pmail_d && c->d_gpoint ? 1 : 0; }
+int32_t lasso_eq_factors_use(lasso_ctx* c, lasso_fr* d_E, uint32_t ell, uint32_t ncirc) {
+  REQUIRE(c, d_E && ncirc >= 1 && ncirc <= LASSO_MAX_PTRS);
+  c->eqc_buf = nullptr; c->eqc_ell = 0;
+  if (!eq_compact_layer_ok(ell, ncirc, dsw::cubic_nx(), dsw::eq_factors())) return fail(c, LASSO_ERR_UNSUPPORTED, "lasso_eq_factors_use: this layer keeps its table (switched off, a table of at most 2^14 or more than 2^32 entries, or a round grid that cannot take the factor form)");
+  c->eqc_buf = d_E; c->eqc_ell = ell;
+  return 0;
+}
+int32_t lasso_eq_factors_drop(lasso_ctx* c) { REQUIRE(c, true); c->eqc_buf = nullptr; c->eqc_ell = 0; return 0; }
 int32_t lasso_sumcheck_cubic_eqw2_begin_eq_ahead(lasso_ctx* c, lasso_fr* const* d_A, lasso_fr* const* d_B, uint32_t ncirc, lasso_fr* d_E_out, size_t n, uint32_t ell) {
   REQUIRE(c, d_A && d_B && d_E_out && ncirc >= 1 && ncirc <= LASSO_MAX_PTRS && n >= 2 && (n & (n - 1)) == 0 && ell < 48 && ((size_t)1 << ell) == n / 2 && !c->proto.waiting_on_device() && !c->proto.defer_next);
   if (!lasso_layer_ahead_ok(c) || n / 2 <= CUBIC_SMALL_Q || ell > 32 || ell > LASSO_POINT_MAX) return fail(c, LASSO_ERR_UNSUPPORTED, "lasso_sumcheck_cubic_eqw2_begin_eq_ahead: tables of 2^7 .. 2^32 entries only");
diff --git a/lasso_amd/csrc/launch_plan.cuh b/lasso_amd/csrc/launch_plan.cuh
--- a/lasso_amd/csrc/launch_plan.cuh
+++ b/lasso_amd/csrc/launch_plan.cuh
@@ -28,15 +28,36 @@
 }
 static inline unsigned tail_threads(size_t q) { return q <= 256 ? 256u : 512u; }
 
-struct CubicSwitches { long cubic_nx; bool wide; unsigned direct_nx; bool eq_inline_big, lb_pipeline, lb_nt; unsigned ahead_inkernel_wgs; };
-struct CubicShape { size_t n; uint32_t ncirc; int NT; bool ahead, has_r, has_eqi, has_eqg; uint32_t eqg_ell; int gate_ell; uint32_t prof_mask; bool direct_ok; };
+struct CubicSwitches { long cubic_nx; bool wide; unsigned direct_nx; bool eq_inline_big, lb_pipeline, lb_nt; unsigned ahead_inkernel_wgs; bool eq_factors; };
+struct CubicShape { size_t n; uint32_t ncirc; int NT; bool ahead, has_r, has_eqi, has_eqg; uint32_t eqg_ell; int gate_ell; uint32_t prof_mask; bool direct_ok; uint32_t compact_ell; };
 enum CubicForm { CUBIC_REFUSED, CUBIC_SMALL, CUBIC_LB, CUBIC_FUSED };
 enum CubicEq {
   CUBIC_EQ_TABLE,
   CUBIC_EQ_LDS,
   CUBIC_EQ_GATED,
-  CUBIC_EQ_FACTORS
-};
+  CUBIC_EQ_FACTORS,
+  CUBIC_EQ_HI
+};
+#define EQ_COMPACT_PREFIX ((size_t)1 << 14)
+struct EqCompactLayout { uint32_t lb, hb; size_t pre, hi_off, lo_off, elems; };
+static inline EqCompactLayout eq_compact_layout(uint32_t ell) {
+  EqCompactLayout L; L.lb = ell / 2; L.hb = ell - L.lb;
+  L.pre = (size_t)1 << L.lb; if (L.pre < EQ_COMPACT_PREFIX) L.pre = EQ_COMPACT_PREFIX;
+  L.hi_off = L.pre; L.lo_off = L.hi_off + ((size_t)1 << L.hb); L.elems = L.lo_off + ((size_t)1 << L.lb);
+  return L;
+}
+static inline bool eq_hi_round_ok(size_t items, unsigned nx, uint32_t lb) {
+  const size_t stride = (size_t)nx * LASSO_BLOCK;
+  return items > ((size_t)1 << lb) && (stride >= items || (stride & (((size_t)1 << lb) - 1)) == 0);
+}
+static inline bool eq_compact_layer_ok(uint32_t ell, uint32_t ncirc, long cubic_nx, bool eq_factors) {
+  if (!eq_factors || ell <= 14 || ell > 32 || ncirc < 1) return false;
+  const EqCompactLayout L = eq_compact_layout(ell);
+  if (L.lb < 6 || L.elems > ((size_t)1 << ell)) return false;
+  for (size_t items = (size_t)1 << ell; items > ((size_t)1 << L.lb) && items > CUBIC_SMALL_Q; items >>= 1)
+    if (!eq_hi_round_ok(items, round_nx(items, ncirc, cubic_nx), L.lb)) return false;
+  return true;
+}
 struct CubicLbPlan {
   CubicEq eq;
   bool gate;
@@ -52,6 +73,7 @@
   bool bind;
   size_t items;
   unsigned nx, ny;
+  bool eq_hi;
   size_t part_elems;
   size_t scratch_elems;
   bool direct;
@@ -63,9 +85,16 @@
   CubicPlan p = {}; p.ny = s.ncirc; p.nx = 1;
   if (s.ahead && (s.NT != 2 || s.n / 4 <= CUBIC_SMALL_Q)) { p.form = CUBIC_REFUSED; p.refusal = "a round launched ahead of its challenge: two-sum streaming rounds only (more than 64 index quadruples per circuit)"; return p; }
   p.bind = s.has_r || s.ahead; p.items = p.bind ? s.n / 4 : s.n / 2;
+  const bool compact = sw.eq_factors && s.compact_ell > 0;
+  const EqCompactLayout cl = eq_compact_layout(compact ? s.compact_ell : 0);
+  if (compact && (p.items > ((size_t)1 << s.compact_ell) || (s.NT != 2 && p.items > cl.pre))) { p.form = CUBIC_REFUSED; p.refusal = "a compact eq buffer (lasso_eq_factors_use) serves the two-sum rounds of its own layer only"; return p; }
   if (p.items <= CUBIC_SMALL_Q) { p.form = CUBIC_SMALL; return p; }
   p.form = p.bind ? CUBIC_FUSED : CUBIC_LB;
   p.nx = round_nx(p.items, p.ny, sw.cubic_nx);
+  if (compact && p.items > cl.pre) {
+    if (!eq_hi_round_ok(p.items, p.nx, cl.lb) || (!p.bind && !(s.has_eqg || s.gate_ell > 14))) { p.form = CUBIC_REFUSED; p.refusal = "a compact eq buffer (lasso_eq_factors_use): this round's grid cannot take the factor form"; return p; }
+    p.eq_hi = true;
+  }
   p.part_elems = p.scratch_elems = (size_t)p.nx * p.ny * 3;
   p.direct = s.direct_ok && p.nx > 1 && p.nx <= sw.direct_nx;
   if (p.bind) {
@@ -79,6 +108,10 @@
   if (s.has_eqg || gbig) p.scratch_elems += ((size_t)1 << l.g_hi) + ((size_t)1 << l.g_lo);
   if (s.NT != 2) { l.eq = CUBIC_EQ_TABLE; l.pipe = 0; return p; }
   l.gate = gated; l.factors = gbig || s.has_eqg; l.factors_gated = gbig; l.eq_outer = l.factors && !sw.eq_inline_big;
+  if (compact) {
+    if (s.has_eqi || (gated && !gbig) || (l.factors && (l.g_ell != s.compact_ell || !p.eq_hi))) { p.form = CUBIC_REFUSED; p.refusal = "a compact eq buffer (lasso_eq_factors_use): round 0 of another shape than the one registered"; return p; }
+    if (l.factors) { l.eq_outer = false; l.eq = CUBIC_EQ_HI; l.pipe = 1u; l.nt = false; return p; }
+  }
   l.eq = l.eq_outer ? CUBIC_EQ_TABLE : gated ? (gbig ? CUBIC_EQ_FACTORS : CUBIC_EQ_GATED) : s.has_eqg ? CUBIC_EQ_FACTORS : s.has_eqi ? CUBIC_EQ_LDS : CUBIC_EQ_TABLE;
   const bool plain = l.eq == CUBIC_EQ_TABLE;
   l.pipe = plain ? (sw.lb_pipeline ? 1u : 0u) : 1u;
diff --git a/lasso_amd/csrc/poly_kernels.cuh b/lasso_amd/csrc/poly_kernels.cuh
--- a/lasso_amd/csrc/poly_kernels.cuh
+++ b/lasso_amd/csrc/poly_kernels.cuh
@@ -336,8 +336,21 @@
 struct EqGlobal { const fr_t* hi; const fr_t* lo; uint32_t lo_bits; uint32_t ell; const uint32_t* gp; uint32_t seq; };
 __device__ __forceinline__ bool eq_inline_build(const EqGlobal& Q, EqInlineTables&) { return Q.gp == nullptr || gate_point_ok(Q.gp, Q.seq); }
 __device__ __forceinline__ bool eq_inline_build(const EqNone&, EqInlineTables&) { return true; }
+struct EqHi { const fr_t* hi = nullptr; const fr_t* lo = nullptr; uint32_t lo_bits = 0; uint32_t ell = 0; const uint32_t* gp = nullptr; uint32_t seq = 0; };
+template <class TE> struct eq_is_hi { static constexpr bool value = false; };
+template <> struct eq_is_hi<EqHi> { static constexpr bool value = true; };
+template <class TE> __device__ __forceinline__ const fr_t* eq_entry(const TE&, const fr_t* __restrict__ E, size_t i) { return E + i; }
+template <> __device__ __forceinline__ const fr_t* eq_entry<EqHi>(const EqHi& Q, const fr_t* __restrict__, size_t i) { return Q.hi + __builtin_amdgcn_readfirstlane((uint32_t)(i >> Q.lo_bits)); }
+template <class TE> __device__ __forceinline__ fr_t eq_lo_load(const TE&, size_t) { return fr_zero(); }
+template <> __device__ __forceinline__ fr_t eq_lo_load<EqHi>(const EqHi& Q, size_t i0) { return Q.lo[i0 & (((size_t)1 << Q.lo_bits) - 1)]; }
+template <class TE> __device__ __forceinline__ void eq_lo_scale(const TE&, const fr_t&, fr29&, fr29&) {}
+template <> __device__ __forceinline__ void eq_lo_scale<EqHi>(const EqHi&, const fr_t& lo, fr29& e0, fr29& e1) {
+  const fr29 ls = fr29_unpack_s(lo);
+  e0 = fr29_mul(e0, ls); e1 = fr29_mul(e1, ls);
+}
 template <class TE> __device__ __forceinline__ bool eq_gate_ok(const TE&) { return true; }
 template <> __device__ __forceinline__ bool eq_gate_ok<EqNone>(const EqNone& Q) { return Q.gp == nullptr || gate_point_ok(Q.gp, Q.seq); }
+template <> __device__ __forceinline__ bool eq_gate_ok<EqHi>(const EqHi& Q) { return Q.gp == nullptr || gate_point_ok(Q.gp, Q.seq); }
 __device__ __forceinline__ fr29 eq_inline_value(const EqInline&, const EqInlineTables& T, uint32_t lb, size_t i, bool write, fr_t* __restrict__ E_out) {
   if (write) E_out[i] = fr29_store(fr29_mul(T.hi_s[i >> lb], T.lo_u[i & ((1u << lb) - 1u)]));
   return eq_inline_s(T, lb, i);
@@ -352,6 +365,7 @@
   return fr29_unpack_s(mem);
 }
 __device__ __forceinline__ fr29 eq_inline_value(const EqNone&, const EqInlineTables&, uint32_t, size_t, bool, fr_t* __restrict__) { return fr29_zero(); }
+__device__ __forceinline__ fr29 eq_inline_value(const EqHi&, const EqInlineTables&, uint32_t, size_t, bool, fr_t* __restrict__) { return fr29_zero(); }
 __device__ __forceinline__ fr_t fr_load_nt(const fr_t* p) {
   const lasso_u32x4* q = reinterpret_cast<const lasso_u32x4*>(p);
   const lasso_u32x4 x = __builtin_nontemporal_load(q), y = __builtin_nontemporal_load(q + 1);
@@ -371,6 +385,7 @@
   fr29_acc w0 = fr29_acc_zero(), w1 = fr29_acc_zero();
   const size_t stride = (size_t)nx * blockDim.x;
   size_t i = g.bx * (size_t)blockDim.x + threadIdx.x;
+  const fr_t lom = eq_lo_load(EQ, i);
   if (NT == 3) {
     for (; i < half; i += stride) {
       fr29 t0, t2, t3;
@@ -378,18 +393,18 @@
     }
   } else if (!pipeline) {
     for (; i < half; i += stride) {
-      const fr29 es = fr29_unpack_s(E[i]), b0 = fr29_unpack_u(b[i]), b1 = fr29_unpack_u(b[i + half]);
+      const fr29 es = fr29_unpack_s(*eq_entry(EQ, E, i)), b0 = fr29_unpack_u(b[i]), b1 = fr29_unpack_u(b[i + half]);
       const fr29 g0 = fr29_mul(fr29_unpack_u(a[i]), es), g1 = fr29_mul(fr29_unpack_u(a[i + half]), es);
       fr29_mul_acc(w0, b0, g0); fr29_mul_acc(w1, fr29_sub(g1, g0), fr29_sub(b1, b0));
       if (++cnt == 3) { fr29_acc_carry(w0); fr29_acc_carry(w1); cnt = 0; }
     }
   } else if (i < half) {
 #define LB_LD(ptr) (NTL ? fr_load_nt(ptr) : *(ptr))
-    fr_t a0 = LB_LD(a + i), a1 = LB_LD(a + i + half), b0m = LB_LD(b + i), b1m = LB_LD(b + i + half), em = EQI ? fr_zero() : E[i];
+    fr_t a0 = LB_LD(a + i), a1 = LB_LD(a + i + half), b0m = LB_LD(b + i), b1m = LB_LD(b + i + half), em = EQI ? fr_zero() : *eq_entry(EQ, E, i);
     for (;;) {
       const size_t in = i + stride; const bool more = in < half;
       const size_t ip = more ? in : i;
-      const fr_t na0 = LB_LD(a + ip), na1 = LB_LD(a + ip + half), nb0 = LB_LD(b + ip), nb1 = LB_LD(b + ip + half), ne = EQI ? fr_zero() : E[ip];
+      const fr_t na0 = LB_LD(a + ip), na1 = LB_LD(a + ip + half), nb0 = LB_LD(b + ip), nb1 = LB_LD(b + ip + half), ne = EQI ? fr_zero() : *eq_entry(EQ, E, ip);
 #undef LB_LD
       fr29 es;
       if (EQI) es = eq_inline_value(EQ, ET, elb, i, g.by == 0, E_out);
@@ -402,16 +417,17 @@
       a0 = na0; a1 = na1; b0m = nb0; b1m = nb1; em = ne; i = in;
     }
   }
-  if (NT == 2) { fr29_acc_carry(w0); fr29_acc_carry(w1); e[0] = fr29_acc_reduce(w0); e[1] = fr29_acc_reduce(w1); }
+  if (NT == 2) { fr29_acc_carry(w0); fr29_acc_carry(w1); e[0] = fr29_acc_reduce(w0); e[1] = fr29_acc_reduce(w1); eq_lo_scale(EQ, lom, e[0], e[1]); }
   cubic_epilogue(e, g, partials, counters, out, flag, seq, S, 5, NT);
 }
-template <int NT, bool WIDE = false, class TM = MutPtrTable, bool AHEAD = false>
+template <int NT, bool WIDE = false, class TM = MutPtrTable, bool AHEAD = false, class TE = EqNone>
 #ifdef LASSO_FUSED_WAVES
 __attribute__((amdgpu_waves_per_eu(LASSO_FUSED_WAVES, LASSO_FUSED_WAVES)))
 #endif
 __global__ void __launch_bounds__(LASSO_BLOCK) k_cubic_eqw_fused(TM A, TM B, uint32_t nx, uint32_t ny, const fr_t* __restrict__ E, size_t q, fr_t r,
                                                                   fr_t* __restrict__ partials, uint32_t* counters, fr_t* __restrict__ out, uint32_t* flag, uint32_t seq,
-                                                                  const uint32_t* gmail = nullptr, const uint32_t* mail = nullptr) {
+                                                                  const uint32_t* gmail = nullptr, const uint32_t* mail = nullptr, TE EQ = TE()) {
+  static_assert(!eq_is_hi<TE>::value || NT == 2, "the factor form serves the two-sum rounds");
   __shared__ RedScratch S;
   const CubicGrid g = cubic_grid(nx, ny);
   fr_t* __restrict__ a = A.p[g.by];
@@ -429,22 +445,25 @@
   const fr29 rs = fr29_unpack_s(r);
   fr29 e[3] = {fr29_zero(), fr29_zero(), fr29_zero()}; uint32_t cnt = 0;
   fr29_acc w0 = fr29_acc_zero(), w1 = fr29_acc_zero();
-  for (size_t i = g.bx * (size_t)blockDim.x + threadIdx.x; i < q; i += (size_t)nx * blockDim.x) {
+  const size_t i0 = g.bx * (size_t)blockDim.x + threadIdx.x;
+  const fr_t lom = eq_lo_load(EQ, i0);
+  for (size_t i = i0; i < q; i += (size_t)nx * blockDim.x) {
     const fr29 a0 = NT == 2 ? bind29_semi(a[i], a[i + 2 * q], rs) : bind29(a[i], a[i + 2 * q], rs), a1 = NT == 2 ? bind29_semi(a[i + q], a[i + 3 * q], rs) : bind29(a[i + q], a[i + 3 * q], rs);
     a[i] = fr29_pack(a0); a[i + q] = fr29_pack(a1);
     const fr29 b0 = NT == 2 ? bind29_semi(b[i], b[i + 2 * q], rs) : bind29(b[i], b[i + 2 * q], rs), b1 = NT == 2 ? bind29_semi(b[i + q], b[i + 3 * q], rs) : bind29(b[i + q], b[i + 3 * q], rs);
     b[i] = fr29_pack(b0); b[i + q] = fr29_pack(b1);
     fr29 t0, t2, t3;
     if (NT == 3) { cubic_eqw_terms(a0, a1, b0, b1, fr29_unpack_s(E[i]), t0, t2, t3); CUBIC_ACCUMULATE(e, t0, t2, t3, cnt); }
-    else if (!WIDE) { cubic_eqw_terms2(a0, a1, b0, b1, fr29_unpack_s(E[i]), t0, t2); CUBIC_ACCUMULATE2(e, t0, t2, cnt); }
+    else if (!WIDE) { cubic_eqw_terms2(a0, a1, b0, b1, fr29_unpack_s(*eq_entry(EQ, E, i)), t0, t2); CUBIC_ACCUMULATE2(e, t0, t2, cnt); }
     else {
-      const fr29 es = fr29_unpack_s(E[i]);
+      const fr29 es = fr29_unpack_s(*eq_entry(EQ, E, i));
       const fr29 g0 = fr29_mul(a0, es), g1 = fr29_mul(a1, es);
       fr29_mul_acc(w0, b0, g0); fr29_mul_acc(w1, fr29_sub(g1, g0), fr29_sub(b1, b0));
       if (++cnt == 3) { fr29_acc_carry(w0); fr29_acc_carry(w1); cnt = 0; }
     }
   }
   if (WIDE && NT == 2) { fr29_acc_carry(w0); fr29_acc_carry(w1); e[0] = fr29_acc_reduce(w0); e[1] = fr29_acc_reduce(w1); }
+  if (NT == 2) eq_lo_scale(EQ, lom, e[0], e[1]);
   cubic_epilogue(e, g, partials, counters, out, flag, seq, S, 5, NT);
 }
 template <bool BIND, int NT, class TM = MutPtrTable>
@@ -1107,6 +1126,45 @@
   for (uint32_t j = 0; j < ell; j++) { const bool bit = (x >> (ell - 1 - j)) & 1; const fr29 rs = fr29_unpack_s(gate_point_fr(gp, j0 + j)); p = fr29_mul(bit ? rs : fr29_sub(one_s, rs), p); }
   (is_lo ? lo : hi)[x] = fr29_store(p);
 }
+struct EqPointArgs { RTable16 Rh, Rl; fr_t scale; uint32_t hi_bits; };
+struct EqPointMem { const uint32_t* gp; uint32_t seq; };
+template <class F> __device__ __forceinline__ fr29 eq_chain(fr29 p, size_t x, uint32_t bits, F coord) {
+  const fr29 one_s = fr29_one_s();
+  for (uint32_t j = 0; j < bits; j++) { const bool bit = (x >> (bits - 1 - j)) & 1; const fr29 rs = fr29_unpack_s(coord(j)); p = fr29_mul(bit ? rs : fr29_sub(one_s, rs), p); }
+  return p;
+}
+__global__ void k_eq_compact(EqPointArgs Q, uint32_t hi_blocks, uint32_t lo_bits, uint32_t lo_blocks, size_t pre, fr_t* __restrict__ hi, fr_t* __restrict__ lo, fr_t* __restrict__ prefix) {
+  if (blockIdx.x < hi_blocks) {
+    const size_t x = blockIdx.x * (size_t)blockDim.x + threadIdx.x; if (x >= ((size_t)1 << Q.hi_bits)) return;
+    hi[x] = fr29_store(eq_chain(fr29_unpack_u(Q.scale), x, Q.hi_bits, [&](uint32_t j) { return Q.Rh.r[j]; }));
+  } else if (blockIdx.x < hi_blocks + lo_blocks) {
+    const size_t x = (blockIdx.x - hi_blocks) * (size_t)blockDim.x + threadIdx.x; if (x >= ((size_t)1 << lo_bits)) return;
+    lo[x] = fr29_store(eq_chain(fr29_unpack_u(fr_one()), x, lo_bits, [&](uint32_t j) { return Q.Rl.r[j]; }));
+  } else {
+    const size_t x = (blockIdx.x - hi_blocks - lo_blocks) * (size_t)blockDim.x + threadIdx.x; if (x >= pre) return;
+    const fr29 h = eq_chain(fr29_unpack_u(Q.scale), x >> lo_bits, Q.hi_bits, [&](uint32_t j) { return Q.Rh.r[j]; });
+    prefix[x] = fr29_store(fr29_mul(h, eq_chain(fr29_one_s(), x & (((size_t)1 << lo_bits) - 1), lo_bits, [&](uint32_t j) { return Q.Rl.r[j]; })));
+  }
+}
+__global__ void k_eq_compact_mem(EqPointMem Q, uint32_t hi_bits, uint32_t hi_blocks, uint32_t lo_bits, uint32_t lo_blocks, size_t pre, fr_t* __restrict__ hi, fr_t* __restrict__ lo, fr_t* __restrict__ prefix) {
+  if (!gate_point_ok(Q.gp, Q.seq)) return;
+  __shared__ fr_t pt[LASSO_POINT_MAX + 1];
+  const uint32_t ell = hi_bits + lo_bits;
+  if (threadIdx.x <= ell) pt[threadIdx.x] = gate_point_fr(Q.gp, threadIdx.x);
+  __syncthreads();
+  const fr29 scale = fr29_unpack_u(pt[ell]);
+  if (blockIdx.x < hi_blocks) {
+    const size_t x = blockIdx.x * (size_t)blockDim.x + threadIdx.x; if (x >= ((size_t)1 << hi_bits)) return;
+    hi[x] = fr29_store(eq_chain(scale, x, hi_bits, [&](uint32_t j) { return pt[j]; }));
+  } else if (blockIdx.x < hi_blocks + lo_blocks) {
+    const size_t x = (blockIdx.x - hi_blocks) * (size_t)blockDim.x + threadIdx.x; if (x >= ((size_t)1 << lo_bits)) return;
+    lo[x] = fr29_store(eq_chain(fr29_unpack_u(fr_one()), x, lo_bits, [&](uint32_t j) { return pt[hi_bits + j]; }));
+  } else {
+    const size_t x = (blockIdx.x - hi_blocks - lo_blocks) * (size_t)blockDim.x + threadIdx.x; if (x >= pre) return;
+    const fr29 h = eq_chain(scale, x >> lo_bits, hi_bits, [&](uint32_t j) { return pt[j]; });
+    prefix[x] = fr29_store(fr29_mul(h, eq_chain(fr29_one_s(), x & (((size_t)1 << lo_bits) - 1), lo_bits, [&](uint32_t j) { return pt[hi_bits + j]; })));
+  }
+}
 __global__ void __launch_bounds__(LASSO_BLOCK) k_eq_outer(const fr_t* __restrict__ hi, const fr_t* __restrict__ lo, uint32_t lo_bits, size_t n, fr_t* __restrict__ out, const uint32_t* __restrict__ gp = nullptr, uint32_t seq = 0) {
   if (gp != nullptr && !gate_point_ok(gp, seq)) return;
   const size_t mask = ((size_t)1 << lo_bits) - 1;
diff --git a/lasso_amd/host/prover.hpp b/lasso_amd/host/prover.hpp
--- a/lasso_amd/host/prover.hpp
+++ b/lasso_amd/host/prover.hpp
@@ -8,6 +8,9 @@
 #include "field_host.hpp"
 #include "field52.hpp"
 #include "switches.hpp"
+#include "../../include/lasso_hip_eq.h"
+extern "C" int32_t lasso_eq_factors_use(lasso_ctx*, lasso_fr*, uint32_t, uint32_t) __attribute__((weak));
+extern "C" int32_t lasso_eq_factors_drop(lasso_ctx*) __attribute__((weak));
 #include "sumcheck_phase.hpp"
 #include "hashes.hpp"
 #include "../../include/lasso_prover.h"
@@ -652,7 +655,16 @@
   std::vector<DBuf> side_keep;
   static size_t tail_q() { static const size_t q = lasso_sumcheck_tail_capacity(); return q; }
   struct LazyEq { bool on = false; std::vector<lasso_fr> rr; lasso_fr scale; lasso_fr* d_table = nullptr; } lazy_eq;
-  struct LayerAhead { bool on = false, tail = false; std::vector<lasso_fr*> A, B; lasso_fr* d_table = nullptr; size_t len = 0, m_stop = 1; uint32_t ell = 0; } layer_ahead;
+  struct LayerAhead { bool on = false, tail = false, compact = false; std::vector<lasso_fr*> A, B; lasso_fr* d_table = nullptr; size_t len = 0, m_stop = 1; uint32_t ell = 0; } layer_ahead;
+  size_t eq_compact_epoch = 0;
+  bool eq_compact_use(lasso_fr* d_table, uint32_t ell, size_t k) {
+    if (!(lasso_eq_factors_use && lasso_eq_factors_drop && sw::eq_factors() && P == 1)) return false;
+    eq_compact_epoch++;
+    const int32_t rc = lasso_eq_factors_use(d.ctx, d_table, ell, (uint32_t)k);
+    if (rc == LASSO_ERR_UNSUPPORTED) return false;
+    d.chk(rc, "lasso_eq_factors_use"); return true;
+  }
+  void eq_compact_drop() { if (lasso_eq_factors_drop) { eq_compact_epoch++; d.chk(lasso_eq_factors_drop(d.ctx), "lasso_eq_factors_drop"); } }
   std::function<void()> next_layer_hook;
   void enqueue_next_layer(const std::vector<lasso_fr*>& trees, size_t n, size_t layer_id, lasso_fr* d_table) {
     layer_ahead.on = false;
@@ -667,9 +679,10 @@
       rc = lasso_sumcheck_cubic_tail_begin_eq_ahead(d.ctx, la.A.data(), la.B.data(), (uint32_t)k, len, ell);
     } else {
       if (ell > 32 || len / 2 <= 64) return;
+      la.compact = eq_compact_use(d_table, ell, k);
       rc = lasso_sumcheck_cubic_eqw2_begin_eq_ahead(d.ctx, la.A.data(), la.B.data(), (uint32_t)k, d_table, len, ell);
     }
-    if (rc == LASSO_ERR_UNSUPPORTED) return;
+    if (rc == LASSO_ERR_UNSUPPORTED) { if (la.compact) eq_compact_drop(); return; }
     d.chk(rc, "lasso_sumcheck_cubic_*_begin_eq_ahead");
     la.on = true; layer_ahead = std::move(la);
   }
@@ -974,18 +987,22 @@
     std::unique_ptr<HostClock> hpro(new HostClock("layer transition: sumcheck prologue"));
     LayerAhead pre = std::move(layer_ahead); layer_ahead.on = false;
     std::function<void()> hook = std::move(next_layer_hook); next_layer_hook = nullptr;
-    if (!rounds) { if (pre.on) d.chk(lasso_point_cancel(d.ctx), "lasso_point_cancel"); return; }
+    if (!rounds) { if (pre.on) { d.chk(lasso_point_cancel(d.ctx), "lasso_point_cancel"); if (pre.compact) eq_compact_drop(); } return; }
     const EqPhase ph(rand, v0, rounds);
     DBuf tj; if (ph.degenerate) tj = DBuf(d, len / 2);
     Sc r_prev = Sc::zero();
     LazyEq lz; if (lazy_eq.on && lazy_eq.d_table == d_E && v0 == 0 && !ph.degenerate) { lz = lazy_eq; } lazy_eq.on = false;
     const size_t tail_from = lasso::tail_from(rounds, len, tail_q(), heads_out && !reduce && !ph.degenerate && sw::cubic_tail(), [&](size_t j0) { return ph.no_zero_from(j0); });
     const HostHandover ho = host_handover(rounds, len, tail_from, host_m_stop(k));
+    const bool compact_ok = !leaf && v0 == 0 && heads_out && !reduce && !sw::cubic_three_sums() && !s_run.is_zero() && ph.no_zero_from(0);
+    bool compact = false; size_t compact_epoch = 0;
+    struct CompactDrop { Prover& p; bool& on; size_t& epoch; ~CompactDrop() { if (on && p.eq_compact_epoch == epoch && lasso_eq_factors_drop) lasso_eq_factors_drop(p.d.ctx); } } compact_drop{*this, compact, compact_epoch};
     bool use_pre = false;
     if (pre.on) {
-      use_pre = lz.on && !ph.degenerate && !leaf && v0 == 0 && heads_out && !reduce && pre.len == len && pre.A == A && pre.B == B && pre.d_table == lz.d_table && pre.ell == lz.rr.size() &&
+      use_pre = (!pre.compact || compact_ok) && lz.on && !ph.degenerate && !leaf && v0 == 0 && heads_out && !reduce && pre.len == len && pre.A == A && pre.B == B && pre.d_table == lz.d_table && pre.ell == lz.rr.size() &&
                 (pre.tail ? (tail_from == 0 && ho.m_stop == pre.m_stop) : (tail_from > 0 && !sw::cubic_three_sums() && !rand[0].is_zero() && !s_run.is_zero()));
-      if (!use_pre) d.chk(lasso_point_cancel(d.ctx), "lasso_point_cancel");
+      if (!use_pre) { d.chk(lasso_point_cancel(d.ctx), "lasso_point_cancel"); if (pre.compact) eq_compact_drop(); }
+      else if (pre.compact) { compact = true; compact_epoch = eq_compact_epoch; }
     }
     const bool ahead_ok = rounds_ahead_ok(ph, reduce, P == 1 && heads_out != nullptr);
     PhaseState st;
@@ -1017,6 +1034,7 @@
         if (j == 1) { A = leaf->work_a; B = leaf->work_b; }
         return true;
       } else if (j == 0 && lz.on && j < tail_from && ell <= 32 && len / 2 > 64) {
+        if (compact_ok && eq_compact_use(lz.d_table, ell, k)) { compact = true; compact_epoch = eq_compact_epoch; }
         d.chk(lasso_sumcheck_cubic_eqw2_begin_eq(d.ctx, A.data(), B.data(), (uint32_t)k, lz.d_table, len, lz.rr.data(), ell, &lz.scale), "lasso_sumcheck_cubic_eqw2_begin_eq"); lz.on = false;
       } else if (j == 0 && lz.on && j >= tail_from && ell <= 9) begin_tail(Tail::with_eq, nullptr, nullptr);
       else {
diff --git a/lasso_amd/host/switches.hpp b/lasso_amd/host/switches.hpp
--- a/lasso_amd/host/switches.hpp
+++ b/lasso_amd/host/switches.hpp
@@ -13,6 +13,7 @@
 LASSO_SWITCH(bool, side_stream, unless0(getenv("LASSO_SIDE_STREAM")))
 LASSO_SWITCH(bool, slab_open, unless0(getenv("LASSO_SLAB_OPEN")))
 LASSO_SWITCH(bool, eq_inline, unless0(getenv("LASSO_EQ_INLINE")))
+LASSO_SWITCH(bool, eq_factors, unless0(getenv("LASSO_EQ_FACTORS")))
 LASSO_SWITCH(bool, cubic_tail, unless0(getenv("LASSO_CUBIC_TAIL")))
 LASSO_SWITCH(bool, linear_tail, unless0(getenv("LASSO_LINEAR_TAIL")))
 LASSO_SWITCH(bool, rounds_ahead, unless0(getenv("LASSO_ROUNDS_AHEAD")))
```

Result: slower. 1.089 billion (-2.6%).
